# emiliofidalgo/liodom

Hardware: AMD Instinct MI355X
Metric: scans/sec (64×1800 cloud, prev_frames=20) at 1 GPU; pose RMSE vs CPU ref (higher is better)
Workload: dtype f64

## Files before the change

liodom_amd/csrc/kernels_knn.h:

```cpp
constexpr float kCellInv = 1.0f;
constexpr double kCellSize = 1.0;

struct Top5 {
  unsigned long long k0, k1, k2, k3, k4;
  int p0, p1, p2, p3, p4;
};
constexpr unsigned long long kTop5Empty = (0x7f800000ull << 32) | 0x7fffffffull;
__device__ __forceinline__ float top5_dist(unsigned long long k) { return __int_as_float((int)(k >> 32)); }
__device__ __forceinline__ int top5_index(unsigned long long k) { return (int)(unsigned int)(k & 0xFFFFFFFFull); }
#define TOP5_STAGE(K, P)                                          \
  {                                                               \
    const bool lt = ck < (K);                                     \
    const unsigned long long nk = lt ? ck : (K);                  \
    const int np = lt ? cp : (P);                                 \
    ck = lt ? (K) : ck;                                           \
    cp = lt ? (P) : cp;                                           \
    (K) = nk; (P) = np;                                           \
  }
__device__ __forceinline__ void top5_insert(Top5& t, float d, int wi, int pos) {
  unsigned long long ck = ((unsigned long long)(unsigned int)__float_as_int(d) << 32) | (unsigned int)wi;
  int cp = pos;
  if (ck < t.k4) {
    TOP5_STAGE(t.k0, t.p0)
    TOP5_STAGE(t.k1, t.p1)
    TOP5_STAGE(t.k2, t.p2)
    TOP5_STAGE(t.k3, t.p3)
    TOP5_STAGE(t.k4, t.p4)
  }
}
#undef TOP5_STAGE
__device__ __forceinline__ void top5_clear(Top5& t) {
  t.k0 = t.k1 = t.k2 = t.k3 = t.k4 = kTop5Empty;
  t.p0 = t.p1 = t.p2 = t.p3 = t.p4 = -1;
}
struct Top5Acc {
  Top5 t;
  __device__ __forceinline__ void consider(bool ok, float d, int wi, int pos) { if (ok && d <= top5_dist(t.k4)) top5_insert(t, d, wi, pos); }
};

struct Best2Acc {
  float m1, m2, m3;
  int p1, p2;
  __device__ __forceinline__ void clear() { m1 = m2 = m3 = __int_as_float(0x7f800000); p1 = p2 = -1; }
  __device__ __forceinline__ void consider(bool ok, float d0, int , int pos) {
    const float d = ok ? d0 : __int_as_float(0x7f800000);
    const bool lt1 = d < m1, lt2 = d < m2;
    m3 = __builtin_amdgcn_fmed3f(m2, m3, d);
    const int q2 = lt2 ? pos : p2;
    p2 = lt1 ? p1 : q2;
    m2 = __builtin_amdgcn_fmed3f(m1, m2, d);
    p1 = lt1 ? pos : p1;
    m1 = lt1 ? d : m1;
  }
};

#ifndef LIODOM_TUNE_B_BIG
#define LIODOM_TUNE_B_BIG 64
#define LIODOM_TUNE_B_LOADS_BIG 2
#define LIODOM_TUNE_B_LOADS_FLAT 2
#define LIODOM_TUNE_B_CURSOR false
#define LIODOM_TUNE_B_NEAR 0.0036f
#endif
#ifndef LIODOM_TUNE_B_WAVES
#define LIODOM_TUNE_B_WAVES 7
#endif
#ifndef LIODOM_TUNE_D_BIG
#define LIODOM_TUNE_D_BIG 128
#define LIODOM_TUNE_D_LOADS 4
#define LIODOM_TUNE_D_NEAR 0.04f
#endif
template <bool kDeep> struct KnnTune {
  static constexpr int kBigCell = kDeep ? LIODOM_TUNE_D_BIG : LIODOM_TUNE_B_BIG;
  static constexpr int kLoadsBig = kDeep ? LIODOM_TUNE_D_LOADS : LIODOM_TUNE_B_LOADS_BIG;
  static constexpr int kLoadsFlat = kDeep ? LIODOM_TUNE_D_LOADS : LIODOM_TUNE_B_LOADS_FLAT;
  static constexpr float kNearSq = kDeep ? LIODOM_TUNE_D_NEAR : LIODOM_TUNE_B_NEAR;
  static constexpr bool kProbeBoth = kDeep;
  static constexpr bool kHoistLoads = kDeep;
  static constexpr bool kCursor = kDeep ? false : LIODOM_TUNE_B_CURSOR;
};
constexpr int kKnnGridDiv = 2;
typedef float f32x2_t __attribute__((ext_vector_type(2)));
__device__ __forceinline__ float sqdist_cand(float qx, float qy, float qz, const float4& m) {
#if defined(LIODOM_KNN_PK)
  const f32x2_t q = {qx, qy};
  const f32x2_t mm = {m.x, m.y};
  const f32x2_t d = q - mm;
  const f32x2_t sq = d * d;
  float r = sq.x;
  r = r + sq.y;
  const float dz = qz - m.z;
  r = r + dz * dz;
  return r;
#else
  return sqdist_f(qx, qy, qz, m.x, m.y, m.z);
#endif
}
template <class Acc, int UB, int U, int kBigCell, bool kCursor = false>
__device__ __forceinline__ void knn_stream_cells(Acc& t, const float4* sp, int* s_incl, int* s_adj,
                                                 unsigned int start, unsigned int cnt, int hl,
                                                 float qx, float qy, float qz, unsigned int* dbg = nullptr) {
  const unsigned long long dbg_t0 = dbg ? wall_clock64() : 0ull;
  {
    const int half_base = (threadIdx.x & 32);
    unsigned int big = (unsigned int)((__ballot(cnt >= (unsigned int)kBigCell) >> half_base) & 0xFFFFFFFFull);
    while (big) {
      const int l = __ffs(big) - 1;
      big &= big - 1u;
      const int cs = __shfl((int)start, l, kKnnGroup), cc = __shfl((int)cnt, l, kKnnGroup);
      const float4* cp = sp + cs;
      for (int i = hl; i < cc; i += UB * kKnnGroup) {
        float4 m[UB];
#pragma unroll
        for (int u = 0; u < UB; u++) { const int iu = i + u * kKnnGroup; m[u] = cp[iu < cc ? iu : cc - 1]; }
#pragma unroll
        for (int u = 0; u < UB; u++) {
          const int iu = i + u * kKnnGroup;
          t.consider(iu < cc, sqdist_cand(qx, qy, qz, m[u]), __float_as_int(m[u].w), cs + iu);
        }
      }
    }
    if (cnt >= (unsigned int)kBigCell) cnt = 0;
  }
  const unsigned int dbg_nseg = dbg ? (unsigned int)__popc((unsigned int)(__ballot(cnt > 0) >> (threadIdx.x & 32))) : 0u;
  const int incl = half_incl_scan_i32((int)cnt);
  s_incl[hl] = incl;
  s_adj[hl] = (int)start - (incl - (int)cnt);
  __builtin_amdgcn_wave_barrier();
  const int T = s_incl[kKnnGroup - 1];
  const unsigned long long dbg_t1 = dbg ? wall_clock64() : 0ull;
  int cur = 0;
  for (int i = hl; i < T; i += U * kKnnGroup) {
    int a[U];
    int c[U];
#pragma unroll
    for (int u = 0; u < U; u++) { const int iu = i + u * kKnnGroup; a[u] = iu < T ? iu : T - 1; c[u] = 0; }
    if (kCursor) {
#pragma unroll
      for (int u = 0; u < U; u++) {
        while (s_incl[cur] <= a[u]) cur++;
        c[u] = cur;
      }
    } else {
#pragma unroll
      for (int step = kKnnGroup / 2; step >= 1; step >>= 1) {
        int pv[U];
#pragma unroll
        for (int u = 0; u < U; u++) pv[u] = s_incl[c[u] + step - 1];
#pragma unroll
        for (int u = 0; u < U; u++) c[u] += pv[u] <= a[u] ? step : 0;
      }
    }
    int adj[U];
#pragma unroll
    for (int u = 0; u < U; u++) adj[u] = s_adj[c[u]];
#pragma unroll
    for (int u = 0; u < U; u++) a[u] += adj[u];
    float4 m[U];
#pragma unroll
    for (int u = 0; u < U; u++) m[u] = sp[a[u]];
#pragma unroll
    for (int u = 0; u < U; u++)
      t.consider(i + u * kKnnGroup < T, sqdist_cand(qx, qy, qz, m[u]), __float_as_int(m[u].w), a[u]);
  }
  __builtin_amdgcn_wave_barrier();
  if (dbg && hl == 0) {
    dbg[0] = (unsigned int)(dbg_t1 - dbg_t0);
    dbg[1] = (unsigned int)(wall_clock64() - dbg_t1);
    dbg[2] = ((unsigned int)((T + U * kKnnGroup - 1) / (U * kKnnGroup)) << 16) | ((unsigned int)T << 20);
    dbg[3] = dbg_nseg;
  }
}

__device__ __forceinline__ bool best2_select(const Best2Acc& t, int hl, int half_shift, float& d5, int (&pos)[5]) {
  unsigned int v = (unsigned int)__float_as_int(t.m1), w = (unsigned int)__float_as_int(t.m2);
  int ph = t.p1, pn = t.p2;
  unsigned int g[6];
#pragma unroll
  for (int r = 0; r < 5; r++) {
    g[r] = half_min_u32(v);
    const unsigned int win = (unsigned int)((__ballot(v == g[r]) >> half_shift) & 0xFFFFFFFFull);
    const int l = __ffs(win) - 1;
    pos[r] = __shfl(ph, l, kKnnGroup);
    const bool mine = hl == l;
    v = mine ? w : v;
    w = mine ? 0x7f800000u : w;
    ph = mine ? pn : ph;
  }
  g[5] = half_min_u32(v);
  const unsigned int s3 = half_min_u32((unsigned int)__float_as_int(t.m3));
  const unsigned int one = 0x3f800000u;
  d5 = __int_as_float((int)g[4]);
  if (g[4] < one) return g[0] < g[1] && g[1] < g[2] && g[2] < g[3] && g[3] < g[4] && g[4] < g[5] && g[4] < s3;
  return s3 >= one;
}


__device__ __forceinline__ void knn_merge(Top5& t, Top5& g, int hl, int half_shift) {
  unsigned long long gk[5]; int gp[5];
#pragma unroll
  for (int r = 0; r < 5; r++) {
    const unsigned long long key = t.k0;
    const unsigned int dmin = half_min_u32((unsigned int)(key >> 32));
    unsigned int win = (unsigned int)((__ballot((unsigned int)(key >> 32) == dmin) >> half_shift) & 0xFFFFFFFFull);
    unsigned long long mk;
    if (__popc(win) == 1) {
      mk = ((unsigned long long)dmin << 32) | (unsigned int)__shfl((int)(unsigned int)(key & 0xFFFFFFFFull), __ffs(win) - 1, kKnnGroup);
    } else {
      mk = half_min_u64(key);
      win = (unsigned int)((__ballot(key == mk) >> half_shift) & 0xFFFFFFFFull);
    }
    const int wl = __ffs(win) - 1;
    gp[r] = __shfl(t.p0, wl, kKnnGroup);
    gk[r] = mk;
    if (hl == wl) {
      t.k0 = t.k1; t.k1 = t.k2; t.k2 = t.k3; t.k3 = t.k4; t.k4 = kTop5Empty;
      t.p0 = t.p1; t.p1 = t.p2; t.p2 = t.p3; t.p3 = t.p4; t.p4 = -1;
    }
  }
  g.k0 = gk[0]; g.k1 = gk[1]; g.k2 = gk[2]; g.k3 = gk[3]; g.k4 = gk[4];
  g.p0 = gp[0]; g.p1 = gp[1]; g.p2 = gp[2]; g.p3 = gp[3]; g.p4 = gp[4];
}

__device__ void rebuild_alloc(const DevView& v, int s, StreamState& st, int block, int nblocks);
__device__ void rebuild_count_and_pad(const DevView& v, int s, StreamState& st, int eb, int block, int* sbase, int* sslot, bool keep);

template <int kQ>
struct KnnShared {
  int incl[kQ][kKnnGroup];
  int adj[kQ][kKnnGroup];
  float nn[kQ][16];
  int res[kQ][4];
  double part[kQ][32];
  double blk[kQ][24];
};

__device__ __forceinline__ float best2_bound(const Best2Acc& t, int half_shift) {
  float B = 1.0f;
  const float thr[4] = {0.36f, 0.09f, 0.0225f, 0.0036f};
#pragma unroll
  for (int k = 0; k < 4; k++) {
    const int c = __popc((unsigned int)(__ballot(t.m1 <= thr[k]) >> half_shift)) + __popc((unsigned int)(__ballot(t.m2 <= thr[k]) >> half_shift));
    B = c >= 5 ? thr[k] : B;
  }
  return B;
}

template <class Tune>
__device__ __forceinline__ void knn_probe_cells(const DevView& v, const StreamState& st, int fc, int hl, int cx, int cy, int cz, float qx, float qy, float qz,
                                                const CellSlot* cells, const unsigned int* bits, unsigned int tmask,
                                                unsigned int& start, unsigned int& cnt, float& lb) {
  if (hl < 27) {
    const int dx = hl % 3 - 1, dy = (hl / 3) % 3 - 1, dz = hl / 9 - 1;
    const unsigned long long key = pack_cell(cx + dx, cy + dy, cz + dz);
    unsigned int h = hash_cell(key, tmask);
    if (Tune::kProbeBoth) {
      const unsigned int word = bits[h >> 5];
      const uint4 raw = *reinterpret_cast<const uint4*>(cells + h);
      const unsigned long long k = ((unsigned long long)raw.y << 32) | raw.x;
      bool more = ((word >> (h & 31)) & 1u) != 0u;
      if (more && k == key) { start = raw.z; cnt = raw.w; more = false; }
      for (int pr = 1; more && pr < v.table_size; pr++) {
        h = (h + 1) & tmask;
        if (!((bits[h >> 5] >> (h & 31)) & 1u)) break;
        const uint4 r2 = *reinterpret_cast<const uint4*>(cells + h);
        if ((((unsigned long long)r2.y << 32) | r2.x) == key) { start = r2.z; cnt = r2.w; break; }
      }
    } else {
      for (int pr = 0; pr < v.table_size; pr++) {
        if (!((bits[h >> 5] >> (h & 31)) & 1u)) break;
        const uint4 raw = *reinterpret_cast<const uint4*>(cells + h);
        const unsigned long long k = ((unsigned long long)raw.y << 32) | raw.x;
        if (k == key) { start = raw.z; cnt = raw.w; break; }
        h = (h + 1) & tmask;
      }
    }
    const float cs = (float)kCellSize;
    const float lx = (float)(cx + dx) * cs, ly = (float)(cy + dy) * cs, lz = (float)(cz + dz) * cs;
    const float ex = qx < lx ? lx - qx : (qx > lx + cs ? qx - (lx + cs) : 0.0f);
    const float ey = qy < ly ? ly - qy : (qy > ly + cs ? qy - (ly + cs) : 0.0f);
    const float ez = qz < lz ? lz - qz : (qz > lz + cs ? qz - (lz + cs) : 0.0f);
    lb = (ex * ex + ey * ey + ez * ez) * (1.0f - 1e-5f);
  } else if (hl == 27 && v.early_rebuild) {
    start = (unsigned int)v.ovf_base;
    cnt = (unsigned int)st.n_ovf[LD_TAB_PARITY(v, fc)];
  }
}

struct KnnPre {
  float gsq;
  float4 sq;
  int p[5];
  float4 c[5];
};
constexpr float kOvMargin = 0.03f;
#ifndef LIODOM_OV_MARGIN_PER_M
#define LIODOM_OV_MARGIN_PER_M 0.004f
#endif
constexpr float kOvMarginPerMetre = LIODOM_OV_MARGIN_PER_M;
constexpr float kOvMarginMax = 0.30f;
template <int kKnnThreads>
__device__ __forceinline__ void knn_presearch(const DevView& v, int s, const StreamState& st, int fc, int e, int E,
                                              KnnShared<kKnnThreads / kKnnGroup>& sh, KnnPre& pre, float range) {
  typedef KnnTune<(kKnnThreads >= 256)> Tune;
  const int grp = threadIdx.x / kKnnGroup, hl = threadIdx.x & (kKnnGroup - 1);
  const int ec = e < v.edge_cap ? e : v.edge_cap - 1;
  pre.gsq = 0.f;
  pre.sq = make_float4(0.f, 0.f, 0.f, __int_as_float(0x7f800000));
#pragma unroll
  for (int k = 0; k < 5; k++) { pre.p[k] = -1; pre.c[k] = make_float4(0.f, 0.f, 0.f, 0.f); }
  if (!v.knn_save_q) return;
  pre.sq = v.knn_save_q[(size_t)s * v.edge_cap + ec];
  const float qx = pre.sq.x, qy = pre.sq.y, qz = pre.sq.z;
  const bool act = e < E && !v.knn_exact_only && ld_isfinite((double)qx) && ld_isfinite((double)qy) && ld_isfinite((double)qz) &&
                   fabsf(qx) < 1.0e9f && fabsf(qy) < 1.0e9f && fabsf(qz) < 1.0e9f;
  if (!act) return;
  const int cx = (int)floorf(qx * kCellInv), cy = (int)floorf(qy * kCellInv), cz = (int)floorf(qz * kCellInv);
  const unsigned int tmask = st.table_mask;
  const int stab = s + LD_TAB_PARITY(v, fc) * v.n_streams;
  const CellSlot* cells = v.cells + (size_t)stab * v.table_size;
  const unsigned int* bits = v.cell_bits + (size_t)stab * (v.table_size >> 5);
  const float4* sp = v.sorted_pts + (size_t)stab * v.sorted_cap;
  unsigned int start = 0, cnt = 0;
  float lb = 0.0f;
  knn_probe_cells<Tune>(v, st, fc, hl, cx, cy, cz, qx, qy, qz, cells, bits, tmask, start, cnt, lb);
  const float margin = fminf(kOvMargin + kOvMarginPerMetre * range, kOvMarginMax);
  const float r = fminf(sqrtf(pre.sq.w), 1.0f) + margin;
  const float B = r * r * (1.0f + 1e-5f);
  Top5Acc ta;
  {
    const unsigned long long sentinel = ((unsigned long long)(unsigned int)__float_as_int(B) << 32) | 0x7fffffffull;
    ta.t.k0 = ta.t.k1 = ta.t.k2 = ta.t.k3 = ta.t.k4 = sentinel;
    ta.t.p0 = ta.t.p1 = ta.t.p2 = ta.t.p3 = ta.t.p4 = -1;
  }
  const bool all = cnt > 0 && !(lb > B);
  knn_stream_cells<Top5Acc, 2, 2, 64>(ta, sp, sh.incl[grp], sh.adj[grp], start, all ? cnt : 0u, hl, qx, qy, qz);
  float gl = B;
  if (ta.t.p4 >= 0) gl = fminf(gl, top5_dist(ta.t.k4));
  pre.gsq = __int_as_float((int)half_min_u32((unsigned int)__float_as_int(gl)));
  pre.p[0] = ta.t.p0; pre.p[1] = ta.t.p1; pre.p[2] = ta.t.p2; pre.p[3] = ta.t.p3; pre.p[4] = ta.t.p4;
#pragma unroll
  for (int k = 0; k < 5; k++) pre.c[k] = sp[pre.p[k] >= 0 ? pre.p[k] : 0];
}

template <int kKnnThreads, bool kPre = false, bool kTail = true, bool kWt = kPre>
__device__ __forceinline__ void knn_block(const DevView& v, int s, StreamState& st, int fc, int outer_it, int eb, int bv, int E,
                                          KnnShared<kKnnThreads / kKnnGroup>& sh, const float4& p_in, const double (&T_in)[12],
                                          const KnnPre& pre, const double* qt) {
  constexpr int kKnnQueries = kKnnThreads / kKnnGroup;
  typedef KnnTune<(kKnnThreads >= 256)> Tune;
  const int grp = threadIdx.x / kKnnGroup;
  const int e = bv * kKnnQueries + grp;
  const int hl = threadIdx.x & (kKnnGroup - 1);
  const int half_shift = (threadIdx.x & 32);
  const bool dbgb = (bv == 5) && (s == 0) && (threadIdx.x == 0) && (outer_it == 0);
  const unsigned long long t_blk = (kInstrument && (v.debug & 32)) ? wall_clock64() : 0ull;
  DBG_STAMP(v, dbgb, 1, 0);
  bool active = e < E;
  float qx = 0.f, qy = 0.f, qz = 0.f;
  if (active) {
    float4 p = p_in;
    double T[12];
#pragma unroll
    for (int i = 0; i < 12; i++) T[i] = T_in[i];
    if (!Tune::kHoistLoads) {
      p = v.edges[((size_t)eb * v.n_streams + s) * v.edge_cap + e];
#pragma unroll
      for (int i = 0; i < 12; i++) T[i] = st.odom[i];
    }
    transform_point(T, p.x, p.y, p.z, &qx, &qy, &qz);
    if (v.knn_q && hl == 0) v.knn_q[((size_t)s * 2 + outer_it) * v.edge_cap + e] = make_float4(qx, qy, qz, 0.f);
    active = ld_isfinite((double)qx) && ld_isfinite((double)qy) && ld_isfinite((double)qz) &&
             fabsf(qx) < 1.0e9f && fabsf(qy) < 1.0e9f && fabsf(qz) < 1.0e9f;
  }
  DBG_STAMP(v, dbgb, 1, 1); DBG_QSTAMP(1);
  if (hl == 0) { sh.res[grp][0] = 0; sh.res[grp][1] = -1; sh.res[grp][2] = -1; }
  float d5 = __int_as_float(0x7f800000);
  if (active) {
    const int cx = (int)floorf(qx * kCellInv), cy = (int)floorf(qy * kCellInv), cz = (int)floorf(qz * kCellInv);
    const unsigned int tmask = st.table_mask;
    const int stab = s + LD_TAB_PARITY(v, fc) * v.n_streams;
    const CellSlot* cells = v.cells + (size_t)stab * v.table_size;
    const unsigned int* bits = v.cell_bits + (size_t)stab * (v.table_size >> 5);
    const float4* sp = v.sorted_pts + (size_t)stab * v.sorted_cap;
    float d5_r = __int_as_float(0x7f800000);
    int pos5[5] = {-1, -1, -1, -1, -1};
    bool reranked = false;
    if (kPre) {
      if ((kInstrument && (v.debug & 64)) && hl == 0 && !(pre.gsq > 0.f)) atomicAdd(&v.dbg_clk[262], 1ull);
      if (pre.gsq > 0.f) {
        Top5 t, g;
        top5_clear(t);
#pragma unroll
        for (int k = 0; k < 5; k++) {
          if (pre.p[k] >= 0) top5_insert(t, sqdist_f(qx, qy, qz, pre.c[k].x, pre.c[k].y, pre.c[k].z), __float_as_int(pre.c[k].w), pre.p[k]);
        }
        knn_merge(t, g, hl, half_shift);
        const float d5n = g.p4 >= 0 ? top5_dist(g.k4) : __int_as_float(0x7f800000);
        const double ddx = (double)qx - (double)pre.sq.x, ddy = (double)qy - (double)pre.sq.y, ddz = (double)qz - (double)pre.sq.z;
        const double delta = sqrt(ddx * ddx + ddy * ddy + ddz * ddz) * (1.0 + 1e-12);
        const double r = sqrt((double)pre.gsq) * (1.0 - 2e-7) - delta;
        double limit = r > 0.0 ? r * r * (1.0 - 1e-6) : 0.0;
        {
          const double cs = kCellSize;
          const double fx = (double)qx - (double)(int)floorf(pre.sq.x * kCellInv) * cs, fy = (double)qy - (double)(int)floorf(pre.sq.y * kCellInv) * cs,
                       fz = (double)qz - (double)(int)floorf(pre.sq.z * kCellInv) * cs;
          const double edge = fmin(fmin(fmin(fx, cs - fx), fmin(fy, cs - fy)), fmin(fz, cs - fz));
          const double ro = (cs + edge) * (1.0 - 2e-7);
          const double lo = ro > 0.0 ? ro * ro * (1.0 - 1e-6) : 0.0;
          limit = limit < lo ? limit : lo;
        }
        reranked = (double)d5n < limit || limit > 1.0;
        if ((kInstrument && (v.debug & 64)) && hl == 0) {
          atomicAdd(&v.dbg_clk[261], 1ull);
          if (!reranked) {
            const float rn = fminf(sqrtf(pre.sq.w), 1.0f) + kOvMargin;
            atomicAdd(&v.dbg_clk[g.p4 < 0 ? 264 : 265], 1ull);
            if (delta > 0.01) atomicAdd(&v.dbg_clk[266], 1ull);
            if (pre.gsq < rn * rn) atomicAdd(&v.dbg_clk[267], 1ull);
            if (!(pre.sq.w < 1.0f)) atomicAdd(&v.dbg_clk[268], 1ull);
            if (delta > 0.03) atomicAdd(&v.dbg_clk[269], 1ull);
          }
        }
        if (reranked) {
          d5_r = d5n;
          pos5[0] = g.p0; pos5[1] = g.p1; pos5[2] = g.p2; pos5[3] = g.p3; pos5[4] = g.p4;
          if (d5n < 1.0f) {
#pragma unroll
            for (int k = 0; k < 5; k++) {
              if (pre.p[k] >= 0) {
                const int r = pre.p[k] == g.p0 ? 0 : pre.p[k] == g.p1 ? 1 : pre.p[k] == g.p2 ? 2 : pre.p[k] == g.p3 ? 3 : pre.p[k] == g.p4 ? 4 : -1;
                if (r >= 0) {
                  sh.nn[grp][r * 3 + 0] = pre.c[k].x; sh.nn[grp][r * 3 + 1] = pre.c[k].y; sh.nn[grp][r * 3 + 2] = pre.c[k].z;
                  if (r < 2) sh.res[grp][1 + r] = __float_as_int(pre.c[k].w);
                }
              }
            }
            if (hl == 0) sh.res[grp][0] = 1;
          }
        }
      }
    } else
    if (outer_it == 1 && v.knn_save_pos && !v.knn_exact_only) {
      const float gsq = v.knn_save_g[(size_t)s * v.edge_cap + e];
      if (gsq > 0.f) {
        const float4 sq = v.knn_save_q[(size_t)s * v.edge_cap + e];
        const int2 sv = v.knn_save_pos[((size_t)s * v.edge_cap + e) * kKnnGroup + hl];
        const float4 m0 = sp[sv.x >= 0 ? sv.x : 0], m1 = sp[sv.y >= 0 ? sv.y : 0];
        Best2Acc br;
        br.clear();
        br.consider(sv.x >= 0, sqdist_f(qx, qy, qz, m0.x, m0.y, m0.z), 0, sv.x);
        br.consider(sv.y >= 0, sqdist_f(qx, qy, qz, m1.x, m1.y, m1.z), 0, sv.y);
        float d5n;
        int p5[5];
        const bool sel_ok = best2_select(br, hl, half_shift, d5n, p5);
        const double ddx = (double)qx - (double)sq.x, ddy = (double)qy - (double)sq.y, ddz = (double)qz - (double)sq.z;
        const double delta = sqrt(ddx * ddx + ddy * ddy + ddz * ddz) * (1.0 + 1e-12);
        const double r = sqrt((double)gsq) * (1.0 - 2e-7) - delta;
        const double limit = r > 0.0 ? r * r * (1.0 - 1e-6) : 0.0;
        reranked = sel_ok && ((double)d5n < limit || limit > 1.0);
        if (reranked) {
          d5_r = d5n;
#pragma unroll
          for (int k = 0; k < 5; k++) pos5[k] = p5[k];
        }
      }
    }
    if ((kInstrument && (v.debug & 64)) && hl == 0 && outer_it == 1) atomicAdd(&v.dbg_clk[259 + (reranked ? 0 : 1)], 1ull);
    if (!reranked) {
    unsigned int start = 0, cnt = 0;
    float lb = 0.0f;
    knn_probe_cells<Tune>(v, st, fc, hl, cx, cy, cz, qx, qy, qz, cells, bits, tmask, start, cnt, lb);
    DBG_STAMP(v, dbgb, 1, 2); DBG_QSTAMP(2);
    float B = 1.0f;
    bool have_b = false;
    if (outer_it == 1 && v.knn_save_q) {
      const float4 sq = kPre ? pre.sq : v.knn_save_q[(size_t)s * v.edge_cap + e];
      if (sq.w < 1.0f) {
        const float ddx = qx - sq.x, ddy = qy - sq.y, ddz = qz - sq.z;
        const float delta = sqrtf(ddx * ddx + ddy * ddy + ddz * ddz);
        const float r = sqrtf(sq.w) * (1.0f + 1e-6f) + delta * (1.0f + 1e-6f) + 1e-7f;
        B = fminf(1.0f, r * r * (1.0f + 1e-5f));
        have_b = true;
      }
    }
    bool pend = cnt > 0;
    Best2Acc b2;
    b2.clear();
    int dbg_n = 0;
    bool dbg_two_phase = false;
    {
      const bool now = pend && (have_b ? !(lb > B) : (hl == 13 || hl == 27 || lb <= Tune::kNearSq));
      if (kInstrument && (v.debug & 32)) dbg_n = __shfl(half_incl_scan_i32(now ? (int)cnt : 0), kKnnGroup - 1, kKnnGroup);
      knn_stream_cells<Best2Acc, Tune::kLoadsBig, Tune::kLoadsFlat, Tune::kBigCell, Tune::kCursor>(b2, sp, sh.incl[grp], sh.adj[grp], start, now ? cnt : 0u, hl, qx, qy, qz,
                                                                                     ((kInstrument && (v.debug & 32)) && s == 0 && e < E) ? v.dbg_q + ((size_t)outer_it * v.edge_cap + e) * 12 + 8 : nullptr);
      pend = pend && !now;
    }
    DBG_STAMP(v, dbgb, 1, 3); DBG_QSTAMP(3);
    if (!have_b && ((__ballot(pend) >> half_shift) & 0xFFFFFFFFull)) {
      B = best2_bound(b2, half_shift);
      pend = pend && !(lb > B);
      if ((__ballot(pend) >> half_shift) & 0xFFFFFFFFull) {
        if (kInstrument && (v.debug & 32)) { dbg_n += __shfl(half_incl_scan_i32(pend ? (int)cnt : 0), kKnnGroup - 1, kKnnGroup); dbg_two_phase = true; }
        knn_stream_cells<Best2Acc, Tune::kLoadsBig, Tune::kLoadsFlat, Tune::kBigCell, Tune::kCursor>(b2, sp, sh.incl[grp], sh.adj[grp], start, pend ? cnt : 0u, hl, qx, qy, qz);
      }
    } else {
      pend = false;
    }
    DBG_STAMP(v, dbgb, 1, 4); DBG_QSTAMP(4);
    const bool certain = best2_select(b2, hl, half_shift, d5, pos5) && !v.knn_exact_only;
    if ((kInstrument && (v.debug & 32)) && s == 0 && e < E && hl == 0) v.dbg_q[((size_t)outer_it * v.edge_cap + e) * 12] = (unsigned int)dbg_n | (dbg_two_phase ? 0x40000000u : 0u) | (certain ? 0u : 0x80000000u);
    if ((kInstrument && (v.debug & 64)) && hl == 0) {
      atomicAdd(&v.dbg_clk[256 + (certain ? 0 : 1)], 1ull);
      if (dbg_two_phase) atomicAdd(&v.dbg_clk[258], 1ull);
      atomicAdd(&v.dbg_clk[384 + (dbg_n / 64 < 63 ? dbg_n / 64 : 63)], 1ull);
    }
    if (!certain) {
      const bool all = cnt > 0 && (!(lb > B) || (!have_b && (hl == 13 || hl == 27 || lb <= Tune::kNearSq)));
      Top5Acc ta;
      Top5 g;
      {
        const float bnd = d5 < 1.0f ? d5 : 1.0f;
        const unsigned long long sentinel = ((unsigned long long)(unsigned int)__float_as_int(bnd) << 32) | 0x7fffffffull;
        ta.t.k0 = ta.t.k1 = ta.t.k2 = ta.t.k3 = ta.t.k4 = sentinel;
        ta.t.p0 = ta.t.p1 = ta.t.p2 = ta.t.p3 = ta.t.p4 = -1;
      }
      knn_stream_cells<Top5Acc, 2, 2, 64>(ta, sp, sh.incl[grp], sh.adj[grp], start, all ? cnt : 0u, hl, qx, qy, qz);
      knn_merge(ta.t, g, hl, half_shift);
      d5 = g.p4 >= 0 ? top5_dist(g.k4) : __int_as_float(0x7f800000);
      pos5[0] = g.p0; pos5[1] = g.p1; pos5[2] = g.p2; pos5[3] = g.p3; pos5[4] = g.p4;
    }
    if (outer_it == 0 && v.knn_save_pos && !(kWt && !kPre)) {
      const float sk = (cnt > 0 && !(!(lb > B) || (!have_b && (hl == 13 || hl == 27 || lb <= Tune::kNearSq)))) ? lb : __int_as_float(0x7f800000);
      unsigned int gd = half_min_u32((unsigned int)__float_as_int(sk));
      const unsigned int m3m = half_min_u32((unsigned int)__float_as_int(b2.m3));
      gd = m3m < gd ? m3m : gd;
      float guard = __int_as_float((int)gd);
      {
        const float cs = (float)kCellSize;
        const float fx = qx - (float)cx * cs, fy = qy - (float)cy * cs, fz = qz - (float)cz * cs;
        float edge = fminf(fminf(fminf(fx, cs - fx), fminf(fy, cs - fy)), fminf(fz, cs - fz));
        edge = edge > 0.f ? edge : 0.f;
        const float outer = (cs + edge) * (cs + edge) * (1.0f - 1e-6f);
        guard = guard < outer ? guard : outer;
      }
      v.knn_save_pos[((size_t)s * v.edge_cap + e) * kKnnGroup + hl] = make_int2(b2.p1, b2.p2);
      if (hl == 0) v.knn_save_g[(size_t)s * v.edge_cap + e] = guard < 3.0e38f ? guard : 3.0e38f;
    }
    if ((kInstrument && (v.debug & 64)) && s == 0 && hl == 0) {
      const int bin = (int)((wall_clock64() - t_blk) / 100ull);
      atomicAdd(&v.dbg_clk[320 + (bin < 63 ? bin : 63)], 1ull);
      const int nb = dbg_n < 64 ? 0 : dbg_n < 128 ? 1 : dbg_n < 256 ? 2 : dbg_n < 512 ? 3 : dbg_n < 1024 ? 4 : 5;
      atomicAdd(&v.dbg_clk[448 + (bin / 4 < 7 ? bin / 4 : 7) * 8 + nb + (dbg_two_phase ? 0 : 0)], 1ull);
      if (!certain) atomicAdd(&v.dbg_clk[448 + (bin / 4 < 7 ? bin / 4 : 7) * 8 + 7], 1ull);
      if (dbg_two_phase) atomicAdd(&v.dbg_clk[448 + (bin / 4 < 7 ? bin / 4 : 7) * 8 + 6], 1ull);
    }
    }
    else d5 = d5_r;
    DBG_STAMP(v, dbgb, 1, 5); DBG_QSTAMP(5);
    if (d5 < 1.0f && !(kPre && reranked)) {
      const int mypos = hl == 0 ? pos5[0] : hl == 1 ? pos5[1] : hl == 2 ? pos5[2] : hl == 3 ? pos5[3] : pos5[4];
      if (hl < 5) {
        const float4 m = sp[mypos];
        sh.nn[grp][hl * 3 + 0] = m.x; sh.nn[grp][hl * 3 + 1] = m.y; sh.nn[grp][hl * 3 + 2] = m.z;
        if (hl < 2) sh.res[grp][1 + hl] = __float_as_int(m.w);
      }
      if (hl == 0) sh.res[grp][0] = 1;
    }
  }
  if (outer_it == 0 && v.knn_save_q && e < E && hl == 0) {
    v.knn_save_q[(size_t)s * v.edge_cap + e] = make_float4(qx, qy, qz, d5);
    if (!active && v.knn_save_g) v.knn_save_g[(size_t)s * v.edge_cap + e] = 0.f;
  }
  if (!kTail) return;
  __syncthreads();
  DBG_STAMP(v, dbgb, 1, 6); DBG_QSTAMP(6);
  if (kKnnThreads < 256 && v.knn_nn) {
    if (threadIdx.x < kKnnQueries * 5) {
      const int q = threadIdx.x / 5, j = threadIdx.x % 5;
      const int eq = bv * kKnnQueries + q;
      if (eq < v.edge_cap) {
        const int w = j == 0 ? sh.res[q][0] : (j == 1 ? sh.res[q][1] : (j == 2 ? sh.res[q][2] : 0));
        v.knn_nn[((size_t)s * v.edge_cap + eq) * 5 + j] = make_float4(sh.nn[q][j * 3], sh.nn[q][j * 3 + 1], sh.nn[q][j * 3 + 2], __int_as_float(w));
      }
    }
    return;
  }
  if (threadIdx.x < kKnnQueries) {
    const int q = threadIdx.x;
    const int eq = bv * kKnnQueries + q;
    bool valid = (eq < E) && (sh.res[q][0] != 0);
    float nx[5], ny[5], nz[5];
#pragma unroll
    for (int j = 0; j < 5; j++) { nx[j] = sh.nn[q][j * 3]; ny[j] = sh.nn[q][j * 3 + 1]; nz[j] = sh.nn[q][j * 3 + 2]; }
    if (valid) valid = line_gate(nx, ny, nz);
    if (eq < E) {
      float4* ca = v.corr_a + ((size_t)s * 2 + outer_it) * v.edge_cap + eq;
      float4* cb = v.corr_b + ((size_t)s * 2 + outer_it) * v.edge_cap + eq;
      int2* cidx = v.corr_idx + ((size_t)s * 2 + outer_it) * v.edge_cap + eq;
      const float4 oa = valid ? make_float4(nx[0], ny[0], nz[0], 1.0f) : make_float4(0, 0, 0, 0);
      const float4 ob = valid ? make_float4(nx[1], ny[1], nz[1], 0.0f) : make_float4(0, 0, 0, 0);
      const int2 oi = valid ? make_int2(sh.res[q][1], sh.res[q][2]) : make_int2(-1, -1);
      if (kWt) {
        wt_store_f4(ca, oa); wt_store_f4(cb, ob);
        wt_store_u64(cidx, ((unsigned long long)(unsigned int)oi.y << 32) | (unsigned int)oi.x);
      } else {
        *ca = oa; *cb = ob; *cidx = oi;
      }
    }
    const unsigned long long vb = __ballot(valid);
    const int nvalid = __popcll(vb);
    if (q == 0) {
      if (nvalid && !v.knn_partials) atomicAdd(&st.info.matches[outer_it], nvalid);
      unsigned char* cm = &v.corr_mask[((size_t)s * 2 + outer_it) * v.mask_stride + bv];
      if (kWt) wt_store_u8(cm, (unsigned char)vb); else *cm = (unsigned char)vb;
    }
    sh.res[q][3] = valid ? 1 : 0;
  } else if (kKnnThreads > 64 && v.knn_partials && threadIdx.x >= 64 && threadIdx.x < 64 + kKnnQueries) {
    const int q = threadIdx.x - 64;
    const int eq = bv * kKnnQueries + q;
    double flag = 0.0;
    if (eq < E && sh.res[q][0] != 0) {
      double Rm[12], pq[4], pt[3];
#pragma unroll
      for (int i = 0; i < 4; i++) pq[i] = kWt ? qt[i] : st.param_q[i];
#pragma unroll
      for (int i = 0; i < 3; i++) pt[i] = kWt ? qt[4 + i] : st.param_t[i];
      iso_from_qt(pq, pt, Rm);
      const float4 pe = v.edges[((size_t)eb * v.n_streams + s) * v.edge_cap + eq];
      const double p[3] = {(double)pe.x, (double)pe.y, (double)pe.z};
      const double a[3] = {(double)sh.nn[q][0], (double)sh.nn[q][1], (double)sh.nn[q][2]};
      const double b[3] = {(double)sh.nn[q][3], (double)sh.nn[q][4], (double)sh.nn[q][5]};
      double J[18], rs[3], rho0, rho1;
      const bool ok = residual_block(Rm, p, a, b, v.min_range, v.max_range, J, rs, &rho0, &rho1);
#pragma unroll
      for (int i = 0; i < 18; i++) sh.blk[q][i] = J[i];
      sh.blk[q][18] = rs[0]; sh.blk[q][19] = rs[1]; sh.blk[q][20] = rs[2]; sh.blk[q][21] = rho0; sh.blk[q][22] = rho1;
      flag = ok ? 1.0 : 2.0;
    }
    sh.blk[q][23] = flag;
  }
  if (!v.knn_partials) return;
  __syncthreads();
  if (hl < kAccN) {
    const double flag = sh.res[grp][3] ? sh.blk[grp][23] : 0.0;
    double x = 0.0;
    if (flag == 1.0) x = residual_entry(sh.blk[grp], sh.blk[grp] + 18, sh.blk[grp][21], sh.blk[grp][22], hl);
    else if (flag == 2.0 && hl == 28) x = 1.0;
    sh.part[grp][hl] = x;
  } else if (hl == kAccN) {
    sh.part[grp][hl] = sh.res[grp][3] ? 1.0 : 0.0;
  }
  __syncthreads();
  if (threadIdx.x <= kAccN) {
    double x = 0.0;
#pragma unroll
    for (int q = 0; q < kKnnQueries; q++) x += sh.part[q][threadIdx.x];
    double* dst = &v.knn_part[(((size_t)s * 2 + outer_it) * v.knn_blocks + bv) * 32 + threadIdx.x];
    if (kWt) wt_store_u64(dst, (unsigned long long)__double_as_longlong(x)); else *dst = x;
  }
  DBG_STAMP(v, dbgb, 1, 7); DBG_QSTAMP(7);
  if ((kInstrument && (v.debug & 64)) && s == 0 && threadIdx.x == 0) {
    const unsigned long long d = wall_clock64() - t_blk;
    const int bin = (int)(d / 100ull);
    atomicAdd(&v.dbg_clk[192 + (bin < 63 ? bin : 63)], 1ull);
  }
}

template <int kKnnThreads>
__device__ __forceinline__ void knn_tail_dual(const DevView& v, int s, int outer_it, int eb, int bvA, int bvB, bool haveB, int E,
                                              KnnShared<kKnnThreads / kKnnGroup>& shA, KnnShared<kKnnThreads / kKnnGroup>& shB, const double* qt) {
  constexpr int kKnnQueries = kKnnThreads / kKnnGroup;
  static_assert(kKnnThreads == 256, "two blocks of 8 queries on four waves");
  const int grp = threadIdx.x / kKnnGroup, hl = threadIdx.x & (kKnnGroup - 1);
  const int half = (int)threadIdx.x >> 7, t = (int)threadIdx.x & 127;
  KnnShared<kKnnQueries>& sh = half ? shB : shA;
  const int bv = half ? bvB : bvA;
  const bool live = half ? haveB : true;
  if (t < kKnnQueries && live) {
    const int q = t;
    const int eq = bv * kKnnQueries + q;
    bool valid = (eq < E) && (sh.res[q][0] != 0);
    float nx[5], ny[5], nz[5];
#pragma unroll
    for (int j = 0; j < 5; j++) { nx[j] = sh.nn[q][j * 3]; ny[j] = sh.nn[q][j * 3 + 1]; nz[j] = sh.nn[q][j * 3 + 2]; }
    if (valid) valid = line_gate(nx, ny, nz);
    if (eq < E) {
      const float4 oa = valid ? make_float4(nx[0], ny[0], nz[0], 1.0f) : make_float4(0, 0, 0, 0);
      const float4 ob = valid ? make_float4(nx[1], ny[1], nz[1], 0.0f) : make_float4(0, 0, 0, 0);
      const int2 oi = valid ? make_int2(sh.res[q][1], sh.res[q][2]) : make_int2(-1, -1);
      wt_store_f4(v.corr_a + ((size_t)s * 2 + outer_it) * v.edge_cap + eq, oa);
      wt_store_f4(v.corr_b + ((size_t)s * 2 + outer_it) * v.edge_cap + eq, ob);
      wt_store_u64(v.corr_idx + ((size_t)s * 2 + outer_it) * v.edge_cap + eq, ((unsigned long long)(unsigned int)oi.y << 32) | (unsigned int)oi.x);
    }
    const unsigned long long vb = __ballot(valid);
    if (q == 0) wt_store_u8(&v.corr_mask[((size_t)s * 2 + outer_it) * v.mask_stride + bv], (unsigned char)vb);
    sh.res[q][3] = valid ? 1 : 0;
  } else if (t >= 64 && t < 64 + kKnnQueries && live) {
    const int q = t - 64;
    const int eq = bv * kKnnQueries + q;
    double flag = 0.0;
    if (eq < E && sh.res[q][0] != 0) {
      double Rm[12], pq[4], pt[3];
#pragma unroll
      for (int i = 0; i < 4; i++) pq[i] = qt[i];
#pragma unroll
      for (int i = 0; i < 3; i++) pt[i] = qt[4 + i];
      iso_from_qt(pq, pt, Rm);
      const float4 pe = v.edges[((size_t)eb * v.n_streams + s) * v.edge_cap + eq];
      const double p[3] = {(double)pe.x, (double)pe.y, (double)pe.z};
      const double a[3] = {(double)sh.nn[q][0], (double)sh.nn[q][1], (double)sh.nn[q][2]};
      const double b[3] = {(double)sh.nn[q][3], (double)sh.nn[q][4], (double)sh.nn[q][5]};
      double J[18], rs[3], rho0, rho1;
      const bool ok = residual_block(Rm, p, a, b, v.min_range, v.max_range, J, rs, &rho0, &rho1);
#pragma unroll
      for (int i = 0; i < 18; i++) sh.blk[q][i] = J[i];
      sh.blk[q][18] = rs[0]; sh.blk[q][19] = rs[1]; sh.blk[q][20] = rs[2]; sh.blk[q][21] = rho0; sh.blk[q][22] = rho1;
      flag = ok ? 1.0 : 2.0;
    }
    sh.blk[q][23] = flag;
  }
  __syncthreads();
#pragma unroll
  for (int b = 0; b < 2; b++) {
    if (b == 1 && !haveB) break;
    KnnShared<kKnnQueries>& shb = b ? shB : shA;
    if (hl < kAccN) {
      const double flag = shb.res[grp][3] ? shb.blk[grp][23] : 0.0;
      double x = 0.0;
      if (flag == 1.0) x = residual_entry(shb.blk[grp], shb.blk[grp] + 18, shb.blk[grp][21], shb.blk[grp][22], hl);
      else if (flag == 2.0 && hl == 28) x = 1.0;
      shb.part[grp][hl] = x;
    } else if (hl == kAccN) {
      shb.part[grp][hl] = shb.res[grp][3] ? 1.0 : 0.0;
    }
  }
  __syncthreads();
  if (t <= kAccN && live) {
    double x = 0.0;
#pragma unroll
    for (int q = 0; q < kKnnQueries; q++) x += sh.part[q][t];
    wt_store_u64(&v.knn_part[(((size_t)s * 2 + outer_it) * v.knn_blocks + bv) * 32 + t], (unsigned long long)__double_as_longlong(x));
  }
}

__device__ __forceinline__ void chain_release_edges(const DevView& v, unsigned int signal_odo) {
  typedef __attribute__((address_space(1))) unsigned int gu32;
  if (signal_odo && threadIdx.x == 0) INJECT_DELAY(14);
  if (signal_odo && threadIdx.x == 0) __hip_atomic_store((gu32*)(v.pipe_flags + kEdgePipeBufs), signal_odo, __ATOMIC_RELAXED, __HIP_MEMORY_SCOPE_AGENT);
}

template <int kKnnThreads, bool kOv, bool kChain>
__device__ __forceinline__ bool knn_pass(const DevView& v, int s, int bxi, int byi, int outer_it, int eb, unsigned int wait_edges,
                                         unsigned int signal_odo, unsigned int seq, int scan_no, KnnShared<kKnnThreads / kKnnGroup>& sh, KnnShared<kKnnThreads / kKnnGroup>& sh2, double* sh_ov, int pred_copy = 0) {
  constexpr int kKnnQueries = kKnnThreads / kKnnGroup;
  static_assert(!(kOv && kChain), "the overlapped pass is the second pass, the chain-mode instance the first");
  StreamState& st = v.state[s];
  if (kOv) {
    if (!pipe_wait(v.ov_flags + s, seq, &st.status)) return false;
    OV_STAMP(v, threadIdx.x == 0 && bxi == 0, 9); OV_STAMP(v, threadIdx.x == 0 && bxi == v.knn_grid - 1, 13);
  } else if (kChain) {
    const bool pred_ok = pred_wait(v, s, bxi % kOvReplicas, (unsigned int)scan_no, sh_ov, &st.status, v.pipe_flags + eb, wait_edges, pred_copy);
    OV_STAMP(v, threadIdx.x == 0 && bxi == 0, 27);
    if (bxi == 0 && threadIdx.x == 0) { st.reb_frame_count = scan_no; st.n_used_tab[(scan_no + 1) & 1] = 0; st.reb_initialized = 1; st.cursor = 0; }
    if (pred_ok && bxi == 0 && threadIdx.x >= 64 && threadIdx.x < 76) st.pred_odom[scan_no & 1][threadIdx.x - 64] = sh_ov[threadIdx.x - 64];
    if (!pred_ok) return false;
  } else if (v.early_rebuild) {
    if (bxi >= v.knn_grid) { if (outer_it == 1) rebuild_alloc(v, s, st, bxi - v.knn_grid, (int)gridDim.x - v.knn_grid); return true; }
    if (outer_it == 0 && bxi == 0 && threadIdx.x == 0) {
      st.reb_frame_count = st.frame_count; st.n_used_tab[(st.frame_count + 1) & 1] = 0; st.reb_initialized = st.initialized;
      st.cursor = 0;
    }
    if (outer_it == 0 && bxi == 0 && threadIdx.x >= 64 && threadIdx.x < 76) st.pred_odom[st.frame_count & 1][threadIdx.x - 64] = st.odom[threadIdx.x - 64];
  }
  if (!kOv && outer_it == 0) {
    if (!kChain && signal_odo && bxi == 0 && byi == 0 && threadIdx.x == 0) {
      typedef __attribute__((address_space(1))) unsigned int gu32;
      __hip_atomic_store((gu32*)(v.pipe_flags + kEdgePipeBufs), signal_odo, __ATOMIC_RELAXED, __HIP_MEMORY_SCOPE_AGENT);
    }
    if (!kChain && wait_edges && !pipe_wait(v.pipe_flags + eb, wait_edges, &st.status)) return false;
  }
  typedef KnnTune<(kKnnThreads >= 256)> Tune;
  const int e_first = bxi * kKnnQueries + (int)(threadIdx.x / kKnnGroup);
  float4 p_first = make_float4(0.f, 0.f, 0.f, 0.f);
  double T[12] = {0, 0, 0, 0, 0, 0, 0, 0, 0, 0, 0, 0};
  if (Tune::kHoistLoads) {
    p_first = v.edges[((size_t)eb * v.n_streams + s) * v.edge_cap + (e_first < v.edge_cap ? e_first : v.edge_cap - 1)];
    if (!kOv && !kChain) {
#pragma unroll
      for (int i = 0; i < 12; i++) T[i] = st.odom[i];
    }
  }
  if (kChain) {
#pragma unroll
    for (int i = 0; i < 12; i++) T[i] = sh_ov[i];
  }
  const unsigned int st_status = st.status;
  const int st_init = kChain ? 1 : st.initialized;
  const int fc = kChain ? scan_no : st.frame_count;
  int E;
  if (kChain) {
    typedef __attribute__((address_space(1))) unsigned int gu32;
    E = (int)__hip_atomic_load((gu32*)(v.edge_cnt + eb * 32 + s), __ATOMIC_RELAXED, __HIP_MEMORY_SCOPE_AGENT);
  } else {
    E = st.n_edges_buf[eb];
  }
  if (st_status & LIODOM_STATUS_PIPE_TIMEOUT) return false;
  if (!st_init) return true;
  static_assert(kKnnGridDiv == 2, "k_knn handles exactly two query blocks per workgroup");
  constexpr bool kWt = kOv || kChain;
  if (bxi * kKnnQueries >= E) {
    if (threadIdx.x == 0) {
      unsigned char* cm = &v.corr_mask[((size_t)s * 2 + outer_it) * v.mask_stride + bxi];
      if (kWt) wt_store_u8(cm, 0); else *cm = 0;
      if (bxi + v.knn_grid < v.knn_blocks) { if (kWt) wt_store_u8(cm + v.knn_grid, 0); else cm[v.knn_grid] = 0; }
    }
    return true;
  }
  const int bv2 = bxi + v.knn_grid;
  const int e_second = bv2 * kKnnQueries + (int)(threadIdx.x / kKnnGroup);
  const bool second = bv2 < v.knn_blocks && bv2 * kKnnQueries < E;
  KnnPre pre1, pre2;
  float4 p_second = make_float4(0.f, 0.f, 0.f, 0.f);
  if (kOv) {
    if (second) p_second = v.edges[((size_t)eb * v.n_streams + s) * v.edge_cap + (e_second < v.edge_cap ? e_second : v.edge_cap - 1)];
    knn_presearch<kKnnThreads>(v, s, st, fc, e_first, E, sh, pre1, sqrtf(p_first.x * p_first.x + p_first.y * p_first.y + p_first.z * p_first.z));
    if (second) knn_presearch<kKnnThreads>(v, s, st, fc, e_second, E, sh2, pre2, sqrtf(p_second.x * p_second.x + p_second.y * p_second.y + p_second.z * p_second.z));
    else pre2.gsq = 0.f;
    if (!ov_wait_pose(v, s, bxi % kOvReplicas, seq, sh_ov, &st.status)) return false;
    OV_STAMP(v, threadIdx.x == 0 && bxi == 0, 10); OV_STAMP(v, threadIdx.x == 0 && bxi == v.knn_grid - 1, 14);
    if (kInstrument && (v.debug & 128) && threadIdx.x == 0) {
      sh_ov[19] = __longlong_as_double((long long)wall_clock64());
      const unsigned long long pub = *(volatile unsigned long long*)&v.dbg_clk[448 + 1];
      const long long d = (long long)wall_clock64() - (long long)pub;
      if (pub && d >= 0) atomicAdd(&v.dbg_clk[320 + (d / 25 < 63 ? d / 25 : 63)], 1ull);
    }
#pragma unroll
    for (int i = 0; i < 12; i++) T[i] = sh_ov[i];
  }
  if constexpr (kOv) {
    knn_block<kKnnThreads, true, false>(v, s, st, fc, outer_it, eb, bxi, E, sh, p_first, T, pre1, sh_ov + 12);
    if (second) knn_block<kKnnThreads, true, false>(v, s, st, fc, outer_it, eb, bv2, E, sh2, p_second, T, pre2, sh_ov + 12);
    else if (bv2 < v.knn_blocks && threadIdx.x == 0) wt_store_u8(&v.corr_mask[((size_t)s * 2 + outer_it) * v.mask_stride + bv2], 0);
    __syncthreads();
    knn_tail_dual<kKnnThreads>(v, s, outer_it, eb, bxi, bv2, second, E, sh, sh2, sh_ov + 12);
    if (!v.speculate) return true;
    const int cf = ov_confirm_pose(v, s, bxi % kOvReplicas, seq, sh_ov, &st.status);
    if ((kInstrument && (v.debug & 64)) && threadIdx.x == 0) atomicAdd(&v.dbg_clk[271 + (cf == 1 ? 0 : 1)], 1ull);
    return cf == 1;
  }
  knn_block<kKnnThreads, false, true, kWt>(v, s, st, fc, outer_it, eb, bxi, E, sh, p_first, T, pre1, kChain ? sh_ov + 12 : nullptr);
  if (bv2 >= v.knn_blocks) return true;
  if (!second) {
    if (threadIdx.x == 0) { unsigned char* cm = &v.corr_mask[((size_t)s * 2 + outer_it) * v.mask_stride + bv2]; if (kWt) wt_store_u8(cm, 0); else *cm = 0; }
    return true;
  }
  __syncthreads();
  double T2[12] = {0, 0, 0, 0, 0, 0, 0, 0, 0, 0, 0, 0};
  if (Tune::kHoistLoads) {
    p_second = v.edges[((size_t)eb * v.n_streams + s) * v.edge_cap + (e_second < v.edge_cap ? e_second : v.edge_cap - 1)];
    asm volatile("" ::: "memory");
    if (kChain) {
#pragma unroll
      for (int i = 0; i < 12; i++) T2[i] = sh_ov[i];
    } else {
#pragma unroll
      for (int i = 0; i < 12; i++) T2[i] = st.odom[i];
    }
  }
  knn_block<kKnnThreads, false, true, kWt>(v, s, st, fc, outer_it, eb, bv2, E, sh, p_second, T2, pre2, kChain ? sh_ov + 12 : nullptr);
  return true;
}

template <int kKnnThreads, bool kOv = false, bool kChain = false>
__global__ __launch_bounds__(kKnnThreads, (kKnnThreads >= 256 ? 1 : LIODOM_TUNE_B_WAVES)) void k_knn(DevView v, int s0, int outer_it, int eb, unsigned int wait_edges, unsigned int signal_odo, unsigned int seq, int scan_no) {
  constexpr int kKnnQueries = kKnnThreads / kKnnGroup;
#if defined(LIODOM_CHAIN_PRIO)
  if (kKnnThreads >= 256) __builtin_amdgcn_s_setprio(LIODOM_CHAIN_PRIO);
#endif
  __shared__ KnnShared<kKnnQueries> shs[kOv ? 2 : 1];
  KnnShared<kKnnQueries>& sh = shs[0];
  __shared__ double sh_ov[(kOv || kChain) ? 20 : 1];
  int bxi = (int)blockIdx.x, byi = (int)blockIdx.y;
  xcd_remap(bxi, byi);
  const int s = s0 + byi;
  if constexpr (kOv) {
    if (bxi >= v.knn_grid) {
      __shared__ int sh_rb_cnt[kMaxFrames + 1];
      __shared__ int sh_rb_slot[kMaxFrames];
      rebuild_count_and_pad(v, s, v.state[s], eb, bxi - v.knn_grid, sh_rb_cnt, sh_rb_slot, true);
      return;
    }
  }
  if (kInstrument && kOv && threadIdx.x == 0) sh_ov[19] = 0.0;
  if (kOv) { OV_STAMP(v, threadIdx.x == 0 && bxi == 0, 8); OV_STAMP(v, threadIdx.x == 0 && bxi == v.knn_grid - 1, 12); }
  else if (outer_it == 0) {
    if (kInstrument && (v.debug & 128) && threadIdx.x == 0 && bxi == 0) {
      volatile unsigned long long* c = v.dbg_clk + 448;
      const unsigned long long t16 = c[16], now = wall_clock64();
      if (t16 && c[18] > t16 && c[1] > c[18] && c[4] > c[1] && c[28] > c[4] && c[26] > c[28]) {
        unsigned long long* a = v.dbg_clk + 480;
        a[0] += c[18] - t16; a[1] += c[1] - c[18]; a[2] += c[4] - c[1]; a[3] += c[28] - c[4]; a[4] += now - t16; a[5] += 1ull;
        a[6] += c[19] > t16 ? 1ull : 0ull; a[7] += c[26] - c[28];
        if (c[20] > c[1]) { a[8] += c[20] - c[1]; a[9] += c[4] - c[20]; }
        if (c[19] > t16 && c[21] < t16) { a[10] += c[1] - c[19]; a[11] += c[20] - c[19]; a[12] += 1ull; a[13] += c[4] - c[1]; }
        if (c[19] > t16 && c[21] > t16) { a[14] += 1ull; a[15] += c[4] - c[1]; }
      }
    }
    OV_STAMP(v, threadIdx.x == 0 && bxi == 0, 16);
  }
  const bool pass_ok = knn_pass<kKnnThreads, kOv, kChain>(v, s, bxi, byi, outer_it, eb, wait_edges, signal_odo, seq, scan_no, sh, shs[kOv ? 1 : 0], sh_ov);
  if (kOv) { if (scan_no >= 0) { if (pass_ok) chain_count_done(v.knn_done0 + 32 + s); } else if (pass_ok || !v.speculate) ov_signal_knn_done(v, s, bxi, seq); }
  if (kChain) {
    int vd = 1;
    if (v.speculate) vd = pred_verdict_wait(v, s, bxi % kOvReplicas, (unsigned int)scan_no, &v.state[s].status);
    if (vd != 2 && bxi == 0) chain_release_edges(v, signal_odo);
    if (pass_ok && vd == 1) chain_count_done(v.knn_done0 + s);
  }
  if (kInstrument && (v.debug & 128) && threadIdx.x == 0) {
    if (kOv) {
      const long long t_seen = __double_as_longlong(sh_ov[19]);
      if (bxi * kKnnQueries < v.state[s].n_edges_buf[eb] && t_seen) { const long long d = (long long)wall_clock64() - t_seen; atomicAdd(&v.dbg_clk[256 + (d / 50 < 63 ? d / 50 : 63)], 1ull); }
    } else if (outer_it == 0) {
      const unsigned long long t0 = *(volatile unsigned long long*)&v.dbg_clk[448 + 16];
      const long long d = (long long)wall_clock64() - (long long)t0;
      if (t0 && d >= 0 && bxi * kKnnQueries < v.state[s].n_edges_buf[eb]) atomicAdd(&v.dbg_clk[384 + (d / 50 < 63 ? d / 50 : 63)], 1ull);
    }
  }
  if (kOv) {
    OV_STAMP(v, threadIdx.x == 0 && bxi == 0, 11); OV_STAMP(v, threadIdx.x == 0 && bxi == v.knn_grid - 1, 15);
    if (kInstrument && (v.debug & 128) && threadIdx.x == 0 && bxi * kKnnQueries < v.state[s].n_edges_buf[eb]) atomicMax(&v.dbg_clk[448 + 20], wall_clock64());
  }
  else if (outer_it == 0) OV_STAMP(v, threadIdx.x == 0 && bxi == v.knn_grid - 1, 17);
}

template <int kKnnThreads>
__global__ __launch_bounds__(kKnnThreads, 1) void k_knn_redo(DevView v, int s0, int eb, unsigned int seq, int scan_no, int alloc_blocks) {
  constexpr int kKnnQueries = kKnnThreads / kKnnGroup;
  __shared__ KnnShared<kKnnQueries> shs[2];
  __shared__ double sh_ov[20];
  __shared__ double sh_first[20];
  if ((int)blockIdx.x < alloc_blocks) { rebuild_alloc(v, s0 + (int)blockIdx.y, v.state[s0 + (int)blockIdx.y], (int)blockIdx.x, alloc_blocks); return; }
  int bxi = (int)blockIdx.x - alloc_blocks, byi = (int)blockIdx.y;
  const int s = s0 + byi;
  StreamState& st = v.state[s];
  const int rep = bxi % kOvReplicas;
  if (!granules_wait<LIODOM_POLL_POSE>(v.pose_xch0 + ((size_t)s * kOvReplicas + rep) * 512, kOvGranules, seq, sh_first, &st.status)) return;
  if (!granules_wait<LIODOM_POLL_POSE>(v.pose_xch0 + ((size_t)s * kOvReplicas + rep) * 512 + kOvFinalOffset, kOvGranules, seq, sh_ov, &st.status)) return;
  bool same = true;
  for (int i = 0; i < 19; i++) same = same && __double_as_longlong(sh_first[i]) == __double_as_longlong(sh_ov[i]);
  if (same) return;
  if (st.status & (LIODOM_STATUS_PIPE_TIMEOUT | LIODOM_STATUS_LM_SYNC_TIMEOUT)) return;
  if ((kInstrument && (v.debug & 64)) && threadIdx.x == 0) atomicAdd(&v.dbg_clk[273], 1ull);
  OV_STAMP(v, threadIdx.x == 0, 21);
  DevView vr = v;
  vr.knn_save_pos = nullptr;
  const int fc = st.frame_count;
  const int E = st.n_edges_buf[eb];
  const int outer_it = 1;
  if (!st.initialized || (st.status & LIODOM_STATUS_PIPE_TIMEOUT)) return;
  const int bv2 = bxi + v.knn_grid;
  if (bxi * kKnnQueries < E) {
    const bool second = bv2 < v.knn_blocks && bv2 * kKnnQueries < E;
    const float4* ed = v.edges + ((size_t)eb * v.n_streams + s) * v.edge_cap;
    const int e_first = bxi * kKnnQueries + (int)(threadIdx.x / kKnnGroup), e_second = bv2 * kKnnQueries + (int)(threadIdx.x / kKnnGroup);
    const float4 p_first = ed[e_first < v.edge_cap ? e_first : v.edge_cap - 1];
    const float4 p_second = ed[e_second < v.edge_cap ? e_second : v.edge_cap - 1];
    double T[12];
#pragma unroll
    for (int i = 0; i < 12; i++) T[i] = sh_ov[i];
    KnnPre none;
    none.gsq = 0.f;
    knn_block<kKnnThreads, false, false, true>(vr, s, st, fc, outer_it, eb, bxi, E, shs[0], p_first, T, none, sh_ov + 12);
    if (second) knn_block<kKnnThreads, false, false, true>(vr, s, st, fc, outer_it, eb, bv2, E, shs[1], p_second, T, none, sh_ov + 12);
    else if (bv2 < v.knn_blocks && threadIdx.x == 0) wt_store_u8(&v.corr_mask[((size_t)s * 2 + outer_it) * v.mask_stride + bv2], 0);
    __syncthreads();
    knn_tail_dual<kKnnThreads>(v, s, outer_it, eb, bxi, bv2, second, E, shs[0], shs[1], sh_ov + 12);
  }
  else return;
  if (scan_no >= 0) chain_count_done(v.knn_done0 + 32 + s); else ov_signal_knn_done(v, s, bxi, seq);
}

__global__ void k_ov_gate(DevView v, int s, unsigned int seq) {
  OV_STAMP(v, threadIdx.x == 0, 6);
  (void)pipe_wait(v.ov_flags + s, seq, &v.state[s].status);
  OV_STAMP(v, threadIdx.x == 0, 7);
}

__global__ __launch_bounds__(256) void k_line_gate(DevView v, int s0, int outer_it, int eb) {
  const int s = s0 + blockIdx.y;
  StreamState& st = v.state[s];
  if (v.knn8_cnt && blockIdx.x == 0 && threadIdx.x == 0) v.knn8_cnt[s] = 0;
  if (!st.initialized) return;
  const int E = st.n_edges_buf[eb];
  const int eq = blockIdx.x * 256 + threadIdx.x;
  const int Q = v.knn_queries;
  if (eq >= v.knn_blocks * Q) return;
  float nx[5], ny[5], nz[5];
  int found = 0, i0 = -1, i1 = -1;
  if (eq < E) {
    const float4* k = v.knn_nn + ((size_t)s * v.edge_cap + eq) * 5;
#pragma unroll
    for (int j = 0; j < 5; j++) {
      const float4 m = k[j];
      nx[j] = m.x; ny[j] = m.y; nz[j] = m.z;
      if (j == 0) found = __float_as_int(m.w);
      if (j == 1) i0 = __float_as_int(m.w);
      if (j == 2) i1 = __float_as_int(m.w);
    }
  } else {
#pragma unroll
    for (int j = 0; j < 5; j++) { nx[j] = 0.f; ny[j] = 0.f; nz[j] = 0.f; }
  }
  bool valid = (eq < E) && (found != 0);
  if (valid) valid = line_gate(nx, ny, nz);
  if (eq < E) {
    float4* ca = v.corr_a + ((size_t)s * 2 + outer_it) * v.edge_cap + eq;
    float4* cb = v.corr_b + ((size_t)s * 2 + outer_it) * v.edge_cap + eq;
    int2* cidx = v.corr_idx + ((size_t)s * 2 + outer_it) * v.edge_cap + eq;
    if (valid) {
      *ca = make_float4(nx[0], ny[0], nz[0], 1.0f);
      *cb = make_float4(nx[1], ny[1], nz[1], 0.0f);
      *cidx = make_int2(i0, i1);
    } else {
      *ca = make_float4(0, 0, 0, 0); *cb = make_float4(0, 0, 0, 0); *cidx = make_int2(-1, -1);
    }
  }
  const unsigned long long vb = __ballot(valid);
  const int lane = threadIdx.x & 63;
  if (lane == 0) { const int nvalid = __popcll(vb); if (nvalid) atomicAdd(&st.info.matches[outer_it], nvalid); }
  if ((lane % Q) == 0) v.corr_mask[((size_t)s * 2 + outer_it) * v.mask_stride + eq / Q] = (unsigned char)((vb >> lane) & ((1ull << Q) - 1ull));
}
```

liodom_amd/csrc/liodom_hip.hip:

```cpp
#include <hip/hip_runtime.h>

#include <algorithm>
#include <cmath>
#include <cstdint>
#include <cstdio>
#include <cstdlib>
#include <cstring>
#include <limits>
#include <atomic>
#include <chrono>
#include <mutex>
#include <string>
#include <vector>

#include "liodom_kernels.h"

using namespace liodom_dev;

namespace {

thread_local std::string g_last_error;

#define HIP_TRY(expr)                                                                         \
  do {                                                                                        \
    hipError_t _e = (expr);                                                                   \
    if (_e != hipSuccess) {                                                                   \
      char _buf[512];                                                                         \
      snprintf(_buf, sizeof(_buf), "%s failed: %s (%s:%d)", #expr, hipGetErrorString(_e),    \
               __FILE__, __LINE__);                                                           \
      g_last_error = _buf;                                                                    \
      return LIODOM_ERR_HIP;                                                                  \
    }                                                                                         \
  } while (0)

enum KernelId {
  KID_CLASSIFY = 0, KID_RING_EXTRACT, KID_COMPACT, KID_KNN, KID_LM, KID_HASH_CLEAR,
  KID_WINDOW_INSERT, KID_HASH_ALLOC, KID_HASH_SCATTER, KID_RING_SCATTER, KID_HASH_BUILD, KID_OTHER
};
const char* kKernelNames[LIODOM_NUM_KERNELS] = {
    "k_classify", "k_ring_extract", "k_compact_edges", "k_knn", "k_lm_solve",
    "k_hash_clear", "k_window_insert", "k_hash_alloc", "k_hash_scatter", "k_ring_scatter", "k_hash_build", "other"};

struct EventPair { hipEvent_t a, b; int kid; };

}

#include "liodom_map_host.h"

std::atomic<int> g_live_handles{0};

struct liodom_handle {
  liodom_handle() {
    for (int b = 0; b < kEdgePipeBufs; b++) { ev_free_valid[b] = false; eb_reader[b] = 0u; tk_seq[b] = 0u; }
  }
  liodom_params_t params;
  liodom_config_t config;
  DevView v{};
  DevView* d_view = nullptr;
  std::mutex mx_x, mx_o;
  hipStream_t stream = nullptr;
  hipStream_t stream_k = nullptr;
  bool counted_live = false;
  bool ov_ok = false;
  unsigned int ov_seq = 0;
  hipEvent_t ev_ov = nullptr;
  bool stream_c_shared = false;
  bool ov_suppress = false;
  bool ov_prev = false;
  double replay_enq_ns = 0.0, replay_wait_ns = 0.0;
  long long replay_timed = 0;
  bool chain_ok = false;
  bool chain_prev = false;
  unsigned int chain_count = 0;
  int verdict_scan = -1;
  bool verdict_confirmed = false;
  bool chain_fix_pending = false;
  bool chain_used = false;
  hipEvent_t ev_ch = nullptr;
  int ov_warm = 0;
  hipStream_t stream_x = nullptr;
  hipStream_t stream_c = nullptr;
  hipEvent_t ev_up[3] = {nullptr, nullptr, nullptr};
  hipEvent_t ev_xdone[3] = {nullptr, nullptr, nullptr};
  bool ev_xdone_valid[3] = {false, false, false};
  hipEvent_t ev_edges[kEdgePipeBufs] = {nullptr, nullptr, nullptr};
  hipEvent_t ev_free[kEdgePipeBufs] = {nullptr, nullptr, nullptr};
  std::atomic<bool> ev_free_valid[kEdgePipeBufs];
  int parity = 0;
  unsigned int ext_seq = 0, odo_seq = 0;
  unsigned int eb_seq[kEdgePipeBufs] = {0, 0, 0};
  std::atomic<unsigned int> eb_reader[kEdgePipeBufs];
  std::atomic<unsigned int> tk_seq[kEdgePipeBufs];
  int x_next = 0;
  int odo_fifo[2] = {0, 0}, odo_pending = 0;
  float4* host_edges = nullptr;
  int4* host_edges_meta = nullptr;
  unsigned int* host_edges_hdr = nullptr;
  float4* pin_ring = nullptr;
  std::vector<double> replay_stamps;
  hipEvent_t ev_pin[kEdgePipeBufs] = {nullptr, nullptr, nullptr};
  bool ev_pin_valid[kEdgePipeBufs] = {false, false, false};
  int pin_next = 0;
  bool safe_mode = false;
  bool ring_split_lb = false;
  unsigned int lb_tag = 0;
  bool ring_split = true;
  int ring_split_max_wgs = 0;
  bool streams_concurrent = true;
  std::atomic<bool> pipe_active{false};
  std::atomic<bool> replay_live{false};
  std::atomic<bool> fallback_pending{false};
  int pf_slot = -1;
  int last_eb = 0;
  hipEvent_t pose_event = nullptr;
  int S = 1, H = 0, P = 0;
  bool lockstep = false;
  size_t ring_lds_bytes = 0;
  float4* stage_in = nullptr;
  float4* resident = nullptr;
  int n_slots = 0;
  HostOut* host_out = nullptr;
  std::vector<int> scans_enqueued;
  std::vector<void*> allocs;
  std::atomic<bool> profiling{false};
  std::vector<liodom_map*> mappers;
  std::vector<int> mapper_cells_xy, mapper_cells_z;
  int hb_since = -1;
  int knn8_grid = 1;
  bool knn8 = false;
  bool lds_hash_build = false;
  bool use_flags = false;
  bool flag_gate = false;
  std::vector<EventPair> ev_pool;
  size_t ev_used = 0;
  double k_ms[LIODOM_NUM_KERNELS] = {0};
  long long k_count[LIODOM_NUM_KERNELS] = {0};
};

namespace {

template <typename T>
int dev_alloc(liodom_handle* h, T** p, size_t count, int memset_value = 0) {
  void* raw = nullptr;
  const size_t bytes = std::max<size_t>(count, 1) * sizeof(T);
  HIP_TRY(hipMalloc(&raw, bytes));
  h->allocs.push_back(raw);
  HIP_TRY(hipMemsetAsync(raw, memset_value, bytes, h->stream));
  *p = static_cast<T*>(raw);
  return LIODOM_OK;
}

void chain_flush(liodom_handle* h) {
  if (!h->chain_fix_pending) return;
  h->chain_fix_pending = false;
  if (h->verdict_scan == h->scans_enqueued[0] && h->verdict_confirmed) return;
  const int nA = (h->v.edge_cap + 255) / 256;
  hipLaunchKernelGGL(k_chain_redo0<256>, dim3(nA, 1), dim3(256), 0, h->stream_k, h->v, 0, 0, 0u, 0u, 0u, h->scans_enqueued[0], nA, 0, 1);
}
hipError_t sync_odometry(liodom_handle* h) {
  chain_flush(h);
  hipError_t e = hipStreamSynchronize(h->stream);
  if (e == hipSuccess && h->chain_used && h->stream_k) e = hipStreamSynchronize(h->stream_k);
  return e;
}

int drain_events(liodom_handle* h) {
  if (h->ev_used == 0) return LIODOM_OK;
  HIP_TRY(hipStreamSynchronize(h->stream));
  if (h->stream_x) HIP_TRY(hipStreamSynchronize(h->stream_x));
  for (size_t i = 0; i < h->ev_used; i++) {
    float ms = 0.f;
    HIP_TRY(hipEventElapsedTime(&ms, h->ev_pool[i].a, h->ev_pool[i].b));
    h->k_ms[h->ev_pool[i].kid] += ms;
    h->k_count[h->ev_pool[i].kid] += 1;
  }
  h->ev_used = 0;
  return LIODOM_OK;
}

struct ProfScope {
  liodom_handle* h;
  EventPair* ep = nullptr;
  hipStream_t st;
  ProfScope(liodom_handle* hh, int kid, hipStream_t stream = nullptr) : h(hh), st(stream ? stream : hh->stream) {
    if (!h->profiling) return;
    if (h->ev_used == h->ev_pool.size()) {
      if (h->ev_pool.size() < 4096) {
        EventPair e; e.kid = kid;
        if (hipEventCreate(&e.a) != hipSuccess || hipEventCreate(&e.b) != hipSuccess) return;
        h->ev_pool.push_back(e);
      } else {
        drain_events(h);
      }
    }
    ep = &h->ev_pool[h->ev_used++];
    ep->kid = kid;
    hipEventRecord(ep->a, st);
  }
  ~ProfScope() { if (ep) hipEventRecord(ep->b, st); }
};

inline int cdiv(long long a, long long b) { return (int)((a + b - 1) / b); }

int launch_extract(liodom_handle* h, hipStream_t q, int eb, int s0, int count, const float4* in, size_t in_stride,
                   int n, int height, int width, unsigned int wait_odo = 0, int mirror = 0, unsigned int* pub_flag = nullptr, unsigned int* pub_host = nullptr, unsigned int pub_value = 0u) {
  const DevView& v = h->v;
  const int tiles = std::max(1, cdiv(n, kTilePts));
  if (v.lidar_type == 1 && width > 0 && (long long)h->H * width <= (long long)v.max_points) {
    ProfScope ps(h, KID_RING_SCATTER, q);
    hipLaunchKernelGGL(k_row_compact, dim3(h->H, count), dim3(kRowThreads), 0, q, v, s0, in, in_stride, n, height, width);
  } else {
    if (h->ring_split_lb && !((long long)tiles * count <= h->ring_split_max_wgs && h->ring_split)) {
      ProfScope ps(h, KID_RING_SCATTER, q);
      if (++h->lb_tag == 0u) h->lb_tag = 1u;
      hipLaunchKernelGGL(k_ring_split_lb, dim3(tiles * count), dim3(kTileThreads), ring_split_lb_lds_bytes(h->H), q, v, s0, in, in_stride, n, height, width, tiles, h->lb_tag);
      hipLaunchKernelGGL(k_ring_split_fix, dim3(1, count), dim3(kTileThreads), ring_split_lb_lds_bytes(h->H), q, v, s0, in, in_stride, n, height, width, tiles);
    } else if (h->ring_split && (long long)tiles * count <= h->ring_split_max_wgs) {
      ProfScope ps(h, KID_RING_SCATTER, q);
      hipLaunchKernelGGL(k_ring_split, dim3(tiles, count), dim3(kTileThreads), ring_scatter_lds_bytes(h->H), q, v, s0, in, in_stride, n, height, width);
    } else {
    {
      ProfScope ps(h, KID_CLASSIFY, q);
      hipLaunchKernelGGL(k_classify, dim3(tiles, count), dim3(kTileThreads), 0, q, v, s0, in, in_stride, n, height, width);
    }
    {
      ProfScope ps(h, KID_RING_SCATTER, q);
      hipLaunchKernelGGL(k_ring_scatter, dim3(tiles, count), dim3(kTileThreads), ring_scatter_lds_bytes(h->H), q, v, s0, in, in_stride, n);
    }
    }
  }
  {
    ProfScope ps(h, KID_RING_EXTRACT, q);
    const int ext = ring_extract_threads(v.scan_regions);
    const int w = h->config.max_width > 0 ? h->config.max_width : std::max(1, h->config.max_points / std::max(1, h->H));
    const int total = std::max(0, w - 10), sector = total / std::max(1, v.scan_regions);
    const bool big = total - sector * (v.scan_regions - 1) > kExLPR * kExIPL;
    const dim3 grid(h->H, count), block(ext);
    if (ext <= 256) {
      if (big) hipLaunchKernelGGL((k_ring_extract<256, kExIPLBig>), grid, block, h->ring_lds_bytes, q, v, s0);
      else hipLaunchKernelGGL((k_ring_extract<256, kExIPL>), grid, block, h->ring_lds_bytes, q, v, s0);
    } else {
      if (big) hipLaunchKernelGGL((k_ring_extract<1024, kExIPLBig>), grid, block, h->ring_lds_bytes, q, v, s0);
      else hipLaunchKernelGGL((k_ring_extract<1024, kExIPL>), grid, block, h->ring_lds_bytes, q, v, s0);
    }
  }
  {
    ProfScope ps(h, KID_COMPACT, q);
    hipLaunchKernelGGL(k_compact_edges, dim3(kCompactBlocks, count), dim3(256), 0, q, v, s0, eb, wait_odo, mirror, pub_flag, pub_host, pub_value);
  }
  HIP_TRY(hipGetLastError());
  return LIODOM_OK;
}

int enqueue_odometry(liodom_handle* h, int eb, int s0, int count, unsigned int wait_edges, unsigned int signal_odo);

int launch_odometry(liodom_handle* h, int eb, int s0, int count, unsigned int wait_edges = 0, unsigned int signal_odo = 0) {
  const int rc = enqueue_odometry(h, eb, s0, count, wait_edges, signal_odo);
  if (rc) return rc;
  h->last_eb = eb;
  for (int i = 0; i < count; i++) h->scans_enqueued[s0 + i]++;
  return LIODOM_OK;
}

struct OverlapModes { bool ov, chain; };
OverlapModes overlap_modes(const liodom_handle* h) {
  const bool base = h->v.early_rebuild && h->use_flags && g_live_handles.load() <= 1;
  return {base && h->ov_ok, base && h->chain_ok && !h->flag_gate};
}

int enqueue_odometry(liodom_handle* h, int eb, int s0, int count, unsigned int wait_edges, unsigned int signal_odo) {
  const DevView& v = h->v;
  const bool knn_small = h->lockstep;
  if (v.use_imu) {
    ProfScope ps(h, KID_OTHER);
    hipLaunchKernelGGL(k_imu_override, dim3(cdiv(count, 64)), dim3(64), 0, h->stream, v, s0, count);
  }
  const int map_blocks = cdiv(h->v.map_cap, 256);
  const bool early = v.early_rebuild != 0;
  const int nC = cdiv(h->v.edge_cap * std::max(1, h->P - 1), kLmThreads), nP = cdiv(h->v.edge_cap, kLmThreads);
  const OverlapModes om = overlap_modes(h);
  const bool chain_cand = om.chain && wait_edges != 0u;
  const bool overlap_ok = (om.ov || chain_cand) && !h->profiling && !h->ov_suppress && count == 1;
  constexpr int kOvWarmScans = 2;
  const bool overlap = overlap_ok && h->ov_warm >= kOvWarmScans;
  if (h->ov_warm < kOvWarmScans) h->ov_warm++;
  unsigned int seq_k = 0u;
  if (overlap) {
    if (++h->ov_seq == 0u) h->ov_seq = 1u;
    seq_k = h->ov_seq;
    if (!h->ov_prev) {
      HIP_TRY(hipEventRecord(h->ev_ov, h->stream));
      HIP_TRY(hipStreamWaitEvent(h->stream_k, h->ev_ov, 0));
    }
  }
  const bool chain = overlap && chain_cand;
  if (chain != h->chain_prev) {
    if (chain) {
      if (h->ov_prev) { HIP_TRY(hipEventRecord(h->ev_ov, h->stream)); HIP_TRY(hipStreamWaitEvent(h->stream_k, h->ev_ov, 0)); }
    } else {
      chain_flush(h);
      HIP_TRY(hipEventRecord(h->ev_ch, h->stream_k));
      HIP_TRY(hipStreamWaitEvent(h->stream, h->ev_ch, 0));
    }
  }
  h->chain_prev = chain;
  h->ov_prev = overlap;
  if (chain) {
    h->chain_used = true;
    const int scan_no = h->scans_enqueued[s0];
    h->chain_count += (unsigned int)v.knn_grid;
    const unsigned int done_target = h->chain_count;
    const int gx = (h->v.lm_groups - 1) * 8 + 1;
    const size_t lds = lm_lds_bytes(h->v.edge_cap);
    const int nCP = cdiv(h->v.edge_cap * std::max(1, h->P - 1), 256) + cdiv(h->v.edge_cap, 256);
    hipLaunchKernelGGL((k_knn<256, false, true>), dim3(v.knn_grid, 1), dim3(256), 0, h->stream_k, v, s0, 0, eb, wait_edges, signal_odo, seq_k, scan_no);
    if (v.speculate) {
      const int nA = cdiv(h->v.edge_cap, 256);
      hipLaunchKernelGGL(k_chain_redo0<256>, dim3(nA + v.knn_grid + 1, 1), dim3(256), 0, h->stream_k, v, s0, eb, wait_edges, signal_odo, seq_k, scan_no, nA, 1, h->chain_fix_pending ? 1 : 0);
    }
    h->chain_fix_pending = v.speculate != 0;
    hipLaunchKernelGGL((k_lm_solve<0, true>), dim3(gx, 1), dim3(kLmThreads), lds, h->stream, v, s0, eb, seq_k, done_target);
    if (!v.speculate) hipLaunchKernelGGL(k_ov_gate, dim3(1), dim3(64), 0, h->stream_k, v, s0, seq_k);
    hipLaunchKernelGGL((k_knn<256, true>), dim3(v.knn_grid + nCP, 1), dim3(256), 0, h->stream_k, v, s0, 1, eb, 0u, 0u, seq_k, scan_no);
    if (v.speculate) hipLaunchKernelGGL(k_knn_redo<256>, dim3(kRebuildAllocBlocks + v.knn_grid, 1), dim3(256), 0, h->stream_k, v, s0, eb, seq_k, scan_no, kRebuildAllocBlocks);
    hipLaunchKernelGGL((k_lm_solve<1, true>), dim3(gx, 1), dim3(kLmThreads), lds, h->stream, v, s0, eb, seq_k, done_target);
    if (!v.speculate) hipLaunchKernelGGL(k_rebuild_alloc, dim3(kRebuildAllocBlocks, 1), dim3(256), 0, h->stream_k, v, s0);
    const int nCf = cdiv(h->v.edge_cap * std::max(1, h->P - 1), kRebFinThreads), nPf = cdiv(h->v.edge_cap, kRebFinThreads);
    hipLaunchKernelGGL(k_rebuild_fin, dim3(nPf + kRebuildAuxBlocks + nCf, 1), dim3(kRebFinThreads), 0, h->stream_k, v, s0, eb);
    HIP_TRY(hipGetLastError());
    return LIODOM_OK;
  }
  for (int it = 0; it < 2; it++) {
    {
      ProfScope ps(h, KID_KNN);
      const int kx = v.knn_grid + ((early && it == 1 && !seq_k) ? kRebuildAuxBlocks : 0);
      if (knn_small && h->knn8) {
        const dim3 g8(h->knn8_grid, count);
        if (it == 0) hipLaunchKernelGGL(k_knn8<0>, g8, dim3(kKnn8Threads), 0, h->stream, v, s0, eb);
        else hipLaunchKernelGGL(k_knn8<1>, g8, dim3(kKnn8Threads), 0, h->stream, v, s0, eb);
        hipLaunchKernelGGL(k_knn8_exact, dim3(kKnn8ExactBlocks, count), dim3(kKnn8Threads), 0, h->stream, v, s0, it, eb);
        hipLaunchKernelGGL(k_line_gate, dim3(cdiv(h->v.knn_blocks * h->v.knn_queries, 256), count), dim3(256), 0, h->stream, v, s0, it, eb);
      } else if (knn_small) {
        hipLaunchKernelGGL(k_knn<128>, dim3(kx, count), dim3(128), 0, h->stream, v, s0, it, eb, wait_edges, signal_odo, 0u, 0);
        hipLaunchKernelGGL(k_line_gate, dim3(cdiv(h->v.knn_blocks * h->v.knn_queries, 256), count), dim3(256), 0, h->stream, v, s0, it, eb);
      } else if (it == 1 && seq_k) {
        hipLaunchKernelGGL(k_ov_gate, dim3(1), dim3(64), 0, h->stream_k, v, s0, seq_k);
        hipLaunchKernelGGL((k_knn<256, true>), dim3(kx, count), dim3(256), 0, h->stream_k, v, s0, it, eb, 0u, 0u, seq_k, -1);
        if (v.speculate) hipLaunchKernelGGL(k_knn_redo<256>, dim3(v.knn_grid, count), dim3(256), 0, h->stream_k, v, s0, eb, seq_k, -1, 0);
        hipLaunchKernelGGL(k_rebuild_alloc, dim3(kRebuildAllocBlocks, count), dim3(256), 0, h->stream, v, s0);
      } else {
        hipLaunchKernelGGL(k_knn<256>, dim3(kx, count), dim3(256), 0, h->stream, v, s0, it, eb, wait_edges, signal_odo, 0u, 0);
      }
    }
    {
      ProfScope ps(h, KID_LM);
      const int extra = !early ? 0 : (it == 0 ? nC + nP : nP + kRebuildAuxBlocks + nC);
      const int gx = std::max(h->v.lm_groups + extra, (h->v.lm_groups - 1) * 8 + 1);
      if (it == 0) hipLaunchKernelGGL((k_lm_solve<0, false>), dim3(gx, count), dim3(kLmThreads), lm_lds_bytes(h->v.edge_cap), h->stream, v, s0, eb, seq_k, 0u);
      else hipLaunchKernelGGL((k_lm_solve<1, false>), dim3(gx, count), dim3(kLmThreads), lm_lds_bytes(h->v.edge_cap), h->stream, v, s0, eb, seq_k, 0u);
    }
  }
  if (v.mapping) {
    for (int s = s0; s < s0 + count; s++) {
      liodom_map* mp = h->mappers[s];
      if (!mp) continue;
      ProfScope ps(h, KID_OTHER);
      StreamState* st = v.state + s;
      int rc = map_enqueue_update(mp, v.edges + ((size_t)eb * v.n_streams + s) * v.edge_cap, &st->n_edges_buf[eb], st->final_odom, h->stream);
      if (rc) return rc;
      rc = map_enqueue_local(mp, st->final_odom, h->mapper_cells_xy[s], h->mapper_cells_z[s], v.recv_pts + (size_t)s * v.recv_cap,
                             v.recv_cap, &st->n_recv, h->stream, 1);
      if (rc) return rc;
    }
  }
  if (early) {
  } else if (h->lds_hash_build) {
    ProfScope ps(h, KID_HASH_BUILD);
    const bool rebuild = !v.hash_incr || h->hb_since < 0 || h->hb_since >= kHbPeriod - 1;
    h->hb_since = rebuild ? 0 : h->hb_since + 1;
    if (!rebuild) hipLaunchKernelGGL(k_hash_append, dim3(count), dim3(kBuildThreads), 0, h->stream, v, s0, eb);
    else hipLaunchKernelGGL(k_hash_build, dim3(count), dim3(kBuildThreads), hash_build_lds_bytes(), h->stream, v, s0, eb);
  } else {
    {
      ProfScope ps(h, KID_WINDOW_INSERT);
      hipLaunchKernelGGL(k_window_insert, dim3(map_blocks, count), dim3(256), 0, h->stream, v, s0, eb);
    }
    {
      ProfScope ps(h, KID_HASH_ALLOC);
      hipLaunchKernelGGL(k_hash_alloc, dim3(map_blocks, count), dim3(256), 0, h->stream, v, s0);
    }
    {
      ProfScope ps(h, KID_HASH_SCATTER);
      hipLaunchKernelGGL(k_hash_scatter, dim3(map_blocks, count), dim3(256), 0, h->stream, v, s0);
    }
  }
  if (v.filter_local_map) {
    {
      ProfScope ps(h, KID_OTHER);
      hipLaunchKernelGGL(k_voxel_bbox, dim3(count), dim3(1024), 0, h->stream, v, s0);
      hipLaunchKernelGGL(k_voxel_insert, dim3(map_blocks, count), dim3(256), 0, h->stream, v, s0);
      hipLaunchKernelGGL(k_voxel_alloc, dim3(map_blocks, count), dim3(256), 0, h->stream, v, s0);
      hipLaunchKernelGGL(k_voxel_scatter, dim3(map_blocks, count), dim3(256), 0, h->stream, v, s0);
      hipLaunchKernelGGL(k_voxel_centroid, dim3(cdiv(h->v.map_cap, 8), count), dim3(256), 0, h->stream, v, s0);
      hipLaunchKernelGGL(k_filt_insert, dim3(map_blocks, count), dim3(256), 0, h->stream, v, s0);
    }
    {
      ProfScope ps(h, KID_HASH_ALLOC);
      hipLaunchKernelGGL(k_filt_alloc, dim3(map_blocks, count), dim3(256), 0, h->stream, v, s0);
    }
    {
      ProfScope ps(h, KID_HASH_SCATTER);
      hipLaunchKernelGGL(k_filt_scatter, dim3(map_blocks, count), dim3(256), 0, h->stream, v, s0);
    }
  }
  HIP_TRY(hipGetLastError());
  return LIODOM_OK;
}

int enter(liodom_handle* h) {
  if (!h) return LIODOM_ERR_INVALID_ARG;
  HIP_TRY(hipSetDevice(h->config.device));
  return LIODOM_OK;
}
int check_stream(liodom_handle* h, int stream) {
  int rc = enter(h);
  if (rc) return rc;
  if (stream < 0 || stream >= h->S) { g_last_error = "stream index out of range"; return LIODOM_ERR_INVALID_ARG; }
  return LIODOM_OK;
}
int check_usable(liodom_handle* h) {
  if (h->fallback_pending.load()) {
    g_last_error = "the handle had a LIODOM_STATUS_PIPE_TIMEOUT: call liodom_reset() before processing further scans";
    return LIODOM_ERR_HIP;
  }
  return LIODOM_OK;
}
struct SideLocks {
  std::unique_lock<std::mutex> lo, lx;
  SideLocks(liodom_handle* h, bool odo, bool ext) {
    if (odo || h->profiling) lo = std::unique_lock<std::mutex>(h->mx_o);
    if (ext || h->profiling) lx = std::unique_lock<std::mutex>(h->mx_x);
    if (h->profiling && !(lo.owns_lock() && lx.owns_lock())) {
      if (lx.owns_lock()) lx.unlock();
      if (!lo.owns_lock()) lo = std::unique_lock<std::mutex>(h->mx_o);
      lx = std::unique_lock<std::mutex>(h->mx_x);
    }
  }
};
hipStream_t extract_queue(liodom_handle* h) { return h->profiling ? h->stream : h->stream_x; }

int round_up(int x, int m) { return (x + m - 1) / m * m; }

int env_int(const char* name, int dflt) {
  const char* e = std::getenv(name);
  return e ? std::atoi(e) : dflt;
}

int tickets_idle(liodom_handle* h) {
  for (int b = 0; b < kEdgePipeBufs; b++) {
    if (h->tk_seq[b].load() != 0u) { g_last_error = "edge tickets of liodom_extract_edges_device are outstanding: consume them with liodom_odometry_step_device first"; return LIODOM_ERR_BUSY; }
  }
  return LIODOM_OK;
}
int drain_pipeline(liodom_handle* h) {
  const bool replayed = h->replay_live.exchange(false);
  if (h->pf_slot >= 0 || h->parity != 0 || h->pipe_active.exchange(false) || replayed) {
    HIP_TRY(hipStreamSynchronize(h->stream_x));
    HIP_TRY(sync_odometry(h));
    h->pf_slot = -1; h->parity = 0; h->ev_free_valid[0] = h->ev_free_valid[1] = h->ev_free_valid[2] = false;
    for (int b = 0; b < kEdgePipeBufs; b++) h->eb_reader[b] = 0;
  }
  return LIODOM_OK;
}

int enqueue_pipeline_odometry(liodom_handle* h, int eb, unsigned int wait_seq) {
  int rc;
  if (h->use_flags) {
    const unsigned int m = ++h->odo_seq == 0 ? ++h->odo_seq : h->odo_seq;
    if (h->flag_gate) {
      hipLaunchKernelGGL(k_pipe_gate, dim3(1), dim3(64), 0, h->stream, h->v, 0, eb, wait_seq, m - 1u);
      rc = launch_odometry(h, eb, 0, h->S);
    } else {
      rc = launch_odometry(h, eb, 0, h->S, wait_seq, m - 1u);
    }
    if (rc) return rc;
    h->eb_reader[eb] = m;
  } else {
    HIP_TRY(hipStreamWaitEvent(h->stream, h->ev_edges[eb], 0));
    rc = launch_odometry(h, eb, 0, h->S);
    if (rc) return rc;
    HIP_TRY(hipEventRecord(h->ev_free[eb], h->stream));
    h->ev_free_valid[eb] = true;
  }
  return LIODOM_OK;
}

int issue_extract(liodom_handle* h, int slot, int eb, int n, int height, int width) {
  hipStream_t q = extract_queue(h);
  const float4* in = h->resident + (size_t)slot * h->S * (size_t)h->v.max_points;
  if (h->use_flags) {
    h->eb_seq[eb] = ++h->ext_seq;
    if (h->ext_seq == 0) h->eb_seq[eb] = ++h->ext_seq;
    return launch_extract(h, q, eb, 0, h->S, in, (size_t)h->v.max_points, n, height, width, h->eb_reader[eb], 0,
                          h->v.pipe_flags + eb, nullptr, h->eb_seq[eb]);
  }
  if (h->ev_free_valid[eb]) HIP_TRY(hipStreamWaitEvent(q, h->ev_free[eb], 0));
  int rc = launch_extract(h, q, eb, 0, h->S, in, (size_t)h->v.max_points, n, height, width);
  if (rc) return rc;
  HIP_TRY(hipEventRecord(h->ev_edges[eb], q));
  return LIODOM_OK;
}

void enter_safe_mode(liodom_handle* h) {
  h->safe_mode = true;
  h->use_flags = false;
  h->chain_ok = false;
  h->v.lm_groups = 1;
  h->v.early_rebuild = 0;
  h->ring_split = false;
  h->ring_split_lb = false;
}

int reset_state(liodom_handle* h) {
  if (h->stream_x) HIP_TRY(hipStreamSynchronize(h->stream_x));
  HIP_TRY(hipStreamSynchronize(h->stream));
  if (h->stream_k) HIP_TRY(hipStreamSynchronize(h->stream_k));
  if (h->fallback_pending.exchange(false)) enter_safe_mode(h);
  std::vector<StreamState> init((size_t)h->S);
  for (auto& st : init) {
    std::memset(&st, 0, sizeof(st));
    iso_identity(st.odom); iso_identity(st.prev_odom); iso_identity(st.final_odom); iso_identity(st.pred_odom[0]); iso_identity(st.pred_odom[1]);
    st.param_q[3] = 1.0;
    st.table_mask = (uint32_t)h->v.table_size - 1u;
  }
  HIP_TRY(hipMemcpyAsync(h->v.state, init.data(), sizeof(StreamState) * init.size(), hipMemcpyHostToDevice, h->stream));
  HIP_TRY(hipMemsetAsync(h->v.pub_counter, 0, sizeof(unsigned int) * (size_t)kEdgeBufs, h->stream));
  if (h->v.lb_ticket) { HIP_TRY(hipMemsetAsync(h->v.lb_ticket, 0, sizeof(unsigned int), h->stream)); HIP_TRY(hipMemsetAsync(h->v.lb_ovf, 0, sizeof(unsigned int) * (size_t)h->S, h->stream)); }
  {
    std::vector<double> qid((size_t)h->S * 4, 0.0);
    for (int s = 0; s < h->S; s++) qid[(size_t)s * 4 + 3] = 1.0;
    HIP_TRY(hipMemcpy(h->v.imu_q, qid.data(), sizeof(double) * qid.size(), hipMemcpyHostToDevice));
  }
  {
    const size_t total = (size_t)h->S * h->v.table_size * (h->v.early_rebuild ? 2 : 1);
    hipLaunchKernelGGL(k_init_cells, dim3((unsigned)((total + 255) / 256)), dim3(256), 0, h->stream, h->v);
    HIP_TRY(hipGetLastError());
  }
  h->pf_slot = -1; h->parity = 0; h->last_eb = 0; h->ev_free_valid[0] = h->ev_free_valid[1] = h->ev_free_valid[2] = false;
  h->replay_live.store(false);
  h->hb_since = -1;
  h->ext_seq = h->odo_seq = 0;
  h->ov_warm = 0; h->ov_prev = false;
  for (int b = 0; b < kEdgePipeBufs; b++) { h->tk_seq[b] = 0u; h->ev_pin_valid[b] = false; }
  if (h->stream_c && !h->stream_c_shared) HIP_TRY(hipStreamSynchronize(h->stream_c));
  h->x_next = 0; h->odo_pending = 0;
  if (h->host_edges_hdr) std::memset(h->host_edges_hdr, 0, sizeof(unsigned int) * 2 * kEdgePipeBufs);
  for (int b = 0; b < kEdgePipeBufs; b++) { h->eb_seq[b] = 0; h->eb_reader[b] = 0; }
  HIP_TRY(hipMemsetAsync(h->v.pipe_flags, 0, sizeof(unsigned int) * (kEdgePipeBufs + 1), h->stream));
  HIP_TRY(hipMemsetAsync(h->v.lm_xch, 0, sizeof(unsigned long long) * (size_t)h->S * 2 * kLmGroupsMax * 64, h->stream));
  HIP_TRY(hipMemsetAsync(h->v.pose_xch, 0, sizeof(unsigned long long) * (size_t)h->S * 64, h->stream));
  HIP_TRY(hipMemsetAsync(h->v.redo_sync, 0, sizeof(unsigned int) * 64, h->stream));
  if (h->v.pred_xch) HIP_TRY(hipMemsetAsync(h->v.pred_xch, 0, sizeof(unsigned long long) * (size_t)h->S * kOvReplicas * 512, h->stream));
  HIP_TRY(hipMemsetAsync(h->v.knn_done0, 0, sizeof(unsigned int) * ((size_t)h->S + 64), h->stream));
  h->chain_prev = false; h->chain_count = 0; h->chain_fix_pending = false; h->verdict_scan = -1; h->replay_enq_ns = 0.0; h->replay_wait_ns = 0.0; h->replay_timed = 0;
  std::memset(h->host_out, 0, sizeof(HostOut) * 2 * (size_t)h->S);
  std::fill(h->scans_enqueued.begin(), h->scans_enqueued.end(), 0);
  HIP_TRY(hipMemsetAsync(h->v.win_n, 0, sizeof(int) * (size_t)h->S * h->P, h->stream));
  HIP_TRY(hipStreamSynchronize(h->stream));
  return LIODOM_OK;
}

}

extern "C" {

const char* liodom_last_error(void) { return g_last_error.c_str(); }

void liodom_params_default(liodom_params_t* p) {
  if (!p) return;
  std::memset(p, 0, sizeof(*p));
  p->min_range = 3.0;
  p->max_range = 75.0;
  p->lidar_type = 0;
  p->scan_lines = 64;
  p->scan_regions = 8;
  p->edges_per_region = 10;
  p->min_points_per_scan = 8 * 10 + 10;
  p->local_map_size = 5;
  p->save_results = 0;
  std::strcpy(p->results_dir, "~/");
  std::strcpy(p->fixed_frame, "odom");
  std::strcpy(p->base_frame, "base_link");
  p->laser_frame[0] = 0;
  p->use_imu = 0; p->filter_local_map = 0; p->mapping = 0;
  p->publish_tf = 1;
}

void liodom_config_default(liodom_config_t* c) {
  if (!c) return;
  std::memset(c, 0, sizeof(*c));
  c->device = 0; c->n_streams = 1; c->max_points = 64 * 1800; c->max_width = 1800;
  c->reserved1 = 0; c->lm_apply_step_on_ftol = 0; c->pose_log_capacity = 1024; c->debug_buffers = 0;
  c->lm_workgroups = 0;
  c->pose_rotation_mode = 1;
}

int liodom_create(const liodom_params_t* params, const liodom_config_t* config, liodom_handle_t** out) {
  if (!params || !config || !out) return LIODOM_ERR_INVALID_ARG;
  *out = nullptr;
  if (params->scan_lines < 1 || params->scan_lines > 254 || params->scan_regions < 1 ||
      params->edges_per_region < 0 || params->local_map_size < 1 || params->local_map_size > (uint64_t)kMaxFrames ||
      config->n_streams < 1 || config->max_points < 1 || !(params->max_range > params->min_range)) {
    g_last_error = "liodom_create: parameter out of range";
    return LIODOM_ERR_INVALID_ARG;
  }
  int ndev = 0;
  if (hipGetDeviceCount(&ndev) != hipSuccess || ndev <= 0) {
    g_last_error = "no HIP device available (libliodom_hip has no CPU fallback)";
    return LIODOM_ERR_NO_DEVICE;
  }
  if (config->device < 0 || config->device >= ndev) { g_last_error = "bad device ordinal"; return LIODOM_ERR_INVALID_ARG; }
  HIP_TRY(hipSetDevice(config->device));
  liodom_handle* h = new liodom_handle();
  h->params = *params;
  h->config = *config;
  h->S = config->n_streams; h->H = params->scan_lines; h->P = (int)params->local_map_size;
  h->lockstep = config->n_streams >= 16;
  int rc = LIODOM_OK;
  auto fail = [&](int code) { liodom_destroy(h); return code; };
  int prio_least = 0, prio_greatest = 0;
  (void)hipDeviceGetStreamPriorityRange(&prio_least, &prio_greatest);
  const bool use_prio = prio_least != prio_greatest;
  auto make_stream = [&](hipStream_t* st, int prio) {
    return use_prio ? hipStreamCreateWithPriority(st, hipStreamNonBlocking, prio) : hipStreamCreateWithFlags(st, hipStreamNonBlocking);
  };
  if (make_stream(&h->stream, prio_greatest) != hipSuccess) { g_last_error = "hipStreamCreate failed"; return fail(LIODOM_ERR_HIP); }
  if (hipEventCreateWithFlags(&h->ev_ov, hipEventDisableTiming) != hipSuccess) { g_last_error = "hipEventCreate failed"; return fail(LIODOM_ERR_HIP); }
  if (hipEventCreateWithFlags(&h->pose_event, hipEventDisableTiming) != hipSuccess) { g_last_error = "hipEventCreate failed"; return fail(LIODOM_ERR_HIP); }
  const int prio_x = (prio_least - prio_greatest >= 2) ? prio_greatest + 1 : prio_least;
  if (make_stream(&h->stream_x, prio_x) != hipSuccess) { g_last_error = "hipStreamCreate failed"; return fail(LIODOM_ERR_HIP); }
  for (int b = 0; b < kEdgePipeBufs; b++) {
    if (hipEventCreateWithFlags(&h->ev_edges[b], hipEventDisableTiming) != hipSuccess ||
        hipEventCreateWithFlags(&h->ev_free[b], hipEventDisableTiming) != hipSuccess) { g_last_error = "hipEventCreate failed"; return fail(LIODOM_ERR_HIP); }
  }

  DevView& v = h->v;
  v.min_range = params->min_range; v.max_range = params->max_range;
  v.lidar_type = params->lidar_type; v.scan_lines = params->scan_lines;
  v.scan_regions = params->scan_regions; v.edges_per_region = params->edges_per_region;
  v.min_points_per_scan = (long long)params->min_points_per_scan;
  v.prev_frames = h->P;
  v.apply_on_ftol = config->lm_apply_step_on_ftol;
  v.rotation_mode = config->pose_rotation_mode != 0 ? 1 : 0;
  v.filter_local_map = (params->filter_local_map && !params->mapping) ? 1 : 0;
  h->lds_hash_build = h->lockstep;
  {
    int cus = 0;
    (void)hipDeviceGetAttribute(&cus, hipDeviceAttributeMultiprocessorCount, config->device);
    const int ecap = round_up(std::max(1, params->scan_lines * params->scan_regions * (params->edges_per_region + 1)), 64);
    h->use_flags = !h->lockstep;
    h->flag_gate = !(config->n_streams == 1 && cdiv(cdiv(ecap, 8), 2) * 4 <= cus * 12);
    for (const char* name : {"AMD_SERIALIZE_KERNEL", "HIP_LAUNCH_BLOCKING", "ROCPROFILER_PMC", "ROCPROF_COUNTERS"}) {
      const char* e = std::getenv(name);
      if (e && e[0] && std::strcmp(e, "0") != 0) h->use_flags = false;
    }
    if (env_int("LIODOM_PIPE_FLAGS", 1) == 0) h->use_flags = false;
  }
  if (const char* e = std::getenv("LIODOM_HASH_BUILD")) h->lds_hash_build = std::strcmp(e, "global") != 0;
  v.lds_cells_max = std::max(1, std::min(kLdsCellsMax, env_int("LIODOM_LDS_CELLS_MAX", kLdsCellsMax)));
  {
    const int ecap = params->scan_lines * params->scan_regions * (params->edges_per_region + 1);
    const int auto_g = config->n_streams > 4 ? 1 : (ecap >= 2048 ? kLmGroupsMax : (ecap >= 512 ? 4 : 1));
    v.lm_groups = config->lm_workgroups == 0 ? auto_g
                                             : (config->lm_workgroups >= kLmGroupsMax ? kLmGroupsMax : (config->lm_workgroups < 1 ? 1 : config->lm_workgroups));
  }
  v.vox_inv = 1.0f / 0.4f;
  v.n_streams = h->S;
  v.max_points = config->max_points;
  v.ring_cap = config->max_points;
  v.slots_per_ring = params->scan_regions * (params->edges_per_region + 1);
  h->ring_lds_bytes = ring_extract_lds_bytes(v.slots_per_ring, params->scan_regions);
  if (h->ring_lds_bytes > 160 * 1024) { g_last_error = "pick lists (scan_regions * (edges_per_region + 1)) exceed 160 KiB of LDS"; return fail(LIODOM_ERR_CAPACITY); }
  v.edge_cap = round_up(std::max(1, h->H * v.slots_per_ring), 64);
  v.use_imu = params->use_imu ? 1 : 0;
  iso_identity(v.laser_to_base);
  v.mapping = params->mapping ? 1 : 0;
  v.early_rebuild = (!h->lds_hash_build && !v.filter_local_map && !params->mapping && config->n_streams <= 4) ? 1 : 0;
  if (env_int("LIODOM_EARLY_REBUILD", 1) == 0) v.early_rebuild = 0;
  if (env_int("LIODOM_SAFE_MODE", 0) != 0) enter_safe_mode(h);
  v.recv_cap = v.mapping ? (config->recv_capacity > 0 ? config->recv_capacity : 262144) : 0;
  v.map_cap = v.edge_cap * h->P + v.recv_cap;
  int ts = 1024;
  while (ts < 2 * (v.map_cap + (v.early_rebuild ? 8 * v.edge_cap : 0))) ts <<= 1;
  v.table_size = ts;
  v.pose_log_cap = std::max(1, config->pose_log_capacity);
  v.debug = config->debug_buffers & 1;
  if (kInstrument) { const int dc = env_int("LIODOM_DEBUG_CLOCKS", 0); if (dc != 0) v.debug |= ((dc & (128 | 256)) ? (dc & 32) : 32) | (dc & (64 | 128)) | ((dc >> 8) << 8); }
  v.ring_id_stride = (size_t)round_up(config->max_points + 512, 256);

  const size_t S = (size_t)h->S;
#define ALLOC(ptr, count, fill) do { rc = dev_alloc(h, &(ptr), (count), (fill)); if (rc != LIODOM_OK) return fail(rc); } while (0)
  ALLOC(v.state, S, 0);
  ALLOC(v.ring_id, S * v.ring_id_stride, 0xFF);
  v.tile_cap = std::max(1, cdiv(config->max_points, kTilePts));
  ALLOC(v.tile_hist, S * (size_t)v.tile_cap * h->H, 0);
  h->ring_split_lb = h->lockstep && params->lidar_type == 0 && !h->safe_mode && env_int("LIODOM_RING_SPLIT_LB", 1) != 0;
  v.ring_pitch = round_up(cdiv((long long)config->max_points * 9, (long long)std::max(1, h->H) * 8), 8);
  if (const char* e = std::getenv("LIODOM_RING_PITCH")) v.ring_pitch = std::max(8, std::atoi(e));
  v.ring_stride = h->ring_split_lb ? std::max((size_t)config->max_points, (size_t)h->H * (size_t)v.ring_pitch) : (size_t)config->max_points;
  v.lb_hpad = round_up(h->H, 64);
  if (h->ring_split_lb) {
    ALLOC(v.lb_desc, S * (size_t)v.tile_cap * v.lb_hpad, 0); ALLOC(v.lb_ticket, 1, 0); ALLOC(v.lb_ovf, S, 0);
    const size_t lds = ring_split_lb_lds_bytes(h->H);
    if (lds > 48 * 1024 && (hipFuncSetAttribute(reinterpret_cast<const void*>(&k_ring_split_lb), hipFuncAttributeMaxDynamicSharedMemorySize, (int)lds) != hipSuccess ||
                            hipFuncSetAttribute(reinterpret_cast<const void*>(&k_ring_split_fix), hipFuncAttributeMaxDynamicSharedMemorySize, (int)lds) != hipSuccess)) {
      (void)hipGetLastError(); h->ring_split_lb = false;
    }
  } else { v.lb_desc = nullptr; v.lb_ticket = nullptr; v.lb_ovf = nullptr; }
  ALLOC(v.ring_pts, S * v.ring_stride + kExLPR * kExIPLBig + 64, 0);
  ALLOC(v.ring_src, S * v.ring_stride, 0);
  ALLOC(v.ring_start, S * (size_t)(h->H + 1), 0);
  ALLOC(v.ring_len, S * (size_t)h->H, 0);
  ALLOC(v.edges_pad, S * h->H * v.slots_per_ring, 0);
  ALLOC(v.edges_pad_meta, S * h->H * v.slots_per_ring, 0);
  ALLOC(v.ring_nedges, S * h->H, 0);
  {
    h->ring_split = env_int("LIODOM_RING_SPLIT", 1) != 0 && !h->safe_mode;
    if (h->ring_split) {
      int cus = 0, per_cu = 0;
      (void)hipDeviceGetAttribute(&cus, hipDeviceAttributeMultiprocessorCount, config->device);
      const size_t lds = ring_scatter_lds_bytes(h->H);
      if (lds > 48 * 1024 &&
          hipFuncSetAttribute(reinterpret_cast<const void*>(&k_ring_split), hipFuncAttributeMaxDynamicSharedMemorySize, (int)lds) != hipSuccess) {
        (void)hipGetLastError(); per_cu = 0;
      } else if (hipOccupancyMaxActiveBlocksPerMultiprocessor(&per_cu, reinterpret_cast<const void*>(&k_ring_split), kTileThreads, lds) != hipSuccess) {
        (void)hipGetLastError(); per_cu = 0;
      }
      long long budget = (long long)std::max(0, per_cu) * std::max(0, cus) / 2;
      if (budget > 256) budget = 256;
      h->ring_split_max_wgs = (int)budget;
      const int tiles_one = std::max(1, cdiv(config->max_points, kTilePts));
      if (tiles_one > h->ring_split_max_wgs) h->ring_split = false;
    }
    v.split_ctr = nullptr;
    v.split_hist = nullptr; v.split_pad = round_up(v.tile_cap, 8);
    if (h->ring_split) { ALLOC(v.split_ctr, 2 * S, 0); ALLOC(v.split_hist, S * (size_t)h->H * v.split_pad + 64, 0); }
  }
  ALLOC(v.ring_npoints, S * h->H, 0);
  ALLOC(v.ring_c, S * v.ring_stride, 0);
  ALLOC(v.ring_picked, S * v.ring_stride, 0);
  ALLOC(v.edges, kEdgeBufs * S * v.edge_cap, 0);
  ALLOC(v.edges_meta, kEdgeBufs * S * v.edge_cap, 0);
  ALLOC(v.corr_a, S * 2 * v.edge_cap, 0);
  ALLOC(v.corr_b, S * 2 * v.edge_cap, 0);
  ALLOC(v.corr_idx, S * 2 * v.edge_cap, 0xFF);
  if (v.debug & 1) ALLOC(v.knn_q, S * 2 * v.edge_cap, 0); else v.knn_q = nullptr;
  ALLOC(v.win_pts, S * h->P * v.edge_cap, 0);
  ALLOC(v.win_n, S * h->P, 0);
  ALLOC(v.win_base, S * (h->P + 1), 0);
  ALLOC(v.win_slot, S * h->P, 0);
  const size_t ntab = v.early_rebuild ? 2 : 1;
  ALLOC(v.cells, ntab * S * v.table_size, 0);
  ALLOC(v.pt_rank, S * v.map_cap, 0);
  ALLOC(v.cell_bits, ntab * S * (size_t)(v.table_size / 32), 0);
  v.used_cap = v.early_rebuild ? v.map_cap + 8 * v.edge_cap : v.map_cap;
  ALLOC(v.used_cells, ntab * S * (size_t)v.used_cap, 0);
  ALLOC(v.pt_cell, S * v.map_cap, 0xFF);
  if (v.recv_cap) ALLOC(v.recv_pts, S * v.recv_cap, 0);
  ALLOC(v.imu_q, S * 4, 0);
  v.ovf_base = v.early_rebuild ? v.map_cap + 8 * v.edge_cap : v.map_cap;
  v.sorted_cap = v.early_rebuild ? v.ovf_base + v.edge_cap : v.map_cap;
  const bool hash_incr_on = env_int("LIODOM_HASH_INCR", 1) != 0;
  if (hash_incr_on && h->lockstep && h->lds_hash_build && !params->mapping && !params->filter_local_map && !v.early_rebuild)
    v.sorted_cap = 2 * v.map_cap + 65536 + (kHbPeriod - 1) * v.edge_cap;
  ALLOC(v.sorted_pts, (v.early_rebuild ? 2 : 1) * S * (size_t)v.sorted_cap, 0);
  if (v.early_rebuild) ALLOC(v.cell_pad, 2 * S * (size_t)v.table_size, 0); else v.cell_pad = nullptr;
  v.rebuild_delta = 0.25f;
  if (const char* e = std::getenv("LIODOM_REBUILD_DELTA")) { const float d = (float)std::atof(e); if (d > 0.0f && d <= 0.45f) v.rebuild_delta = d; }
  if (v.filter_local_map) {
    ALLOC(v.vox_cells, S * v.table_size, 0);
    ALLOC(v.vox_fill, S * v.table_size, 0);
    ALLOC(v.vox_used_list, S * v.map_cap, 0);
    ALLOC(v.pt_vox, S * v.map_cap, 0xFF);
    ALLOC(v.vox_pts, S * v.map_cap, 0);
    ALLOC(v.filt_pts, S * v.map_cap, 0);
    ALLOC(v.filt_int, S * v.map_cap, 0);
  }
  ALLOC(v.pose_log, S * v.pose_log_cap * 7, 0);
  ALLOC(v.info_log, S * v.pose_log_cap, 0);
  ALLOC(h->stage_in, S * (size_t)config->max_points, 0);
  ALLOC(v.dbg_clk, 16 * 32, 0);
  if (v.debug & 32) ALLOC(v.dbg_q, 2 * (size_t)v.edge_cap * 12, 0); else v.dbg_q = nullptr;
  ALLOC(v.lm_xch, S * 2 * kLmGroupsMax * 64, 0);
  ALLOC(v.pose_xch, S * 64, 0);
  ALLOC(v.redo_sync, 64, 0);
  ALLOC(v.pipe_flags, kEdgePipeBufs + 1, 0);
  v.host_edges = nullptr; v.host_edges_meta = nullptr; v.host_edges_hdr = nullptr;
  if (S == 1) {
    const size_t ne = (size_t)kEdgePipeBufs * v.edge_cap;
    void *he = nullptr, *hm = nullptr, *hh = nullptr;
    if (hipHostMalloc(&he, sizeof(float4) * ne, hipHostMallocMapped | hipHostMallocCoherent) != hipSuccess ||
        hipHostMalloc(&hm, sizeof(int4) * ne, hipHostMallocMapped | hipHostMallocCoherent) != hipSuccess ||
        hipHostMalloc(&hh, sizeof(unsigned int) * 2 * kEdgePipeBufs, hipHostMallocMapped | hipHostMallocCoherent) != hipSuccess) {
      if (he) hipHostFree(he);
      if (hm) hipHostFree(hm);
      g_last_error = "hipHostMalloc (edge mirror) failed"; return fail(LIODOM_ERR_HIP);
    }
    h->host_edges = static_cast<float4*>(he); h->host_edges_meta = static_cast<int4*>(hm); h->host_edges_hdr = static_cast<unsigned int*>(hh);
    std::memset(hh, 0, sizeof(unsigned int) * 2 * kEdgePipeBufs);
    void *de = nullptr, *dm = nullptr, *dh = nullptr;
    if (hipHostGetDevicePointer(&de, he, 0) != hipSuccess || hipHostGetDevicePointer(&dm, hm, 0) != hipSuccess ||
        hipHostGetDevicePointer(&dh, hh, 0) != hipSuccess) { g_last_error = "hipHostGetDevicePointer failed"; return fail(LIODOM_ERR_HIP); }
    v.host_edges = static_cast<float4*>(de); v.host_edges_meta = static_cast<int4*>(dm); v.host_edges_hdr = static_cast<unsigned int*>(dh);
  }
  if (h->use_flags) {
    unsigned int* probe = nullptr;
    ALLOC(probe, 4, 0);
    hipLaunchKernelGGL(k_set_flag, dim3(1), dim3(1), 0, h->stream, probe + 2, 1u);
    hipLaunchKernelGGL(k_set_flag, dim3(1), dim3(1), 0, h->stream_x, probe + 3, 1u);
    if (hipStreamSynchronize(h->stream) != hipSuccess || hipStreamSynchronize(h->stream_x) != hipSuccess) { g_last_error = "stream probe failed"; return fail(LIODOM_ERR_HIP); }
    hipLaunchKernelGGL(k_probe_wait, dim3(1), dim3(64), 0, h->stream, probe, probe + 1);
    hipLaunchKernelGGL(k_set_flag, dim3(1), dim3(1), 0, h->stream_x, probe, 1u);
    unsigned int res = 0;
    if (hipStreamSynchronize(h->stream) != hipSuccess || hipStreamSynchronize(h->stream_x) != hipSuccess ||
        hipMemcpy(&res, probe + 1, sizeof(res), hipMemcpyDeviceToHost) != hipSuccess) { g_last_error = "stream probe failed"; return fail(LIODOM_ERR_HIP); }
    h->streams_concurrent = res == 1u;
    if (!h->streams_concurrent) h->use_flags = false;
  }
  if (h->lockstep) ALLOC(v.knn_nn, S * (size_t)v.edge_cap * 5, 0); else v.knn_nn = nullptr;
  h->knn8 = h->lockstep && env_int("LIODOM_KNN8", 1) != 0;
  h->knn8_grid = std::max(1, cdiv(cdiv(v.edge_cap, kKnn8Queries), kKnnGridDiv));
  v.hash_incr = (hash_incr_on && h->knn8 && h->lds_hash_build && !params->mapping && !params->filter_local_map && h->P > kHbPeriod &&
                 v.sorted_cap >= 2 * v.map_cap + (kHbPeriod - 1) * v.edge_cap) ? 1 : 0;
  v.hb_spill_base = v.sorted_cap - (kHbPeriod - 1) * v.edge_cap;
  if (v.hash_incr) ALLOC(v.cell_cap, S * (size_t)v.table_size, 0); else v.cell_cap = nullptr;
  v.hb_slack_min = kHbSlackMin; v.hb_new_room = kHbNewRoom;
  if (const char* e = std::getenv("LIODOM_HB_SLACK")) v.hb_slack_min = std::max(0, std::atoi(e));
  if (const char* e = std::getenv("LIODOM_HB_NEW_ROOM")) v.hb_new_room = std::max(1, std::atoi(e));
  if (h->knn8) { ALLOC(v.knn8_cnt, S, 0); ALLOC(v.knn8_list, S * (size_t)v.edge_cap, 0); } else { v.knn8_cnt = nullptr; v.knn8_list = nullptr; }
  v.knn_queries = h->lockstep ? 4 : 8;
  v.knn_partials = h->lockstep ? 0 : 1;
  v.knn_blocks = round_up(cdiv(v.edge_cap, v.knn_queries), 4);
  v.knn_grid = std::max(1, cdiv(v.knn_blocks, kKnnGridDiv));
  {
    const int save = env_int("LIODOM_KNN_SAVE", 2);
    if (save >= 1) ALLOC(v.knn_save_q, S * (size_t)v.edge_cap, 0); else v.knn_save_q = nullptr;
    if (save >= 2) { ALLOC(v.knn_save_pos, S * (size_t)v.edge_cap * kKnnGroup, 0xFF); ALLOC(v.knn_save_g, S * (size_t)v.edge_cap, 0); }
    else { v.knn_save_pos = nullptr; v.knn_save_g = nullptr; }
  }
  v.knn_exact_only = env_int("LIODOM_KNN_EXACT_ONLY", 0) != 0 ? 1 : 0;
  ALLOC(v.knn_part, S * 2 * (size_t)v.knn_blocks * 32, 0);
  ALLOC(v.ov_flags, S, 0);
  ALLOC(v.pose_xch0, S * (size_t)kOvReplicas * 512, 0);
  ALLOC(v.knn_done, S * (size_t)v.knn_grid, 0);
  ALLOC(v.knn_done0, S + 64, 0);
  if (v.early_rebuild) ALLOC(v.pred_xch, S * (size_t)kOvReplicas * 512, 0); else v.pred_xch = nullptr;
  ALLOC(v.edge_cnt, (size_t)kEdgeBufs * 32, 0);
  ALLOC(v.pub_counter, (size_t)kEdgeBufs, 0);
  if (v.early_rebuild) ALLOC(v.edges_keep, S * (size_t)v.edge_cap, 0); else v.edges_keep = nullptr;
  v.mask_stride = round_up(v.knn_blocks, 128);
  ALLOC(v.corr_mask, S * 2 * (size_t)v.mask_stride, 0);
  {
    void* hp = nullptr;
    if (hipHostMalloc(&hp, sizeof(HostOut) * 2 * S, hipHostMallocMapped | hipHostMallocCoherent) != hipSuccess) { g_last_error = "hipHostMalloc failed"; return fail(LIODOM_ERR_HIP); }
    h->host_out = static_cast<HostOut*>(hp);
    std::memset(hp, 0, sizeof(HostOut) * 2 * S);
    void* dp = nullptr;
    if (hipHostGetDevicePointer(&dp, hp, 0) != hipSuccess) { g_last_error = "hipHostGetDevicePointer failed"; return fail(LIODOM_ERR_HIP); }
    v.host_out = static_cast<HostOut*>(dp);
    h->scans_enqueued.assign(S, 0);
    h->mappers.assign(S, nullptr); h->mapper_cells_xy.assign(S, 2); h->mapper_cells_z.assign(S, 1);
  }
  if (ring_scatter_lds_bytes(h->H) > 48 * 1024) {
    if (hipFuncSetAttribute(reinterpret_cast<const void*>(&k_ring_scatter), hipFuncAttributeMaxDynamicSharedMemorySize,
                            (int)ring_scatter_lds_bytes(h->H)) != hipSuccess) {
      g_last_error = "hipFuncSetAttribute(max dynamic LDS) failed"; return fail(LIODOM_ERR_HIP);
    }
  }
  if (hipFuncSetAttribute(reinterpret_cast<const void*>(&k_hash_build), hipFuncAttributeMaxDynamicSharedMemorySize,
                          (int)hash_build_lds_bytes()) != hipSuccess) {
    g_last_error = "hipFuncSetAttribute(max dynamic LDS) failed"; return fail(LIODOM_ERR_HIP);
  }
  v.lm_lds_reduce = lm_lds_reduce_fits(v.edge_cap) ? 1 : 0;
  if (lm_lds_bytes(v.edge_cap) + 8192 > 160 * 1024) { g_last_error = "liodom_create: edge capacity too large for the solve's LDS tile"; return fail(LIODOM_ERR_INVALID_ARG); }
  if (hipFuncSetAttribute(reinterpret_cast<const void*>(&k_lm_solve<0, false>), hipFuncAttributeMaxDynamicSharedMemorySize, (int)lm_lds_bytes(h->v.edge_cap)) != hipSuccess ||
      hipFuncSetAttribute(reinterpret_cast<const void*>(&k_lm_solve<1, false>), hipFuncAttributeMaxDynamicSharedMemorySize, (int)lm_lds_bytes(h->v.edge_cap)) != hipSuccess ||
      hipFuncSetAttribute(reinterpret_cast<const void*>(&k_lm_solve<0, true>), hipFuncAttributeMaxDynamicSharedMemorySize, (int)lm_lds_bytes(h->v.edge_cap)) != hipSuccess ||
      hipFuncSetAttribute(reinterpret_cast<const void*>(&k_lm_solve<1, true>), hipFuncAttributeMaxDynamicSharedMemorySize, (int)lm_lds_bytes(h->v.edge_cap)) != hipSuccess) {
    g_last_error = "hipFuncSetAttribute(max dynamic LDS) failed"; return fail(LIODOM_ERR_HIP);
  }
  if (h->ring_lds_bytes > 48 * 1024) {
    if (hipFuncSetAttribute(reinterpret_cast<const void*>(&k_ring_extract<256, kExIPL>), hipFuncAttributeMaxDynamicSharedMemorySize, (int)h->ring_lds_bytes) != hipSuccess ||
        hipFuncSetAttribute(reinterpret_cast<const void*>(&k_ring_extract<256, kExIPLBig>), hipFuncAttributeMaxDynamicSharedMemorySize, (int)h->ring_lds_bytes) != hipSuccess ||
        hipFuncSetAttribute(reinterpret_cast<const void*>(&k_ring_extract<1024, kExIPL>), hipFuncAttributeMaxDynamicSharedMemorySize, (int)h->ring_lds_bytes) != hipSuccess ||
        hipFuncSetAttribute(reinterpret_cast<const void*>(&k_ring_extract<1024, kExIPLBig>), hipFuncAttributeMaxDynamicSharedMemorySize, (int)h->ring_lds_bytes) != hipSuccess) {
      g_last_error = "hipFuncSetAttribute(max dynamic LDS) failed"; return fail(LIODOM_ERR_HIP);
    }
  }
  {
    int cus = 0;
    (void)hipDeviceGetAttribute(&cus, hipDeviceAttributeMultiprocessorCount, config->device);
    const int knn_overlap = env_int("LIODOM_KNN_OVERLAP", 1);
    h->ov_ok = knn_overlap != 0 && v.early_rebuild && S == 1 && v.knn_partials && (knn_overlap == 2 || (long long)v.knn_grid * 4 * 3 <= (long long)cus * 24);
    h->chain_ok = v.early_rebuild && S == 1 && v.knn_partials && !v.use_imu && (long long)v.knn_grid * 4 * 2 <= (long long)cus * 24;
    if (knn_overlap == 0 || env_int("LIODOM_CHAIN", 1) == 0) h->chain_ok = false;
    v.speculate = (h->ov_ok || h->chain_ok) ? 1 : 0;
    if (v.speculate) v.speculate = std::max(0, std::min(7, env_int("LIODOM_SPECULATE", 1)));
    v.spec_backoff = 16;
    v.spec_theta = 0.8;
    if (const char* e = std::getenv("LIODOM_SPEC_THETA")) v.spec_theta = std::atof(e);
    if ((h->ov_ok || h->chain_ok) && make_stream(&h->stream_k, prio_greatest) != hipSuccess) { g_last_error = "hipStreamCreate failed"; return fail(LIODOM_ERR_HIP); }
    if (h->chain_ok && hipEventCreateWithFlags(&h->ev_ch, hipEventDisableTiming) != hipSuccess) { g_last_error = "hipEventCreate failed"; return fail(LIODOM_ERR_HIP); }
  }
  {
    double ms = 50.0;
    if (const char* e = std::getenv("LIODOM_WAIT_MS")) { const double x = std::atof(e); if (x >= 1.0 && x <= 10000.0) ms = x; }
    const unsigned long long ticks = (unsigned long long)(ms * 1.0e5);
    if (hipMemcpyToSymbol(HIP_SYMBOL(g_wait_ticks), &ticks, sizeof(ticks)) != hipSuccess) { g_last_error = "hipMemcpyToSymbol(g_wait_ticks) failed"; return fail(LIODOM_ERR_HIP); }
  }
  ALLOC(h->d_view, 1, 0);
  if (hipMemcpy(h->d_view, &h->v, sizeof(DevView), hipMemcpyHostToDevice) != hipSuccess) { g_last_error = "DevView upload failed"; return fail(LIODOM_ERR_HIP); }
  rc = reset_state(h);
  if (rc != LIODOM_OK) return fail(rc);
  g_live_handles.fetch_add(1);
  h->counted_live = true;
  *out = h;
  return LIODOM_OK;
#undef ALLOC
}

void liodom_destroy(liodom_handle_t* h) {
  if (!h) return;
  if (h->counted_live) g_live_handles.fetch_sub(1);
  if (h->stream_x) hipStreamSynchronize(h->stream_x);
  if (h->stream) hipStreamSynchronize(h->stream);
  if (h->stream_k) { hipStreamSynchronize(h->stream_k); hipStreamDestroy(h->stream_k); }
  if (h->ev_ov) hipEventDestroy(h->ev_ov);
  if (h->ev_ch) hipEventDestroy(h->ev_ch);
  for (liodom_map* mp : h->mappers) {
    if (!mp) continue;
    mp->stream = nullptr; mp->own_stream = false;
    if (hipStreamCreateWithFlags(&mp->stream, hipStreamNonBlocking) == hipSuccess) mp->own_stream = true;
  }
  for (void* p : h->allocs) hipFree(p);
  if (h->resident) hipFree(h->resident);
  if (h->host_out) hipHostFree(h->host_out);
  if (h->host_edges) hipHostFree(h->host_edges);
  if (h->host_edges_meta) hipHostFree(h->host_edges_meta);
  if (h->host_edges_hdr) hipHostFree(h->host_edges_hdr);
  if (h->pin_ring) hipHostFree(h->pin_ring);
  for (int b = 0; b < kEdgePipeBufs; b++) { if (h->ev_pin[b]) hipEventDestroy(h->ev_pin[b]); }
  for (auto& e : h->ev_pool) { hipEventDestroy(e.a); hipEventDestroy(e.b); }
  if (h->pose_event) hipEventDestroy(h->pose_event);
  for (int b = 0; b < kEdgePipeBufs; b++) { if (h->ev_edges[b]) hipEventDestroy(h->ev_edges[b]); if (h->ev_free[b]) hipEventDestroy(h->ev_free[b]); }
  if (h->stream_c && !h->stream_c_shared) { hipStreamSynchronize(h->stream_c); hipStreamDestroy(h->stream_c); }
  for (int b = 0; b < 3; b++) { if (h->ev_up[b]) hipEventDestroy(h->ev_up[b]); if (h->ev_xdone[b]) hipEventDestroy(h->ev_xdone[b]); }
  if (h->stream_x) hipStreamDestroy(h->stream_x);
  if (h->stream) hipStreamDestroy(h->stream);
  delete h;
}

int liodom_reset(liodom_handle_t* h) {
  int rc = enter(h);
  if (rc) return rc;
  SideLocks lk(h, true, true);
  return reset_state(h);
}

static int copy_edges_out(liodom_handle_t* h, int stream, int eb, hipStream_t q, float* edges_xyzi, int32_t* edge_ring,
                          int32_t* edge_idx, int32_t* edge_src, int cap, int* n_edges) {
  int E = 0;
  HIP_TRY(hipMemcpyAsync(&E, &h->v.state[stream].n_edges_buf[eb], sizeof(int), hipMemcpyDeviceToHost, q));
  HIP_TRY(hipStreamSynchronize(q));
  if (n_edges) *n_edges = E;
  if (E > cap) { g_last_error = "edge buffer too small"; return LIODOM_ERR_CAPACITY; }
  if (E == 0) return LIODOM_OK;
  if (edges_xyzi)
    HIP_TRY(hipMemcpyAsync(edges_xyzi, h->v.edges + ((size_t)eb * h->S + stream) * h->v.edge_cap, sizeof(float4) * (size_t)E, hipMemcpyDeviceToHost, q));
  std::vector<int4> meta;
  if (edge_ring || edge_idx || edge_src) {
    meta.resize((size_t)E);
    HIP_TRY(hipMemcpyAsync(meta.data(), h->v.edges_meta + ((size_t)eb * h->S + stream) * h->v.edge_cap, sizeof(int4) * (size_t)E, hipMemcpyDeviceToHost, q));
  }
  HIP_TRY(hipStreamSynchronize(q));
  for (int i = 0; i < E && !meta.empty(); i++) {
    if (edge_ring) edge_ring[i] = meta[i].x;
    if (edge_idx) edge_idx[i] = meta[i].y;
    if (edge_src) edge_src[i] = meta[i].z;
  }
  return LIODOM_OK;
}

int liodom_extract_edges(liodom_handle_t* h, int stream, const float* xyzi, int64_t n, int height,
                         int width, float* edges_xyzi, int32_t* edge_ring, int32_t* edge_idx,
                         int32_t* edge_src, int cap, int* n_edges) {
  int rc = check_stream(h, stream);
  if (rc) return rc;
  if ((rc = check_usable(h))) return rc;
  if (n < 0 || n > h->v.max_points || (n > 0 && !xyzi)) { g_last_error = "bad point count"; return LIODOM_ERR_CAPACITY; }
  SideLocks lk(h, false, true);
  hipStream_t q = extract_queue(h);
  float4* in = h->stage_in + (size_t)stream * h->v.max_points;
  if (n) HIP_TRY(hipMemcpyAsync(in, xyzi, sizeof(float4) * (size_t)n, hipMemcpyHostToDevice, q));
  rc = launch_extract(h, q, kEdgeBufX, stream, 1, in, 0, (int)n, height, width);
  if (rc) return rc;
  return copy_edges_out(h, stream, kEdgeBufX, q, edges_xyzi, edge_ring, edge_idx, edge_src, cap, n_edges);
}

int liodom_get_edges(liodom_handle_t* h, int stream, float* edges_xyzi, int32_t* edge_ring,
                     int32_t* edge_idx, int32_t* edge_src, int cap, int* n_edges) {
  int rc = check_stream(h, stream);
  if (rc) return rc;
  SideLocks lk(h, true, false);
  return copy_edges_out(h, stream, h->last_eb, h->stream, edges_xyzi, edge_ring, edge_idx, edge_src, cap, n_edges);
}

static int wait_pose(liodom_handle_t* h, int s0, int count, double* pose_out, liodom_step_info_t* info, int lag = 0) {
  bool timed_out = false;
  for (int i = 0; i < count; i++) {
    const int expect = h->scans_enqueued[s0 + i] - lag;
    volatile HostOut* ho = h->host_out + (size_t)(s0 + i) * 2 + ((expect - 1) & 1);
    unsigned long long spins = 0;
    while (__atomic_load_n(&ho->seq, __ATOMIC_ACQUIRE) != expect) {
      if ((++spins & 0xFFFFull) == 0) {
        const hipError_t q = hipStreamQuery(h->stream);
        if (q != hipErrorNotReady && q != hipSuccess) { g_last_error = std::string("stream error while waiting: ") + hipGetErrorString(q); return LIODOM_ERR_HIP; }
        if (q == hipSuccess && __atomic_load_n(&ho->seq, __ATOMIC_ACQUIRE) != expect) { g_last_error = "stream drained without publishing the scan result"; return LIODOM_ERR_HIP; }
      }
    }
    const HostOut* r = h->host_out + (size_t)(s0 + i) * 2 + ((expect - 1) & 1);
    if (pose_out) std::memcpy(pose_out + 7 * i, r->pose, sizeof(double) * 7);
    if (info) info[i] = r->info;
    if (r->info.status & (LIODOM_STATUS_PIPE_TIMEOUT | LIODOM_STATUS_LM_SYNC_TIMEOUT)) timed_out = true;
    if (s0 + i == 0) { h->verdict_scan = expect; h->verdict_confirmed = r->pad == 1; }
  }
  if (timed_out) {
    h->fallback_pending.store(true);
    g_last_error = "a kernel timed out waiting for another kernel of the handle (LIODOM_STATUS_PIPE_TIMEOUT / LM_SYNC_TIMEOUT): kernels are "
                   "serialised across streams (profiler with --pmc, AMD_SERIALIZE_KERNEL, debugger) or the GPU is saturated by another "
                   "process; the scan's result is invalid; call liodom_reset(): the handle then continues in safe mode (no in-kernel waits)";
    return LIODOM_ERR_HIP;
  }
  return LIODOM_OK;
}

int liodom_odometry_step(liodom_handle_t* h, int stream, const float* edges_xyzi, int n_edges,
                         double stamp, double* pose_out, liodom_step_info_t* info) {
  (void)stamp;
  int rc = check_stream(h, stream);
  if (rc) return rc;
  if ((rc = check_usable(h))) return rc;
  if (n_edges < 0 || n_edges > h->v.edge_cap || (n_edges > 0 && !edges_xyzi)) { g_last_error = "edge count exceeds capacity"; return LIODOM_ERR_CAPACITY; }
  SideLocks lk(h, true, false);
  if ((rc = tickets_idle(h))) return rc;
  rc = drain_pipeline(h);
  if (rc) return rc;
  if (n_edges)
    HIP_TRY(hipMemcpyAsync(h->v.edges + (size_t)stream * h->v.edge_cap, edges_xyzi, sizeof(float4) * (size_t)n_edges, hipMemcpyHostToDevice, h->stream));
  {
    ProfScope ps(h, KID_OTHER);
    hipLaunchKernelGGL(k_set_edges, dim3(1), dim3(64), 0, h->stream, h->v, stream, n_edges, 0);
  }
  rc = launch_odometry(h, 0, stream, 1);
  if (rc) return rc;
  return wait_pose(h, stream, 1, pose_out, info);
}

static int ensure_pin_ring(liodom_handle* h) {
  if (h->pin_ring) return LIODOM_OK;
  void* p = nullptr;
  HIP_TRY(hipHostMalloc(&p, sizeof(float4) * (size_t)kEdgePipeBufs * (size_t)h->v.max_points, hipHostMallocDefault));
  h->pin_ring = static_cast<float4*>(p);
  for (int b = 0; b < kEdgePipeBufs; b++) HIP_TRY(hipEventCreateWithFlags(&h->ev_pin[b], hipEventDisableTiming));
  return LIODOM_OK;
}

int liodom_scan_buffer(liodom_handle_t* h, int stream, float** xyzi, int64_t* capacity_points) {
  int rc = check_stream(h, stream);
  if (rc) return rc;
  if (!xyzi) return LIODOM_ERR_INVALID_ARG;
  if (h->S != 1) { g_last_error = "liodom_scan_buffer: one-stream handles only"; return LIODOM_ERR_UNSUPPORTED; }
  SideLocks lk(h, false, true);
  if ((rc = ensure_pin_ring(h))) return rc;
  const int r = h->pin_next;
  if (h->ev_pin_valid[r]) { HIP_TRY(hipEventSynchronize(h->ev_pin[r])); h->ev_pin_valid[r] = false; }
  *xyzi = reinterpret_cast<float*>(h->pin_ring + (size_t)r * h->v.max_points);
  if (capacity_points) *capacity_points = h->v.max_points;
  return LIODOM_OK;
}

int liodom_extract_edges_device(liodom_handle_t* h, int stream, const float* xyzi, int64_t n, int height, int width,
                                liodom_edge_ticket_t* ticket) {
  int rc = check_stream(h, stream);
  if (rc) return rc;
  if ((rc = check_usable(h))) return rc;
  if (!ticket) return LIODOM_ERR_INVALID_ARG;
  if (h->S != 1) { g_last_error = "liodom_extract_edges_device: one-stream handles only (lock-step handles advance all streams together: liodom_process_resident)"; return LIODOM_ERR_UNSUPPORTED; }
  if (n < 0 || n > h->v.max_points || (n > 0 && !xyzi)) { g_last_error = "bad point count"; return LIODOM_ERR_CAPACITY; }
  SideLocks lk(h, false, true);
  if (h->pf_slot >= 0) { g_last_error = "liodom_extract_edges_device: a pipelined replay of this handle has an extraction issued ahead: call liodom_sync() first"; return LIODOM_ERR_NEEDS_SYNC; }
  if (h->replay_live.load()) { g_last_error = "liodom_extract_edges_device: scans of a pipelined replay (liodom_process_resident / liodom_replay_*) are still in the edge buffers: call liodom_sync() first"; return LIODOM_ERR_NEEDS_SYNC; }
  const int eb = h->x_next;
  if (h->tk_seq[eb].load() != 0u) {
    g_last_error = "liodom_extract_edges_device: all hand-off slots hold edge clouds no liodom_odometry_step_device has taken yet";
    return LIODOM_ERR_BUSY;
  }
  hipStream_t q = extract_queue(h);
  float4* in = h->stage_in + (size_t)stream * h->v.max_points;
  if (n) {
    if ((rc = ensure_pin_ring(h))) return rc;
    const char* lo = reinterpret_cast<const char*>(h->pin_ring);
    const char* hi = lo + sizeof(float4) * (size_t)kEdgePipeBufs * (size_t)h->v.max_points;
    const char* src = reinterpret_cast<const char*>(xyzi);
    bool own = src >= lo && src < hi, pinned = own;
    if (!own) {
      hipPointerAttribute_t attr;
      if (hipPointerGetAttributes(&attr, xyzi) == hipSuccess) pinned = attr.type == hipMemoryTypeHost;
      else (void)hipGetLastError();
    }
    const int r = own ? (int)((src - lo) / (sizeof(float4) * (size_t)h->v.max_points)) : h->pin_next;
    if (!pinned) {
      if (h->ev_pin_valid[r]) { HIP_TRY(hipEventSynchronize(h->ev_pin[r])); h->ev_pin_valid[r] = false; }
      std::memcpy(h->pin_ring + (size_t)r * h->v.max_points, xyzi, sizeof(float4) * (size_t)n);
      xyzi = reinterpret_cast<const float*>(h->pin_ring + (size_t)r * h->v.max_points);
    }
    HIP_TRY(hipMemcpyAsync(in, xyzi, sizeof(float4) * (size_t)n, hipMemcpyHostToDevice, q));
    if (own || !pinned) {
      HIP_TRY(hipEventRecord(h->ev_pin[r], q));
      h->ev_pin_valid[r] = true;
      h->pin_next = (r + 1) % kEdgePipeBufs;
    }
  }
  unsigned int seq = ++h->ext_seq;
  if (seq == 0u) seq = ++h->ext_seq;
  unsigned int* host_seq = h->v.host_edges_hdr ? h->v.host_edges_hdr + eb : nullptr;
  unsigned int* const dev_flag = h->use_flags ? h->v.pipe_flags + eb : (unsigned int*)nullptr;
  rc = launch_extract(h, q, eb, stream, 1, in, 0, (int)n, height, width, 0u, 1, dev_flag, host_seq, seq);
  if (rc) return rc;
  if (!h->use_flags) HIP_TRY(hipEventRecord(h->ev_edges[eb], q));
  h->eb_seq[eb] = seq;
  h->pipe_active.store(true);
  h->tk_seq[eb].store(seq);
  h->x_next = (eb + 1) % kEdgePipeBufs;
  ticket->seq = seq; ticket->slot = eb; ticket->stream = stream; ticket->reserved = 0;
  return LIODOM_OK;
}

int liodom_wait_edges(liodom_handle_t* h, const liodom_edge_ticket_t* ticket, float* edges_xyzi, int32_t* edge_ring,
                      int32_t* edge_idx, int32_t* edge_src, int cap, int* n_edges) {
  if (!h || !ticket) return LIODOM_ERR_INVALID_ARG;
  int rc = check_stream(h, ticket->stream);
  if (rc) return rc;
  const int eb = ticket->slot;
  if (eb < 0 || eb >= kEdgePipeBufs || !h->host_edges_hdr) { g_last_error = "liodom_wait_edges: bad ticket"; return LIODOM_ERR_INVALID_ARG; }
  volatile unsigned int* hs = h->host_edges_hdr + eb;
  unsigned long long spins = 0;
  while ((int)(__atomic_load_n(hs, __ATOMIC_ACQUIRE) - ticket->seq) < 0) {
    if ((++spins & 0xFFFFull) == 0) {
      const hipError_t q = hipStreamQuery(extract_queue(h));
      if (q != hipErrorNotReady && q != hipSuccess) { g_last_error = std::string("stream error while waiting for edges: ") + hipGetErrorString(q); return LIODOM_ERR_HIP; }
      if (q == hipSuccess && (int)(__atomic_load_n(hs, __ATOMIC_ACQUIRE) - ticket->seq) < 0) { g_last_error = "extraction stream drained without publishing the ticket's edges"; return LIODOM_ERR_HIP; }
    }
  }
  if (__atomic_load_n(hs, __ATOMIC_ACQUIRE) != ticket->seq) { g_last_error = "liodom_wait_edges: the ticket's slot has been reused (stale ticket)"; return LIODOM_ERR_INVALID_ARG; }
  const int E = (int)h->host_edges_hdr[kEdgePipeBufs + eb];
  if (n_edges) *n_edges = E;
  if (E > cap && (edges_xyzi || edge_ring || edge_idx || edge_src)) { g_last_error = "edge buffer too small"; return LIODOM_ERR_CAPACITY; }
  const float4* he = h->host_edges + (size_t)eb * h->v.edge_cap;
  const int4* hm = h->host_edges_meta + (size_t)eb * h->v.edge_cap;
  if (edges_xyzi && E) std::memcpy(edges_xyzi, he, sizeof(float4) * (size_t)E);
  if (edge_ring || edge_idx || edge_src) {
    for (int i = 0; i < E; i++) {
      if (edge_ring) edge_ring[i] = hm[i].x;
      if (edge_idx) edge_idx[i] = hm[i].y;
      if (edge_src) edge_src[i] = hm[i].z;
    }
  }
  return LIODOM_OK;
}

int liodom_odometry_submit_device(liodom_handle_t* h, const liodom_edge_ticket_t* ticket, double stamp) {
  (void)stamp;
  if (!h || !ticket) return LIODOM_ERR_INVALID_ARG;
  int rc = check_stream(h, ticket->stream);
  if (rc) return rc;
  if ((rc = check_usable(h))) return rc;
  const int eb = ticket->slot;
  if (h->S != 1 || eb < 0 || eb >= kEdgePipeBufs) { g_last_error = "liodom_odometry_submit_device: bad ticket"; return LIODOM_ERR_INVALID_ARG; }
  SideLocks lk(h, true, false);
  if (ticket->seq == 0u || h->tk_seq[eb].load() != ticket->seq) {
    g_last_error = "liodom_odometry_submit_device: stale or unknown ticket (already consumed, or voided by liodom_reset)";
    return LIODOM_ERR_INVALID_ARG;
  }
  for (int i = 0; i < h->odo_pending; i++) if (h->odo_fifo[i] == eb) { g_last_error = "liodom_odometry_submit_device: ticket already submitted"; return LIODOM_ERR_INVALID_ARG; }
  if (h->odo_pending >= 2) { g_last_error = "liodom_odometry_submit_device: two scans are in flight: collect a pose first (liodom_odometry_collect)"; return LIODOM_ERR_BUSY; }
  rc = enqueue_pipeline_odometry(h, eb, ticket->seq);
  if (rc) return rc;
  h->pipe_active.store(true);
  h->odo_fifo[h->odo_pending++] = eb;
  return LIODOM_OK;
}

int liodom_odometry_collect(liodom_handle_t* h, int stream, double* pose_out, liodom_step_info_t* info) {
  int rc = check_stream(h, stream);
  if (rc) return rc;
  SideLocks lk(h, true, false);
  if (h->odo_pending <= 0) { g_last_error = "liodom_odometry_collect: no scan has been submitted"; return LIODOM_ERR_INVALID_ARG; }
  rc = wait_pose(h, stream, 1, pose_out, info, h->odo_pending - 1);
  const int eb = h->odo_fifo[0];
  h->odo_fifo[0] = h->odo_fifo[1];
  h->odo_pending--;
  h->tk_seq[eb].store(0u);
  return rc;
}

int liodom_odometry_step_device(liodom_handle_t* h, const liodom_edge_ticket_t* ticket, double stamp, double* pose_out,
                                liodom_step_info_t* info) {
  if (!h || !ticket) return LIODOM_ERR_INVALID_ARG;
  if (h->odo_pending != 0) { g_last_error = "liodom_odometry_step_device: a submitted scan has not been collected (liodom_odometry_collect)"; return LIODOM_ERR_BUSY; }
  const int rc = liodom_odometry_submit_device(h, ticket, stamp);
  if (rc) return rc;
  return liodom_odometry_collect(h, ticket->stream, pose_out, info);
}

int liodom_process_scan(liodom_handle_t* h, int stream, const float* xyzi, int64_t n, int height,
                        int width, double stamp, double* pose_out, liodom_step_info_t* info) {
  (void)stamp;
  int rc = check_stream(h, stream);
  if (rc) return rc;
  if ((rc = check_usable(h))) return rc;
  if (n < 0 || n > h->v.max_points || (n > 0 && !xyzi)) { g_last_error = "bad point count"; return LIODOM_ERR_CAPACITY; }
  SideLocks lk(h, true, true);
  if ((rc = tickets_idle(h))) return rc;
  rc = drain_pipeline(h);
  if (rc) return rc;
  float4* in = h->stage_in + (size_t)stream * h->v.max_points;
  if (n) HIP_TRY(hipMemcpyAsync(in, xyzi, sizeof(float4) * (size_t)n, hipMemcpyHostToDevice, h->stream));
  rc = launch_extract(h, h->stream, 0, stream, 1, in, 0, (int)n, height, width);
  if (rc) return rc;
  rc = launch_odometry(h, 0, stream, 1);
  if (rc) return rc;
  return wait_pose(h, stream, 1, pose_out, info);
}

static int rebuild_search_structure(liodom_handle* h, int stream) {
  const DevView& v = h->v;
  const int map_blocks = cdiv(v.map_cap, 256);
  hipLaunchKernelGGL(k_hash_reset, dim3(64), dim3(256), 0, h->stream, v, stream);
  hipLaunchKernelGGL(k_hash_reset_done, dim3(1), dim3(1), 0, h->stream, v, stream);
  if (h->lds_hash_build) {
    hipLaunchKernelGGL(k_hash_build, dim3(1), dim3(kBuildThreads), hash_build_lds_bytes(), h->stream, v, stream, -1);
  } else {
    hipLaunchKernelGGL(k_window_insert, dim3(map_blocks, 1), dim3(256), 0, h->stream, v, stream, -1);
    hipLaunchKernelGGL(k_hash_alloc, dim3(map_blocks, 1), dim3(256), 0, h->stream, v, stream);
    hipLaunchKernelGGL(k_hash_scatter, dim3(map_blocks, 1), dim3(256), 0, h->stream, v, stream);
  }
  HIP_TRY(hipGetLastError());
  return LIODOM_OK;
}

int liodom_set_received_map(liodom_handle_t* h, int stream, const float* xyzi, int64_t n) {
  int rc = check_stream(h, stream);
  if (rc) return rc;
  if (!h->v.mapping) { g_last_error = "liodom_set_received_map: the handle was created with mapping = 0"; return LIODOM_ERR_UNSUPPORTED; }
  if (n < 0 || (n > 0 && !xyzi)) return LIODOM_ERR_INVALID_ARG;
  if (n > h->v.recv_cap) { g_last_error = "liodom_set_received_map: cloud larger than recv_capacity"; return LIODOM_ERR_CAPACITY; }
  SideLocks lk(h, true, false);
  const int ni = (int)n;
  if (n) HIP_TRY(hipMemcpyAsync(h->v.recv_pts + (size_t)stream * h->v.recv_cap, xyzi, sizeof(float4) * (size_t)n, hipMemcpyHostToDevice, h->stream));
  HIP_TRY(hipMemcpyAsync(&h->v.state[stream].n_recv, &ni, sizeof(int), hipMemcpyHostToDevice, h->stream));
  rc = rebuild_search_structure(h, stream);
  if (rc) return rc;
  HIP_TRY(sync_odometry(h));
  return LIODOM_OK;
}

int liodom_set_imu_orientation(liodom_handle_t* h, int stream, const double* q_xyzw) {
  int rc = check_stream(h, stream);
  if (rc) return rc;
  if (!q_xyzw) return LIODOM_ERR_INVALID_ARG;
  SideLocks lk(h, true, false);
  HIP_TRY(hipMemcpyAsync(h->v.imu_q + (size_t)stream * 4, q_xyzw, sizeof(double) * 4, hipMemcpyHostToDevice, h->stream));
  return LIODOM_OK;
}

int liodom_set_laser_to_base(liodom_handle_t* h, const double* T) {
  if (!h || !T) return LIODOM_ERR_INVALID_ARG;
  if (int rc = enter(h)) return rc;
  SideLocks lk(h, true, true);
  for (int k = 0; k < 12; k++) h->v.laser_to_base[k] = T[k];
  return LIODOM_OK;
}

int liodom_get_received_map(liodom_handle_t* h, int stream, float* xyzi, int64_t cap, int64_t* n_points) {
  int rc = check_stream(h, stream);
  if (rc) return rc;
  if (!h->v.mapping) { if (n_points) *n_points = 0; return LIODOM_OK; }
  SideLocks lk(h, true, false);
  HIP_TRY(sync_odometry(h));
  int n = 0;
  HIP_TRY(hipMemcpy(&n, &h->v.state[stream].n_recv, sizeof(int), hipMemcpyDeviceToHost));
  if (n_points) *n_points = n;
  if (n > cap) { g_last_error = "received-map buffer too small"; return LIODOM_ERR_CAPACITY; }
  if (n && xyzi) HIP_TRY(hipMemcpy(xyzi, h->v.recv_pts + (size_t)stream * h->v.recv_cap, sizeof(float4) * (size_t)n, hipMemcpyDeviceToHost));
  return LIODOM_OK;
}

int liodom_attach_mapper(liodom_handle_t* h, int stream, liodom_map_t* m, int cells_xy, int cells_z) {
  int rc = check_stream(h, stream);
  if (rc) return rc;
  if (!h->v.mapping) { g_last_error = "liodom_attach_mapper: the handle was created with mapping = 0"; return LIODOM_ERR_UNSUPPORTED; }
  SideLocks lk(h, true, false);
  HIP_TRY(sync_odometry(h));
  if (liodom_map* old = h->mappers[stream]) {
    h->mappers[stream] = nullptr;
    old->stream = nullptr; old->own_stream = false;
    HIP_TRY(hipStreamCreateWithFlags(&old->stream, hipStreamNonBlocking));
    old->own_stream = true;
  }
  if (!m) return LIODOM_OK;
  if (m->device != h->config.device) { g_last_error = "liodom_attach_mapper: map and handle live on different devices"; return LIODOM_ERR_INVALID_ARG; }
  if (cells_xy < 0 || cells_z < 0) return LIODOM_ERR_INVALID_ARG;
  HIP_TRY(hipStreamSynchronize(m->stream));
  if (m->own_stream) { (void)hipStreamDestroy(m->stream); m->own_stream = false; }
  m->stream = h->stream;
  h->mappers[stream] = m;
  h->mapper_cells_xy[stream] = cells_xy;
  h->mapper_cells_z[stream] = cells_z;
  return LIODOM_OK;
}

int liodom_alloc_resident(liodom_handle_t* h, int n_slots) {
  if (!h || n_slots < 1) return LIODOM_ERR_INVALID_ARG;
  int rc0 = enter(h);
  if (rc0) return rc0;
  SideLocks lk(h, true, true);
  HIP_TRY(hipStreamSynchronize(h->stream_x));
  HIP_TRY(sync_odometry(h));
  h->pf_slot = -1;
  if (h->resident) { hipFree(h->resident); h->resident = nullptr; h->n_slots = 0; }
  const size_t bytes = sizeof(float4) * (size_t)h->S * (size_t)n_slots * (size_t)h->v.max_points;
  void* raw = nullptr;
  HIP_TRY(hipMalloc(&raw, bytes));
  h->resident = static_cast<float4*>(raw);
  h->n_slots = n_slots;
  return LIODOM_OK;
}

int liodom_upload_scan(liodom_handle_t* h, int stream, int slot, const float* xyzi, int64_t n) {
  int rc = check_stream(h, stream);
  if (rc) return rc;
  if (!h->resident || slot < 0 || slot >= h->n_slots || n < 0 || n > h->v.max_points) { g_last_error = "bad resident slot"; return LIODOM_ERR_INVALID_ARG; }
  SideLocks lk(h, false, true);
  float4* dst = h->resident + ((size_t)slot * h->S + stream) * (size_t)h->v.max_points;
  if (n) HIP_TRY(hipMemcpy(dst, xyzi, sizeof(float4) * (size_t)n, hipMemcpyHostToDevice));
  return LIODOM_OK;
}

int liodom_process_resident(liodom_handle_t* h, int slot, int64_t n, int height, int width,
                            double* poses_out, liodom_step_info_t* infos_out) {
  return liodom_process_resident_pipelined(h, slot, -1, n, height, width, poses_out, infos_out);
}

static int replay_one(liodom_handle_t* h, int slot, int next_slot, int64_t n, int height, int width, bool wait,
                      double* poses_out, liodom_step_info_t* infos_out, const float* next_host = nullptr, int64_t host_stride = 0);

int liodom_process_resident_pipelined(liodom_handle_t* h, int slot, int next_slot, int64_t n, int height,
                                      int width, double* poses_out, liodom_step_info_t* infos_out) {
  int rc0 = enter(h);
  if (rc0) return rc0;
  if ((rc0 = check_usable(h))) return rc0;
  SideLocks lk(h, true, true);
  if ((rc0 = tickets_idle(h))) return rc0;
  return replay_one(h, slot, next_slot, n, height, width, poses_out != nullptr || infos_out != nullptr, poses_out, infos_out);
}

int liodom_replay_resident(liodom_handle_t* h, int first_slot, int count, int ahead, int depth, int64_t n, int height, int width,
                           double* poses_out, liodom_step_info_t* infos_out) {
  int rc0 = enter(h);
  if (rc0) return rc0;
  if ((rc0 = check_usable(h))) return rc0;
  if (count < 0 || first_slot < 0 || depth < 0 || depth > 1) { g_last_error = "bad resident range / depth"; return LIODOM_ERR_INVALID_ARG; }
  SideLocks lk(h, true, true);
  if ((rc0 = tickets_idle(h))) return rc0;
  auto out_p = [&](int i) { return poses_out ? poses_out + (size_t)i * h->S * 7 : nullptr; };
  auto out_i = [&](int i) { return infos_out ? infos_out + (size_t)i * h->S : nullptr; };
  const auto t_call = std::chrono::steady_clock::now();
  h->replay_stamps.clear();
  h->replay_stamps.reserve((size_t)count);
  auto stamp = [&]() { h->replay_stamps.push_back(std::chrono::duration<double, std::micro>(std::chrono::steady_clock::now() - t_call).count()); };
  for (int i = 0; i < count; i++) {
    const int slot = first_slot + i;
    const int next = (i + 1 < count || ahead) ? slot + 1 : -1;
    if (depth == 0) {
      const int rc = replay_one(h, slot, next, n, height, width, true, out_p(i), out_i(i));
      if (rc) return rc;
      continue;
    }
    const auto t_a = std::chrono::steady_clock::now();
    int rc = replay_one(h, slot, next, n, height, width, false, nullptr, nullptr);
    if (rc) return rc;
    const auto t_b = std::chrono::steady_clock::now();
    if (i > 0) { rc = wait_pose(h, 0, h->S, out_p(i - 1), out_i(i - 1), 1); if (rc) return rc; stamp(); }
    h->replay_enq_ns += std::chrono::duration<double, std::nano>(t_b - t_a).count();
    h->replay_wait_ns += std::chrono::duration<double, std::nano>(std::chrono::steady_clock::now() - t_b).count();
    h->replay_timed++;
  }
  if (depth == 1 && count > 0) { const int rc = wait_pose(h, 0, h->S, out_p(count - 1), out_i(count - 1), 0); if (rc) return rc; stamp(); }
  return LIODOM_OK;
}

static int upload_slot_async(liodom_handle_t* h, int slot, const float* host, int64_t stride, int64_t n) {
  const int r = slot % 3;
  if (!h->stream_c) {
    if (h->stream_k) { h->stream_c = h->stream_k; h->stream_c_shared = true; }
    else HIP_TRY(hipStreamCreateWithFlags(&h->stream_c, hipStreamNonBlocking));
  }
  if (!h->ev_up[0]) {
    for (int b = 0; b < 3; b++) {
      HIP_TRY(hipEventCreateWithFlags(&h->ev_up[b], hipEventDisableTiming));
      HIP_TRY(hipEventCreateWithFlags(&h->ev_xdone[b], hipEventDisableTiming));
    }
  }
  hipStream_t q = extract_queue(h);
  if (h->ev_xdone_valid[r]) HIP_TRY(hipStreamWaitEvent(h->stream_c, h->ev_xdone[r], 0));
  for (int s = 0; s < h->S && n > 0; s++) {
    float4* dst = h->resident + ((size_t)slot * h->S + s) * (size_t)h->v.max_points;
    HIP_TRY(hipMemcpyAsync(dst, host + (size_t)s * (size_t)stride, sizeof(float4) * (size_t)n, hipMemcpyHostToDevice, h->stream_c));
  }
  HIP_TRY(hipEventRecord(h->ev_up[r], h->stream_c));
  HIP_TRY(hipStreamWaitEvent(q, h->ev_up[r], 0));
  return LIODOM_OK;
}
static int upload_slot_consumed(liodom_handle_t* h, int slot) {
  const int r = slot % 3;
  HIP_TRY(hipEventRecord(h->ev_xdone[r], extract_queue(h)));
  h->ev_xdone_valid[r] = true;
  return LIODOM_OK;
}

static int replay_one(liodom_handle_t* h, int slot, int next_slot, int64_t n, int height, int width, bool wait,
                      double* poses_out, liodom_step_info_t* infos_out, const float* next_host, int64_t host_stride) {
  if (!h->resident || slot < 0 || slot >= h->n_slots || next_slot >= h->n_slots || n < 0 || n > h->v.max_points) {
    g_last_error = "bad resident slot"; return LIODOM_ERR_INVALID_ARG;
  }
  h->replay_live.store(true);
  const int eb = h->parity;
  int rc;
  if (h->pf_slot != slot) {
    rc = issue_extract(h, slot, eb, (int)n, height, width);
    if (rc) return rc;
  }
  h->pf_slot = -1;
  rc = enqueue_pipeline_odometry(h, eb, h->eb_seq[eb]);
  if (rc) return rc;
  h->parity = (eb + 1) % kEdgePipeBufs;
  if (next_slot >= 0) {
    if (next_host) { rc = upload_slot_async(h, next_slot, next_host, host_stride, n); if (rc) return rc; }
    rc = issue_extract(h, next_slot, h->parity, (int)n, height, width);
    if (rc) return rc;
    if (next_host) { rc = upload_slot_consumed(h, next_slot); if (rc) return rc; }
    h->pf_slot = next_slot;
  }
  if (wait) return wait_pose(h, 0, h->S, poses_out, infos_out);
  return LIODOM_OK;
}

int liodom_replay_host(liodom_handle_t* h, const float* xyzi_base, int64_t scan_stride_floats, int count, int depth,
                       int64_t n, int height, int width, double* poses_out, liodom_step_info_t* infos_out) {
  int rc0 = enter(h);
  if (rc0) return rc0;
  if ((rc0 = check_usable(h))) return rc0;
  if (count < 0 || depth < 0 || depth > 1 || n < 0 || n > h->v.max_points || (count > 0 && n > 0 && !xyzi_base) || scan_stride_floats < 4 * n) {
    g_last_error = "liodom_replay_host: bad arguments"; return LIODOM_ERR_INVALID_ARG;
  }
  constexpr int kRing = 3;
  if (h->n_slots < kRing) { const int rc = liodom_alloc_resident(h, kRing); if (rc) return rc; }
  SideLocks lk(h, true, true);
  int rc = tickets_idle(h);
  if (rc) return rc;
  rc = drain_pipeline(h);
  if (rc) return rc;
  struct Suppress { liodom_handle* h; ~Suppress() { h->ov_suppress = false; } } suppress{h};
  h->ov_suppress = true;
  auto out_p = [&](int i) { return poses_out ? poses_out + (size_t)i * h->S * 7 : nullptr; };
  auto out_i = [&](int i) { return infos_out ? infos_out + (size_t)i * h->S : nullptr; };
  auto src = [&](int i) { return xyzi_base + (size_t)i * (size_t)h->S * (size_t)scan_stride_floats; };
  for (int i = 0; i < count; i++) {
    const int slot = i % kRing, next = (i + 1 < count) ? (i + 1) % kRing : -1;
    if (i == 0) {
      rc = upload_slot_async(h, slot, src(0), scan_stride_floats, n);
      if (rc) return rc;
      rc = issue_extract(h, slot, h->parity, (int)n, height, width);
      if (rc) return rc;
      h->pf_slot = slot;
      rc = upload_slot_consumed(h, slot);
      if (rc) return rc;
    }
    const float* nh = next >= 0 ? src(i + 1) : nullptr;
    if (depth == 0) {
      rc = replay_one(h, slot, next, n, height, width, true, out_p(i), out_i(i), nh, scan_stride_floats);
      if (rc) return rc;
      continue;
    }
    rc = replay_one(h, slot, next, n, height, width, false, nullptr, nullptr, nh, scan_stride_floats);
    if (rc) return rc;
    if (i > 0) { rc = wait_pose(h, 0, h->S, out_p(i - 1), out_i(i - 1), 1); if (rc) return rc; }
  }
  if (depth == 1 && count > 0) { rc = wait_pose(h, 0, h->S, out_p(count - 1), out_i(count - 1), 0); if (rc) return rc; }
  if (h->stream_c) HIP_TRY(hipStreamSynchronize(h->stream_c));
  for (int b = 0; b < 3; b++) h->ev_xdone_valid[b] = false;
  return drain_pipeline(h);
}

int liodom_pin_host_buffer(void* p, int64_t bytes) {
  if (!p || bytes <= 0) return LIODOM_ERR_INVALID_ARG;
  HIP_TRY(hipHostRegister(p, (size_t)bytes, hipHostRegisterDefault));
  return LIODOM_OK;
}
int liodom_unpin_host_buffer(void* p) {
  if (!p) return LIODOM_ERR_INVALID_ARG;
  HIP_TRY(hipHostUnregister(p));
  return LIODOM_OK;
}

int liodom_sync(liodom_handle_t* h) {
  int rc0 = enter(h);
  if (rc0) return rc0;
  SideLocks lk(h, true, true);
  HIP_TRY(hipStreamSynchronize(h->stream_x));
  HIP_TRY(sync_odometry(h));
  if (h->stream_k) HIP_TRY(hipStreamSynchronize(h->stream_k));
  if (h->pf_slot < 0) return drain_pipeline(h);
  return LIODOM_OK;
}

int liodom_get_pose_log(liodom_handle_t* h, int stream, int first, int count, double* poses_out,
                        liodom_step_info_t* infos_out) {
  int rc = check_stream(h, stream);
  if (rc) return rc;
  if (first < 0 || count < 0 || first + count > h->v.pose_log_cap) { g_last_error = "pose log range"; return LIODOM_ERR_INVALID_ARG; }
  SideLocks lk(h, true, false);
  HIP_TRY(sync_odometry(h));
  if (poses_out && count)
    HIP_TRY(hipMemcpy(poses_out, h->v.pose_log + ((size_t)stream * h->v.pose_log_cap + first) * 7, sizeof(double) * 7 * (size_t)count, hipMemcpyDeviceToHost));
  if (infos_out && count)
    HIP_TRY(hipMemcpy(infos_out, h->v.info_log + (size_t)stream * h->v.pose_log_cap + first, sizeof(liodom_step_info_t) * (size_t)count, hipMemcpyDeviceToHost));
  return LIODOM_OK;
}

static int get_window_impl(liodom_handle_t* h, int stream, float* xyzi, int64_t cap, int64_t* n_points, int* n_frames) {
  HIP_TRY(sync_odometry(h));
  StreamState st;
  HIP_TRY(hipMemcpy(&st, h->v.state + stream, sizeof(st), hipMemcpyDeviceToHost));
  const int P = h->P;
  std::vector<int> base((size_t)P + 1), slot((size_t)P);
  HIP_TRY(hipMemcpy(base.data(), h->v.win_base + (size_t)stream * (P + 1), sizeof(int) * (P + 1), hipMemcpyDeviceToHost));
  HIP_TRY(hipMemcpy(slot.data(), h->v.win_slot + (size_t)stream * P, sizeof(int) * P, hipMemcpyDeviceToHost));
  if (n_points) *n_points = st.n_map;
  if (n_frames) *n_frames = st.n_frames;
  if (st.n_map > cap) { g_last_error = "window buffer too small"; return LIODOM_ERR_CAPACITY; }
  for (int j = 0; j < st.n_frames && xyzi; j++) {
    const int cnt = base[j + 1] - base[j];
    if (cnt > 0)
      HIP_TRY(hipMemcpy(xyzi + 4 * (size_t)base[j], h->v.win_pts + ((size_t)stream * P + slot[j]) * h->v.edge_cap,
                        sizeof(float4) * (size_t)cnt, hipMemcpyDeviceToHost));
  }
  return LIODOM_OK;
}

int liodom_get_window(liodom_handle_t* h, int stream, float* xyzi, int64_t cap, int64_t* n_points, int* n_frames) {
  int rc = check_stream(h, stream);
  if (rc) return rc;
  SideLocks lk(h, true, false);
  return get_window_impl(h, stream, xyzi, cap, n_points, n_frames);
}

int liodom_get_local_map(liodom_handle_t* h, int stream, float* xyzi, int64_t cap, int64_t* n_points, int* filtered) {
  int rc = check_stream(h, stream);
  if (rc) return rc;
  SideLocks lk(h, true, false);
  HIP_TRY(sync_odometry(h));
  StreamState st;
  HIP_TRY(hipMemcpy(&st, h->v.state + stream, sizeof(st), hipMemcpyDeviceToHost));
  if (filtered) *filtered = st.n_filt > 0 ? 1 : 0;
  if (st.n_filt == 0) {
    int nf = 0;
    int64_t nw = 0;
    rc = get_window_impl(h, stream, xyzi, cap, &nw, &nf);
    const int nr = h->v.mapping ? st.n_recv : 0;
    if (n_points) *n_points = nw + nr;
    if (rc) return rc;
    if (nw + nr > cap) { g_last_error = "local-map buffer too small"; return LIODOM_ERR_CAPACITY; }
    if (nr && xyzi) HIP_TRY(hipMemcpy(xyzi + 4 * (size_t)nw, h->v.recv_pts + (size_t)stream * h->v.recv_cap, sizeof(float4) * (size_t)nr, hipMemcpyDeviceToHost));
    return LIODOM_OK;
  }
  const int n = st.n_filt;
  if (n_points) *n_points = n;
  if (n > cap) { g_last_error = "local-map buffer too small"; return LIODOM_ERR_CAPACITY; }
  std::vector<float4> pts((size_t)n);
  std::vector<float> inten((size_t)n);
  HIP_TRY(hipMemcpy(pts.data(), h->v.filt_pts + (size_t)stream * h->v.map_cap, sizeof(float4) * (size_t)n, hipMemcpyDeviceToHost));
  HIP_TRY(hipMemcpy(inten.data(), h->v.filt_int + (size_t)stream * h->v.map_cap, sizeof(float) * (size_t)n, hipMemcpyDeviceToHost));
  std::vector<int> order((size_t)n);
  for (int i = 0; i < n; i++) order[i] = i;
  auto leaf = [&](int i) { unsigned int u; std::memcpy(&u, &pts[i].w, 4); return u; };
  std::sort(order.begin(), order.end(), [&](int a, int b) { return leaf(a) < leaf(b); });
  for (int i = 0; i < n && xyzi; i++) {
    const float4& p = pts[order[i]];
    xyzi[4 * i] = p.x; xyzi[4 * i + 1] = p.y; xyzi[4 * i + 2] = p.z; xyzi[4 * i + 3] = inten[order[i]];
  }
  return LIODOM_OK;
}

int liodom_get_correspondences(liodom_handle_t* h, int stream, int it, int32_t* valid, int32_t* idx_a,
                               int32_t* idx_b, int cap, int* n) {
  int rc = check_stream(h, stream);
  if (rc) return rc;
  if (it < 0 || it > 1) return LIODOM_ERR_INVALID_ARG;
  SideLocks lk(h, true, false);
  HIP_TRY(sync_odometry(h));
  StreamState st;
  HIP_TRY(hipMemcpy(&st, h->v.state + stream, sizeof(st), hipMemcpyDeviceToHost));
  const int E = st.n_edges_buf[h->last_eb];
  if (n) *n = E;
  if (E > cap) { g_last_error = "correspondence buffer too small"; return LIODOM_ERR_CAPACITY; }
  std::vector<int2> ci((size_t)std::max(E, 1));
  if (E) HIP_TRY(hipMemcpy(ci.data(), h->v.corr_idx + ((size_t)stream * 2 + it) * h->v.edge_cap, sizeof(int2) * (size_t)E, hipMemcpyDeviceToHost));
  for (int i = 0; i < E; i++) {
    if (valid) valid[i] = ci[i].x >= 0 ? 1 : 0;
    if (idx_a) idx_a[i] = ci[i].x;
    if (idx_b) idx_b[i] = ci[i].y;
  }
  return LIODOM_OK;
}

int liodom_get_knn_queries(liodom_handle_t* h, int stream, int it, float* xyz0, int cap, int* n) {
  int rc = check_stream(h, stream);
  if (rc) return rc;
  if (it < 0 || it > 1) return LIODOM_ERR_INVALID_ARG;
  if (!h->v.knn_q) { g_last_error = "create the handle with debug_buffers = 1"; return LIODOM_ERR_UNSUPPORTED; }
  SideLocks lk(h, true, false);
  HIP_TRY(sync_odometry(h));
  int E = 0;
  HIP_TRY(hipMemcpy(&E, &h->v.state[stream].n_edges_buf[h->last_eb], sizeof(int), hipMemcpyDeviceToHost));
  if (n) *n = E;
  if (E > cap) { g_last_error = "query buffer too small"; return LIODOM_ERR_CAPACITY; }
  if (E && xyz0) HIP_TRY(hipMemcpy(xyz0, h->v.knn_q + ((size_t)stream * 2 + it) * h->v.edge_cap, sizeof(float4) * (size_t)E, hipMemcpyDeviceToHost));
  return LIODOM_OK;
}

int liodom_get_curvature(liodom_handle_t* h, int stream, double* curv, int64_t cap, int32_t* ring_offsets) {
  int rc = check_stream(h, stream);
  if (rc) return rc;
  if (!(h->v.debug & 1)) { g_last_error = "create the handle with debug_buffers = 1"; return LIODOM_ERR_UNSUPPORTED; }
  SideLocks lk(h, true, true);
  HIP_TRY(hipStreamSynchronize(h->stream_x));
  HIP_TRY(sync_odometry(h));
  std::vector<int> rs((size_t)h->H + 1), rl((size_t)h->H);
  HIP_TRY(hipMemcpy(rs.data(), h->v.ring_start + (size_t)stream * (h->H + 1), sizeof(int) * (h->H + 1), hipMemcpyDeviceToHost));
  HIP_TRY(hipMemcpy(rl.data(), h->v.ring_len + (size_t)stream * h->H, sizeof(int) * h->H, hipMemcpyDeviceToHost));
  int64_t off = 0;
  for (int r = 0; r < h->H; r++) { if (ring_offsets) ring_offsets[r] = (int32_t)off; off += rl[r]; }
  if (ring_offsets) ring_offsets[h->H] = (int32_t)off;
  if (off > cap) { g_last_error = "curvature buffer too small"; return LIODOM_ERR_CAPACITY; }
  int64_t o = 0;
  for (int r = 0; r < h->H && curv; r++) {
    if (rl[r]) HIP_TRY(hipMemcpy(curv + o, h->v.ring_c + (size_t)stream * h->v.ring_stride + rs[r], sizeof(double) * (size_t)rl[r], hipMemcpyDeviceToHost));
    o += rl[r];
  }
  return LIODOM_OK;
}

int liodom_set_profiling(liodom_handle_t* h, int enable) {
  int rc = enter(h);
  if (rc) return rc;
  std::unique_lock<std::mutex> lo(h->mx_o), lx(h->mx_x);
  rc = drain_events(h);
  h->profiling = enable != 0;
  return rc;
}

int liodom_get_kernel_stats(liodom_handle_t* h, liodom_kernel_stat_t* stats) {
  if (!h || !stats) return LIODOM_ERR_INVALID_ARG;
  int rc = enter(h);
  if (rc) return rc;
  SideLocks lk(h, true, true);
  rc = drain_events(h);
  if (rc) return rc;
  for (int i = 0; i < LIODOM_NUM_KERNELS; i++) {
    std::memset(&stats[i], 0, sizeof(stats[i]));
    std::strncpy(stats[i].name, kKernelNames[i], sizeof(stats[i].name) - 1);
    stats[i].launches = h->k_count[i];
    stats[i].total_ms = h->k_ms[i];
  }
  return LIODOM_OK;
}

int liodom_reset_kernel_stats(liodom_handle_t* h) {
  int rc = enter(h);
  if (rc) return rc;
  SideLocks lk(h, true, true);
  rc = drain_events(h);
  for (int i = 0; i < LIODOM_NUM_KERNELS; i++) { h->k_ms[i] = 0; h->k_count[i] = 0; }
  return rc;
}

int liodom_debug_set_inject_seed(liodom_handle_t* h, unsigned int seed) {
#if defined(LIODOM_INJECT_DELAY)
  if (!h) return LIODOM_ERR_INVALID_ARG;
  if (int rc = enter(h)) return rc;
  SideLocks lk(h, true, true);
  HIP_TRY(hipStreamSynchronize(h->stream_x));
  HIP_TRY(sync_odometry(h));
  HIP_TRY(hipMemcpyToSymbol(HIP_SYMBOL(g_inject_seed), &seed, sizeof(seed)));
  return LIODOM_OK;
#else
  (void)h; (void)seed;
  g_last_error = "liodom_debug_set_inject_seed: the product library carries no delay injection; build a variant with -DLIODOM_INJECT_DELAY (tools/variant_build.sh)";
  return LIODOM_ERR_UNSUPPORTED;
#endif
}

int liodom_debug_replay_stamps(liodom_handle_t* h, double* out_us, int cap) {
  if (!h || !out_us || cap < 0) return LIODOM_ERR_INVALID_ARG;
  const int n = (int)std::min<size_t>(h->replay_stamps.size(), (size_t)cap);
  for (int i = 0; i < n; i++) out_us[i] = h->replay_stamps[(size_t)i];
  return n;
}
int liodom_debug_clocks(liodom_handle_t* h, unsigned long long* out512) {
  if (!h || !out512) return LIODOM_ERR_INVALID_ARG;
  if (!kInstrument) { g_last_error = "liodom_debug_clocks: the product library carries no instrumentation; build a variant with -DLIODOM_INSTRUMENT (tools/variant_build.sh)"; return LIODOM_ERR_UNSUPPORTED; }
  if (int rc = enter(h)) return rc;
  SideLocks lk(h, true, true);
  HIP_TRY(hipStreamSynchronize(h->stream_x));
  HIP_TRY(sync_odometry(h));
  HIP_TRY(hipMemcpy(out512, h->v.dbg_clk, sizeof(unsigned long long) * 512, hipMemcpyDeviceToHost));
  return LIODOM_OK;
}

int liodom_debug_knn_times(liodom_handle_t* h, unsigned int* out, int* cap) {
  if (!h || !cap) return LIODOM_ERR_INVALID_ARG;
  *cap = h->v.edge_cap;
  if (!out) return LIODOM_OK;
  if (!h->v.dbg_q) return LIODOM_ERR_UNSUPPORTED;
  if (int rc = enter(h)) return rc;
  SideLocks lk(h, true, true);
  HIP_TRY(hipStreamSynchronize(h->stream_x));
  HIP_TRY(sync_odometry(h));
  HIP_TRY(hipMemcpy(out, h->v.dbg_q, sizeof(unsigned int) * 2 * (size_t)h->v.edge_cap * 12, hipMemcpyDeviceToHost));
  return LIODOM_OK;
}

int liodom_get_modes(liodom_handle_t* h, char* buf, int cap) {
  if (!h || !buf || cap < 2) return LIODOM_ERR_INVALID_ARG;
  if (int rc = enter(h)) return rc;
  SideLocks lk(h, true, true);
  const DevView& v = h->v;
  const OverlapModes om = overlap_modes(h);
  int spec[4] = {0, 0, 0, 0}, hbs[4] = {0, 0, 0, 0};
  unsigned int done_cnt[64] = {0};
  if (v.knn_done0) (void)hipMemcpy(done_cnt, v.knn_done0, sizeof(done_cnt), hipMemcpyDeviceToHost);
  (void)hipMemcpy(spec, reinterpret_cast<const char*>(v.state) + offsetof(StreamState, spec_stats), sizeof(spec), hipMemcpyDeviceToHost);
  (void)hipMemcpy(hbs, reinterpret_cast<const char*>(v.state) + offsetof(StreamState, hb_stats), sizeof(hbs), hipMemcpyDeviceToHost);
  snprintf(buf, (size_t)cap,
           "n_streams=%d early_rebuild=%d hash_build=%s pipe_flags=%d flag_gate=%d lm_groups=%d knn_instance=%d knn_queries=%d "
           "knn_grid=%d/%d knn8=%d hash_incr=%d hash_rebuilds=%d hash_appends=%d hash_appends_spilled=%d hash_points_spilled=%d knn_partials=%d knn_saved_bound=%d knn_exact_only=%d line_gate_kernel=%d filter_local_map=%d mapping=%d "
           "rotation_mode=%d table_size=%d rebuild_delta=%.3f knn_overlap=%d streams_concurrent=%d safe_mode=%d ring_split=%d ring_split_max_wgs=%d ring_split_lb=%d chain=%d speculate=%d spec_early=%d/%d spec_unconfirmed=%d/%d chain_done=%u/%u/%u replay_enqueue_us=%.2f replay_wait_us=%.2f debug=%d",
           h->S, v.early_rebuild, v.early_rebuild ? "streamed" : (h->lds_hash_build ? "lds" : "global"), h->use_flags ? 1 : 0,
           (h->use_flags && h->flag_gate) ? 1 : 0, v.lm_groups, h->lockstep ? 128 : 256, v.knn_queries, v.knn_grid,
           v.knn_blocks, h->knn8 ? 1 : 0, v.hash_incr, hbs[0], hbs[1], hbs[2], hbs[3], v.knn_partials, v.knn_save_pos ? 2 : (v.knn_save_q ? 1 : 0), v.knn_exact_only, v.knn_nn ? 1 : 0, v.filter_local_map, v.mapping,
           v.rotation_mode, v.table_size, (double)v.rebuild_delta,
           (om.ov || om.chain) ? 1 : 0, h->streams_concurrent ? 1 : 0, h->safe_mode ? 1 : 0, h->ring_split ? 1 : 0, h->ring_split ? h->ring_split_max_wgs : 0, h->ring_split_lb ? 1 : 0,
           om.chain ? 1 : 0, v.speculate, spec[0], spec[2], spec[1], spec[3], h->chain_count, done_cnt[0], done_cnt[32],
           h->replay_timed ? h->replay_enq_ns / (1e3 * (double)h->replay_timed) : 0.0, h->replay_timed ? h->replay_wait_ns / (1e3 * (double)h->replay_timed) : 0.0, v.debug);
  return LIODOM_OK;
}

int liodom_device_count(int* count) {
  if (!count) return LIODOM_ERR_INVALID_ARG;
  int n = 0;
  if (hipGetDeviceCount(&n) != hipSuccess) n = 0;
  *count = n;
  return LIODOM_OK;
}

int liodom_device_pci_bus_id(int device, char* bus_id, int cap) {
  if (!bus_id || cap < 16) return LIODOM_ERR_INVALID_ARG;
  HIP_TRY(hipDeviceGetPCIBusId(bus_id, cap, device));
  return LIODOM_OK;
}

int liodom_device_info(liodom_handle_t* h, char* name, int name_cap, int* compute_units) {
  if (!h) return LIODOM_ERR_INVALID_ARG;
  hipDeviceProp_t prop;
  HIP_TRY(hipGetDeviceProperties(&prop, h->config.device));
  if (name && name_cap > 0) {
    const char* nm = prop.name[0] ? prop.name : prop.gcnArchName;
    std::strncpy(name, nm, (size_t)name_cap - 1); name[name_cap - 1] = 0;
  }
  if (compute_units) *compute_units = prop.multiProcessorCount;
  return LIODOM_OK;
}

}
```

liodom_amd/csrc/wave_ops.h:

```cpp
#pragma once
#include <hip/hip_runtime.h>

namespace liodom_dev {

constexpr int DPP_XOR1 = 0xB1;
constexpr int DPP_XOR2 = 0x4E;
constexpr int DPP_HALF_MIRROR = 0x141;
constexpr int DPP_MIRROR = 0x140;
constexpr int DPP_ROW_SHR1 = 0x111, DPP_ROW_SHR2 = 0x112, DPP_ROW_SHR4 = 0x114, DPP_ROW_SHR8 = 0x118;
constexpr int DPP_ROW_BCAST15 = 0x142, DPP_ROW_BCAST31 = 0x143;

template <int CTRL>
__device__ __forceinline__ int dpp_i32(int v) {
  return __builtin_amdgcn_update_dpp(0, v, CTRL, 0xF, 0xF, true);
}
template <int CTRL>
__device__ __forceinline__ unsigned long long dpp_u64(unsigned long long v) {
  const int lo = dpp_i32<CTRL>((int)(unsigned int)v);
  const int hi = dpp_i32<CTRL>((int)(unsigned int)(v >> 32));
  return ((unsigned long long)(unsigned int)hi << 32) | (unsigned int)lo;
}
template <int CTRL>
__device__ __forceinline__ double dpp_f64(double v) {
  return __longlong_as_double((long long)dpp_u64<CTRL>((unsigned long long)__double_as_longlong(v)));
}

__device__ __forceinline__ int xor16_i32(int v) {
  const auto r = __builtin_amdgcn_permlane16_swap((unsigned int)v, (unsigned int)v, false, false);
  const int a = (int)r[0], b = (int)r[1];
  return (a != v) ? a : b;
}
__device__ __forceinline__ int xor32_i32(int v) {
  const auto r = __builtin_amdgcn_permlane32_swap((unsigned int)v, (unsigned int)v, false, false);
  const int a = (int)r[0], b = (int)r[1];
  return (a != v) ? a : b;
}
__device__ __forceinline__ unsigned long long xor16_u64(unsigned long long v) {
  const unsigned int lo = (unsigned int)xor16_i32((int)(unsigned int)v);
  const unsigned int hi = (unsigned int)xor16_i32((int)(unsigned int)(v >> 32));
  return ((unsigned long long)hi << 32) | lo;
}
__device__ __forceinline__ unsigned long long xor32_u64(unsigned long long v) {
  const unsigned int lo = (unsigned int)xor32_i32((int)(unsigned int)v);
  const unsigned int hi = (unsigned int)xor32_i32((int)(unsigned int)(v >> 32));
  return ((unsigned long long)hi << 32) | lo;
}

__device__ __forceinline__ unsigned long long row_max_u64(unsigned long long v) {
  unsigned long long o;
  o = dpp_u64<DPP_XOR1>(v); v = o > v ? o : v;
  o = dpp_u64<DPP_XOR2>(v); v = o > v ? o : v;
  o = dpp_u64<DPP_HALF_MIRROR>(v); v = o > v ? o : v;
  o = dpp_u64<DPP_MIRROR>(v); v = o > v ? o : v;
  return v;
}
__device__ __forceinline__ unsigned long long wave_max_u64(unsigned long long v) {
  v = row_max_u64(v);
  unsigned long long o = xor16_u64(v); v = o > v ? o : v;
  o = xor32_u64(v); v = o > v ? o : v;
  return v;
}
__device__ __forceinline__ unsigned long long half_min_u64(unsigned long long v) {
  unsigned long long o;
  o = dpp_u64<DPP_XOR1>(v); v = o < v ? o : v;
  o = dpp_u64<DPP_XOR2>(v); v = o < v ? o : v;
  o = dpp_u64<DPP_HALF_MIRROR>(v); v = o < v ? o : v;
  o = dpp_u64<DPP_MIRROR>(v); v = o < v ? o : v;
  o = xor16_u64(v); v = o < v ? o : v;
  return v;
}
__device__ __forceinline__ unsigned int half_min_u32(unsigned int v) {
  unsigned int o;
  o = (unsigned int)dpp_i32<DPP_XOR1>((int)v); v = o < v ? o : v;
  o = (unsigned int)dpp_i32<DPP_XOR2>((int)v); v = o < v ? o : v;
  o = (unsigned int)dpp_i32<DPP_HALF_MIRROR>((int)v); v = o < v ? o : v;
  o = (unsigned int)dpp_i32<DPP_MIRROR>((int)v); v = o < v ? o : v;
  o = (unsigned int)xor16_i32((int)v); v = o < v ? o : v;
  return v;
}
__device__ __forceinline__ unsigned int wave_max_u32(unsigned int v) {
  unsigned int o;
  o = (unsigned int)dpp_i32<DPP_XOR1>((int)v); v = o > v ? o : v;
  o = (unsigned int)dpp_i32<DPP_XOR2>((int)v); v = o > v ? o : v;
  o = (unsigned int)dpp_i32<DPP_HALF_MIRROR>((int)v); v = o > v ? o : v;
  o = (unsigned int)dpp_i32<DPP_MIRROR>((int)v); v = o > v ? o : v;
  o = (unsigned int)xor16_i32((int)v); v = o > v ? o : v;
  o = (unsigned int)xor32_i32((int)v); v = o > v ? o : v;
  return v;
}
__device__ __forceinline__ int wave_min_i32(int v) {
  int o;
  o = dpp_i32<DPP_XOR1>(v); v = o < v ? o : v;
  o = dpp_i32<DPP_XOR2>(v); v = o < v ? o : v;
  o = dpp_i32<DPP_HALF_MIRROR>(v); v = o < v ? o : v;
  o = dpp_i32<DPP_MIRROR>(v); v = o < v ? o : v;
  o = xor16_i32(v); v = o < v ? o : v;
  o = xor32_i32(v); v = o < v ? o : v;
  return v;
}

__device__ __forceinline__ double row_sum_f64(double x) {
  x += dpp_f64<DPP_XOR1>(x);
  x += dpp_f64<DPP_XOR2>(x);
  x += dpp_f64<DPP_HALF_MIRROR>(x);
  x += dpp_f64<DPP_MIRROR>(x);
  return x;
}

__device__ __forceinline__ int wave_incl_scan_i32(int v) {
  v += __builtin_amdgcn_update_dpp(0, v, DPP_ROW_SHR1, 0xF, 0xF, true);
  v += __builtin_amdgcn_update_dpp(0, v, DPP_ROW_SHR2, 0xF, 0xF, true);
  v += __builtin_amdgcn_update_dpp(0, v, DPP_ROW_SHR4, 0xF, 0xF, true);
  v += __builtin_amdgcn_update_dpp(0, v, DPP_ROW_SHR8, 0xF, 0xF, true);
  v += __builtin_amdgcn_update_dpp(0, v, DPP_ROW_BCAST15, 0xA, 0xF, true);
  v += __builtin_amdgcn_update_dpp(0, v, DPP_ROW_BCAST31, 0xC, 0xF, true);
  return v;
}
__device__ __forceinline__ int half_incl_scan_i32(int v) {
  v += __builtin_amdgcn_update_dpp(0, v, DPP_ROW_SHR1, 0xF, 0xF, true);
  v += __builtin_amdgcn_update_dpp(0, v, DPP_ROW_SHR2, 0xF, 0xF, true);
  v += __builtin_amdgcn_update_dpp(0, v, DPP_ROW_SHR4, 0xF, 0xF, true);
  v += __builtin_amdgcn_update_dpp(0, v, DPP_ROW_SHR8, 0xF, 0xF, true);
  v += __builtin_amdgcn_update_dpp(0, v, DPP_ROW_BCAST15, 0xA, 0xF, true);
  return v;
}

__device__ __forceinline__ int readlane_i32(int v, int lane ) {
  return __builtin_amdgcn_readlane(v, lane);
}

}
```

Before: 14450.

## Add whole-wave-per-query KNN variant for the chain-mode first pass

Templates the KNN cell streaming, merge, select and bound helpers on group width, so a query can use a full 64-lane wave instead of half a wave. When chain mode is on and the KNN grid is small relative to the CU count, the first pass launches with 512 threads and one query per wave. This doubles the lanes streaming each query's candidate cells, aiming to cut per-query latency on an under-filled GPU. In exchange it adds wider reductions and a separate tuning set, and the wide path skips saving positions for the second pass, which may cost reuse later.

```diff
diff --git a/liodom_amd/csrc/kernels_knn.h b/liodom_amd/csrc/kernels_knn.h
--- a/liodom_amd/csrc/kernels_knn.h
+++ b/liodom_amd/csrc/kernels_knn.h
@@ -69,11 +69,16 @@
 #define LIODOM_TUNE_D_LOADS 4
 #define LIODOM_TUNE_D_NEAR 0.04f
 #endif
-template <bool kDeep> struct KnnTune {
-  static constexpr int kBigCell = kDeep ? LIODOM_TUNE_D_BIG : LIODOM_TUNE_B_BIG;
-  static constexpr int kLoadsBig = kDeep ? LIODOM_TUNE_D_LOADS : LIODOM_TUNE_B_LOADS_BIG;
-  static constexpr int kLoadsFlat = kDeep ? LIODOM_TUNE_D_LOADS : LIODOM_TUNE_B_LOADS_FLAT;
-  static constexpr float kNearSq = kDeep ? LIODOM_TUNE_D_NEAR : LIODOM_TUNE_B_NEAR;
+#ifndef LIODOM_TUNE_W_BIG
+#define LIODOM_TUNE_W_BIG 128
+#define LIODOM_TUNE_W_LOADS 4
+#define LIODOM_TUNE_W_NEAR 0.04f
+#endif
+template <bool kDeep, bool kWide = false> struct KnnTune {
+  static constexpr int kBigCell = kWide ? LIODOM_TUNE_W_BIG : kDeep ? LIODOM_TUNE_D_BIG : LIODOM_TUNE_B_BIG;
+  static constexpr int kLoadsBig = kWide ? LIODOM_TUNE_W_LOADS : kDeep ? LIODOM_TUNE_D_LOADS : LIODOM_TUNE_B_LOADS_BIG;
+  static constexpr int kLoadsFlat = kWide ? LIODOM_TUNE_W_LOADS : kDeep ? LIODOM_TUNE_D_LOADS : LIODOM_TUNE_B_LOADS_FLAT;
+  static constexpr float kNearSq = kWide ? LIODOM_TUNE_W_NEAR : kDeep ? LIODOM_TUNE_D_NEAR : LIODOM_TUNE_B_NEAR;
   static constexpr bool kProbeBoth = kDeep;
   static constexpr bool kHoistLoads = kDeep;
   static constexpr bool kCursor = kDeep ? false : LIODOM_TUNE_B_CURSOR;
@@ -95,45 +100,46 @@
   return sqdist_f(qx, qy, qz, m.x, m.y, m.z);
 #endif
 }
-template <class Acc, int UB, int U, int kBigCell, bool kCursor = false>
+template <class Acc, int UB, int U, int kBigCell, bool kCursor = false, int kG = kKnnGroup>
 __device__ __forceinline__ void knn_stream_cells(Acc& t, const float4* sp, int* s_incl, int* s_adj,
                                                  unsigned int start, unsigned int cnt, int hl,
                                                  float qx, float qy, float qz, unsigned int* dbg = nullptr) {
   const unsigned long long dbg_t0 = dbg ? wall_clock64() : 0ull;
   {
-    const int half_base = (threadIdx.x & 32);
-    unsigned int big = (unsigned int)((__ballot(cnt >= (unsigned int)kBigCell) >> half_base) & 0xFFFFFFFFull);
+    grp_mask_t<kG> big = grp_ballot<kG>(cnt >= (unsigned int)kBigCell);
     while (big) {
-      const int l = __ffs(big) - 1;
+      const int l = grp_ffs<kG>(big) - 1;
       big &= big - 1u;
-      const int cs = __shfl((int)start, l, kKnnGroup), cc = __shfl((int)cnt, l, kKnnGroup);
+      const int cs = __shfl((int)start, l, kG), cc = __shfl((int)cnt, l, kG);
       const float4* cp = sp + cs;
-      for (int i = hl; i < cc; i += UB * kKnnGroup) {
+      for (int i = hl; i < cc; i += UB * kG) {
         float4 m[UB];
 #pragma unroll
-        for (int u = 0; u < UB; u++) { const int iu = i + u * kKnnGroup; m[u] = cp[iu < cc ? iu : cc - 1]; }
+        for (int u = 0; u < UB; u++) { const int iu = i + u * kG; m[u] = cp[iu < cc ? iu : cc - 1]; }
 #pragma unroll
         for (int u = 0; u < UB; u++) {
-          const int iu = i + u * kKnnGroup;
+          const int iu = i + u * kG;
           t.consider(iu < cc, sqdist_cand(qx, qy, qz, m[u]), __float_as_int(m[u].w), cs + iu);
         }
       }
     }
     if (cnt >= (unsigned int)kBigCell) cnt = 0;
   }
-  const unsigned int dbg_nseg = dbg ? (unsigned int)__popc((unsigned int)(__ballot(cnt > 0) >> (threadIdx.x & 32))) : 0u;
+  const unsigned int dbg_nseg = dbg ? (unsigned int)grp_popc<kG>(grp_ballot<kG>(cnt > 0)) : 0u;
   const int incl = half_incl_scan_i32((int)cnt);
-  s_incl[hl] = incl;
-  s_adj[hl] = (int)start - (incl - (int)cnt);
+  if (kG == kKnnGroup || hl < kKnnGroup) {
+    s_incl[hl] = incl;
+    s_adj[hl] = (int)start - (incl - (int)cnt);
+  }
   __builtin_amdgcn_wave_barrier();
   const int T = s_incl[kKnnGroup - 1];
   const unsigned long long dbg_t1 = dbg ? wall_clock64() : 0ull;
   int cur = 0;
-  for (int i = hl; i < T; i += U * kKnnGroup) {
+  for (int i = hl; i < T; i += U * kG) {
     int a[U];
     int c[U];
 #pragma unroll
-    for (int u = 0; u < U; u++) { const int iu = i + u * kKnnGroup; a[u] = iu < T ? iu : T - 1; c[u] = 0; }
+    for (int u = 0; u < U; u++) { const int iu = i + u * kG; a[u] = iu < T ? iu : T - 1; c[u] = 0; }
     if (kCursor) {
 #pragma unroll
       for (int u = 0; u < U; u++) {
@@ -160,34 +166,34 @@
     for (int u = 0; u < U; u++) m[u] = sp[a[u]];
 #pragma unroll
     for (int u = 0; u < U; u++)
-      t.consider(i + u * kKnnGroup < T, sqdist_cand(qx, qy, qz, m[u]), __float_as_int(m[u].w), a[u]);
+      t.consider(i + u * kG < T, sqdist_cand(qx, qy, qz, m[u]), __float_as_int(m[u].w), a[u]);
   }
   __builtin_amdgcn_wave_barrier();
   if (dbg && hl == 0) {
     dbg[0] = (unsigned int)(dbg_t1 - dbg_t0);
     dbg[1] = (unsigned int)(wall_clock64() - dbg_t1);
-    dbg[2] = ((unsigned int)((T + U * kKnnGroup - 1) / (U * kKnnGroup)) << 16) | ((unsigned int)T << 20);
+    dbg[2] = ((unsigned int)((T + U * kG - 1) / (U * kG)) << 16) | ((unsigned int)T << 20);
     dbg[3] = dbg_nseg;
   }
 }
 
-__device__ __forceinline__ bool best2_select(const Best2Acc& t, int hl, int half_shift, float& d5, int (&pos)[5]) {
+template <int kG = kKnnGroup>
+__device__ __forceinline__ bool best2_select(const Best2Acc& t, int hl, float& d5, int (&pos)[5]) {
   unsigned int v = (unsigned int)__float_as_int(t.m1), w = (unsigned int)__float_as_int(t.m2);
   int ph = t.p1, pn = t.p2;
   unsigned int g[6];
 #pragma unroll
   for (int r = 0; r < 5; r++) {
-    g[r] = half_min_u32(v);
-    const unsigned int win = (unsigned int)((__ballot(v == g[r]) >> half_shift) & 0xFFFFFFFFull);
-    const int l = __ffs(win) - 1;
-    pos[r] = __shfl(ph, l, kKnnGroup);
+    g[r] = grp_min_u32<kG>(v);
+    const int l = grp_ffs<kG>(grp_ballot<kG>(v == g[r])) - 1;
+    pos[r] = __shfl(ph, l, kG);
     const bool mine = hl == l;
     v = mine ? w : v;
     w = mine ? 0x7f800000u : w;
     ph = mine ? pn : ph;
   }
-  g[5] = half_min_u32(v);
-  const unsigned int s3 = half_min_u32((unsigned int)__float_as_int(t.m3));
+  g[5] = grp_min_u32<kG>(v);
+  const unsigned int s3 = grp_min_u32<kG>((unsigned int)__float_as_int(t.m3));
   const unsigned int one = 0x3f800000u;
   d5 = __int_as_float((int)g[4]);
   if (g[4] < one) return g[0] < g[1] && g[1] < g[2] && g[2] < g[3] && g[3] < g[4] && g[4] < g[5] && g[4] < s3;
@@ -195,22 +201,23 @@
 }
 
 
-__device__ __forceinline__ void knn_merge(Top5& t, Top5& g, int hl, int half_shift) {
+template <int kG = kKnnGroup>
+__device__ __forceinline__ void knn_merge(Top5& t, Top5& g, int hl) {
   unsigned long long gk[5]; int gp[5];
 #pragma unroll
   for (int r = 0; r < 5; r++) {
     const unsigned long long key = t.k0;
-    const unsigned int dmin = half_min_u32((unsigned int)(key >> 32));
-    unsigned int win = (unsigned int)((__ballot((unsigned int)(key >> 32) == dmin) >> half_shift) & 0xFFFFFFFFull);
+    const unsigned int dmin = grp_min_u32<kG>((unsigned int)(key >> 32));
+    grp_mask_t<kG> win = grp_ballot<kG>((unsigned int)(key >> 32) == dmin);
     unsigned long long mk;
-    if (__popc(win) == 1) {
-      mk = ((unsigned long long)dmin << 32) | (unsigned int)__shfl((int)(unsigned int)(key & 0xFFFFFFFFull), __ffs(win) - 1, kKnnGroup);
+    if (grp_popc<kG>(win) == 1) {
+      mk = ((unsigned long long)dmin << 32) | (unsigned int)__shfl((int)(unsigned int)(key & 0xFFFFFFFFull), grp_ffs<kG>(win) - 1, kG);
     } else {
-      mk = half_min_u64(key);
-      win = (unsigned int)((__ballot(key == mk) >> half_shift) & 0xFFFFFFFFull);
-    }
-    const int wl = __ffs(win) - 1;
-    gp[r] = __shfl(t.p0, wl, kKnnGroup);
+      mk = grp_min_u64<kG>(key);
+      win = grp_ballot<kG>(key == mk);
+    }
+    const int wl = grp_ffs<kG>(win) - 1;
+    gp[r] = __shfl(t.p0, wl, kG);
     gk[r] = mk;
     if (hl == wl) {
       t.k0 = t.k1; t.k1 = t.k2; t.k2 = t.k3; t.k3 = t.k4; t.k4 = kTop5Empty;
@@ -234,12 +241,13 @@
   double blk[kQ][24];
 };
 
-__device__ __forceinline__ float best2_bound(const Best2Acc& t, int half_shift) {
+template <int kG = kKnnGroup>
+__device__ __forceinline__ float best2_bound(const Best2Acc& t) {
   float B = 1.0f;
   const float thr[4] = {0.36f, 0.09f, 0.0225f, 0.0036f};
 #pragma unroll
   for (int k = 0; k < 4; k++) {
-    const int c = __popc((unsigned int)(__ballot(t.m1 <= thr[k]) >> half_shift)) + __popc((unsigned int)(__ballot(t.m2 <= thr[k]) >> half_shift));
+    const int c = grp_popc<kG>(grp_ballot<kG>(t.m1 <= thr[k])) + grp_popc<kG>(grp_ballot<kG>(t.m2 <= thr[k]));
     B = c >= 5 ? thr[k] : B;
   }
   return B;
@@ -342,16 +350,16 @@
   for (int k = 0; k < 5; k++) pre.c[k] = sp[pre.p[k] >= 0 ? pre.p[k] : 0];
 }
 
-template <int kKnnThreads, bool kPre = false, bool kTail = true, bool kWt = kPre>
+template <int kKnnThreads, bool kPre = false, bool kTail = true, bool kWt = kPre, int kG = kKnnGroup>
 __device__ __forceinline__ void knn_block(const DevView& v, int s, StreamState& st, int fc, int outer_it, int eb, int bv, int E,
-                                          KnnShared<kKnnThreads / kKnnGroup>& sh, const float4& p_in, const double (&T_in)[12],
+                                          KnnShared<kKnnThreads / kG>& sh, const float4& p_in, const double (&T_in)[12],
                                           const KnnPre& pre, const double* qt) {
-  constexpr int kKnnQueries = kKnnThreads / kKnnGroup;
-  typedef KnnTune<(kKnnThreads >= 256)> Tune;
-  const int grp = threadIdx.x / kKnnGroup;
+  constexpr int kKnnQueries = kKnnThreads / kG;
+  static_assert(kG == kKnnGroup || (!kPre && kWt), "whole-wave queries: the chain-mode first pass only");
+  typedef KnnTune<(kKnnThreads >= 256), (kG == 64)> Tune;
+  const int grp = threadIdx.x / kG;
   const int e = bv * kKnnQueries + grp;
-  const int hl = threadIdx.x & (kKnnGroup - 1);
-  const int half_shift = (threadIdx.x & 32);
+  const int hl = threadIdx.x & (kG - 1);
   const bool dbgb = (bv == 5) && (s == 0) && (threadIdx.x == 0) && (outer_it == 0);
   const unsigned long long t_blk = (kInstrument && (v.debug & 32)) ? wall_clock64() : 0ull;
   DBG_STAMP(v, dbgb, 1, 0);
@@ -394,7 +402,7 @@
         for (int k = 0; k < 5; k++) {
           if (pre.p[k] >= 0) top5_insert(t, sqdist_f(qx, qy, qz, pre.c[k].x, pre.c[k].y, pre.c[k].z), __float_as_int(pre.c[k].w), pre.p[k]);
         }
-        knn_merge(t, g, hl, half_shift);
+        knn_merge(t, g, hl);
         const float d5n = g.p4 >= 0 ? top5_dist(g.k4) : __int_as_float(0x7f800000);
         const double ddx = (double)qx - (double)pre.sq.x, ddy = (double)qy - (double)pre.sq.y, ddz = (double)qz - (double)pre.sq.z;
         const double delta = sqrt(ddx * ddx + ddy * ddy + ddz * ddz) * (1.0 + 1e-12);
@@ -440,7 +448,7 @@
         }
       }
     } else
-    if (outer_it == 1 && v.knn_save_pos && !v.knn_exact_only) {
+    if (kG == kKnnGroup && outer_it == 1 && v.knn_save_pos && !v.knn_exact_only) {
       const float gsq = v.knn_save_g[(size_t)s * v.edge_cap + e];
       if (gsq > 0.f) {
         const float4 sq = v.knn_save_q[(size_t)s * v.edge_cap + e];
@@ -452,7 +460,7 @@
         br.consider(sv.y >= 0, sqdist_f(qx, qy, qz, m1.x, m1.y, m1.z), 0, sv.y);
         float d5n;
         int p5[5];
-        const bool sel_ok = best2_select(br, hl, half_shift, d5n, p5);
+        const bool sel_ok = best2_select<kG>(br, hl, d5n, p5);
         const double ddx = (double)qx - (double)sq.x, ddy = (double)qy - (double)sq.y, ddz = (double)qz - (double)sq.z;
         const double delta = sqrt(ddx * ddx + ddy * ddy + ddz * ddz) * (1.0 + 1e-12);
         const double r = sqrt((double)gsq) * (1.0 - 2e-7) - delta;
@@ -490,24 +498,24 @@
     bool dbg_two_phase = false;
     {
       const bool now = pend && (have_b ? !(lb > B) : (hl == 13 || hl == 27 || lb <= Tune::kNearSq));
-      if (kInstrument && (v.debug & 32)) dbg_n = __shfl(half_incl_scan_i32(now ? (int)cnt : 0), kKnnGroup - 1, kKnnGroup);
-      knn_stream_cells<Best2Acc, Tune::kLoadsBig, Tune::kLoadsFlat, Tune::kBigCell, Tune::kCursor>(b2, sp, sh.incl[grp], sh.adj[grp], start, now ? cnt : 0u, hl, qx, qy, qz,
+      if (kInstrument && (v.debug & 32)) dbg_n = __shfl(half_incl_scan_i32(now ? (int)cnt : 0), kKnnGroup - 1, kG);
+      knn_stream_cells<Best2Acc, Tune::kLoadsBig, Tune::kLoadsFlat, Tune::kBigCell, Tune::kCursor, kG>(b2, sp, sh.incl[grp], sh.adj[grp], start, now ? cnt : 0u, hl, qx, qy, qz,
                                                                                      ((kInstrument && (v.debug & 32)) && s == 0 && e < E) ? v.dbg_q + ((size_t)outer_it * v.edge_cap + e) * 12 + 8 : nullptr);
       pend = pend && !now;
     }
     DBG_STAMP(v, dbgb, 1, 3); DBG_QSTAMP(3);
-    if (!have_b && ((__ballot(pend) >> half_shift) & 0xFFFFFFFFull)) {
-      B = best2_bound(b2, half_shift);
+    if (!have_b && grp_ballot<kG>(pend)) {
+      B = best2_bound<kG>(b2);
       pend = pend && !(lb > B);
-      if ((__ballot(pend) >> half_shift) & 0xFFFFFFFFull) {
-        if (kInstrument && (v.debug & 32)) { dbg_n += __shfl(half_incl_scan_i32(pend ? (int)cnt : 0), kKnnGroup - 1, kKnnGroup); dbg_two_phase = true; }
-        knn_stream_cells<Best2Acc, Tune::kLoadsBig, Tune::kLoadsFlat, Tune::kBigCell, Tune::kCursor>(b2, sp, sh.incl[grp], sh.adj[grp], start, pend ? cnt : 0u, hl, qx, qy, qz);
+      if (grp_ballot<kG>(pend)) {
+        if (kInstrument && (v.debug & 32)) { dbg_n += __shfl(half_incl_scan_i32(pend ? (int)cnt : 0), kKnnGroup - 1, kG); dbg_two_phase = true; }
+        knn_stream_cells<Best2Acc, Tune::kLoadsBig, Tune::kLoadsFlat, Tune::kBigCell, Tune::kCursor, kG>(b2, sp, sh.incl[grp], sh.adj[grp], start, pend ? cnt : 0u, hl, qx, qy, qz);
       }
     } else {
       pend = false;
     }
     DBG_STAMP(v, dbgb, 1, 4); DBG_QSTAMP(4);
-    const bool certain = best2_select(b2, hl, half_shift, d5, pos5) && !v.knn_exact_only;
+    const bool certain = best2_select<kG>(b2, hl, d5, pos5) && !v.knn_exact_only;
     if ((kInstrument && (v.debug & 32)) && s == 0 && e < E && hl == 0) v.dbg_q[((size_t)outer_it * v.edge_cap + e) * 12] = (unsigned int)dbg_n | (dbg_two_phase ? 0x40000000u : 0u) | (certain ? 0u : 0x80000000u);
     if ((kInstrument && (v.debug & 64)) && hl == 0) {
       atomicAdd(&v.dbg_clk[256 + (certain ? 0 : 1)], 1ull);
@@ -524,12 +532,12 @@
         ta.t.k0 = ta.t.k1 = ta.t.k2 = ta.t.k3 = ta.t.k4 = sentinel;
         ta.t.p0 = ta.t.p1 = ta.t.p2 = ta.t.p3 = ta.t.p4 = -1;
       }
-      knn_stream_cells<Top5Acc, 2, 2, 64>(ta, sp, sh.incl[grp], sh.adj[grp], start, all ? cnt : 0u, hl, qx, qy, qz);
-      knn_merge(ta.t, g, hl, half_shift);
+      knn_stream_cells<Top5Acc, 2, 2, 64, false, kG>(ta, sp, sh.incl[grp], sh.adj[grp], start, all ? cnt : 0u, hl, qx, qy, qz);
+      knn_merge<kG>(ta.t, g, hl);
       d5 = g.p4 >= 0 ? top5_dist(g.k4) : __int_as_float(0x7f800000);
       pos5[0] = g.p0; pos5[1] = g.p1; pos5[2] = g.p2; pos5[3] = g.p3; pos5[4] = g.p4;
     }
-    if (outer_it == 0 && v.knn_save_pos && !(kWt && !kPre)) {
+    if (kG == kKnnGroup && outer_it == 0 && v.knn_save_pos && !(kWt && !kPre)) {
       const float sk = (cnt > 0 && !(!(lb > B) || (!have_b && (hl == 13 || hl == 27 || lb <= Tune::kNearSq)))) ? lb : __int_as_float(0x7f800000);
       unsigned int gd = half_min_u32((unsigned int)__float_as_int(sk));
       const unsigned int m3m = half_min_u32((unsigned int)__float_as_int(b2.m3));
@@ -749,11 +757,12 @@
   if (signal_odo && threadIdx.x == 0) __hip_atomic_store((gu32*)(v.pipe_flags + kEdgePipeBufs), signal_odo, __ATOMIC_RELAXED, __HIP_MEMORY_SCOPE_AGENT);
 }
 
-template <int kKnnThreads, bool kOv, bool kChain>
+template <int kKnnThreads, bool kOv, bool kChain, int kG = kKnnGroup>
 __device__ __forceinline__ bool knn_pass(const DevView& v, int s, int bxi, int byi, int outer_it, int eb, unsigned int wait_edges,
-                                         unsigned int signal_odo, unsigned int seq, int scan_no, KnnShared<kKnnThreads / kKnnGroup>& sh, KnnShared<kKnnThreads / kKnnGroup>& sh2, double* sh_ov, int pred_copy = 0) {
-  constexpr int kKnnQueries = kKnnThreads / kKnnGroup;
+                                         unsigned int signal_odo, unsigned int seq, int scan_no, KnnShared<kKnnThreads / kG>& sh, KnnShared<kKnnThreads / kG>& sh2, double* sh_ov, int pred_copy = 0) {
+  constexpr int kKnnQueries = kKnnThreads / kG;
   static_assert(!(kOv && kChain), "the overlapped pass is the second pass, the chain-mode instance the first");
+  static_assert(kG == kKnnGroup || kChain, "whole-wave queries: the chain-mode first pass only");
   StreamState& st = v.state[s];
   if (kOv) {
     if (!pipe_wait(v.ov_flags + s, seq, &st.status)) return false;
@@ -779,8 +788,8 @@
     }
     if (!kChain && wait_edges && !pipe_wait(v.pipe_flags + eb, wait_edges, &st.status)) return false;
   }
-  typedef KnnTune<(kKnnThreads >= 256)> Tune;
-  const int e_first = bxi * kKnnQueries + (int)(threadIdx.x / kKnnGroup);
+  typedef KnnTune<(kKnnThreads >= 256), (kG == 64)> Tune;
+  const int e_first = bxi * kKnnQueries + (int)(threadIdx.x / kG);
   float4 p_first = make_float4(0.f, 0.f, 0.f, 0.f);
   double T[12] = {0, 0, 0, 0, 0, 0, 0, 0, 0, 0, 0, 0};
   if (Tune::kHoistLoads) {
@@ -817,11 +826,11 @@
     return true;
   }
   const int bv2 = bxi + v.knn_grid;
-  const int e_second = bv2 * kKnnQueries + (int)(threadIdx.x / kKnnGroup);
+  const int e_second = bv2 * kKnnQueries + (int)(threadIdx.x / kG);
   const bool second = bv2 < v.knn_blocks && bv2 * kKnnQueries < E;
   KnnPre pre1, pre2;
   float4 p_second = make_float4(0.f, 0.f, 0.f, 0.f);
-  if (kOv) {
+  if constexpr (kOv) {
     if (second) p_second = v.edges[((size_t)eb * v.n_streams + s) * v.edge_cap + (e_second < v.edge_cap ? e_second : v.edge_cap - 1)];
     knn_presearch<kKnnThreads>(v, s, st, fc, e_first, E, sh, pre1, sqrtf(p_first.x * p_first.x + p_first.y * p_first.y + p_first.z * p_first.z));
     if (second) knn_presearch<kKnnThreads>(v, s, st, fc, e_second, E, sh2, pre2, sqrtf(p_second.x * p_second.x + p_second.y * p_second.y + p_second.z * p_second.z));
@@ -848,7 +857,7 @@
     if ((kInstrument && (v.debug & 64)) && threadIdx.x == 0) atomicAdd(&v.dbg_clk[271 + (cf == 1 ? 0 : 1)], 1ull);
     return cf == 1;
   }
-  knn_block<kKnnThreads, false, true, kWt>(v, s, st, fc, outer_it, eb, bxi, E, sh, p_first, T, pre1, kChain ? sh_ov + 12 : nullptr);
+  knn_block<kKnnThreads, false, true, kWt, kG>(v, s, st, fc, outer_it, eb, bxi, E, sh, p_first, T, pre1, kChain ? sh_ov + 12 : nullptr);
   if (bv2 >= v.knn_blocks) return true;
   if (!second) {
     if (threadIdx.x == 0) { unsigned char* cm = &v.corr_mask[((size_t)s * 2 + outer_it) * v.mask_stride + bv2]; if (kWt) wt_store_u8(cm, 0); else *cm = 0; }
@@ -867,13 +876,13 @@
       for (int i = 0; i < 12; i++) T2[i] = st.odom[i];
     }
   }
-  knn_block<kKnnThreads, false, true, kWt>(v, s, st, fc, outer_it, eb, bv2, E, sh, p_second, T2, pre2, kChain ? sh_ov + 12 : nullptr);
+  knn_block<kKnnThreads, false, true, kWt, kG>(v, s, st, fc, outer_it, eb, bv2, E, sh, p_second, T2, pre2, kChain ? sh_ov + 12 : nullptr);
   return true;
 }
 
-template <int kKnnThreads, bool kOv = false, bool kChain = false>
+template <int kKnnThreads, bool kOv = false, bool kChain = false, int kG = kKnnGroup>
 __global__ __launch_bounds__(kKnnThreads, (kKnnThreads >= 256 ? 1 : LIODOM_TUNE_B_WAVES)) void k_knn(DevView v, int s0, int outer_it, int eb, unsigned int wait_edges, unsigned int signal_odo, unsigned int seq, int scan_no) {
-  constexpr int kKnnQueries = kKnnThreads / kKnnGroup;
+  constexpr int kKnnQueries = kKnnThreads / kG;
 #if defined(LIODOM_CHAIN_PRIO)
   if (kKnnThreads >= 256) __builtin_amdgcn_s_setprio(LIODOM_CHAIN_PRIO);
 #endif
@@ -908,7 +917,7 @@
     }
     OV_STAMP(v, threadIdx.x == 0 && bxi == 0, 16);
   }
-  const bool pass_ok = knn_pass<kKnnThreads, kOv, kChain>(v, s, bxi, byi, outer_it, eb, wait_edges, signal_odo, seq, scan_no, sh, shs[kOv ? 1 : 0], sh_ov);
+  const bool pass_ok = knn_pass<kKnnThreads, kOv, kChain, kG>(v, s, bxi, byi, outer_it, eb, wait_edges, signal_odo, seq, scan_no, sh, shs[kOv ? 1 : 0], sh_ov);
   if (kOv) { if (scan_no >= 0) { if (pass_ok) chain_count_done(v.knn_done0 + 32 + s); } else if (pass_ok || !v.speculate) ov_signal_knn_done(v, s, bxi, seq); }
   if (kChain) {
     int vd = 1;
diff --git a/liodom_amd/csrc/liodom_hip.hip b/liodom_amd/csrc/liodom_hip.hip
--- a/liodom_amd/csrc/liodom_hip.hip
+++ b/liodom_amd/csrc/liodom_hip.hip
@@ -70,6 +70,7 @@
   double replay_enq_ns = 0.0, replay_wait_ns = 0.0;
   long long replay_timed = 0;
   bool chain_ok = false;
+  bool chain_wide = false;
   bool chain_prev = false;
   unsigned int chain_count = 0;
   int verdict_scan = -1;
@@ -313,7 +314,8 @@
     const int gx = (h->v.lm_groups - 1) * 8 + 1;
     const size_t lds = lm_lds_bytes(h->v.edge_cap);
     const int nCP = cdiv(h->v.edge_cap * std::max(1, h->P - 1), 256) + cdiv(h->v.edge_cap, 256);
-    hipLaunchKernelGGL((k_knn<256, false, true>), dim3(v.knn_grid, 1), dim3(256), 0, h->stream_k, v, s0, 0, eb, wait_edges, signal_odo, seq_k, scan_no);
+    if (h->chain_wide) hipLaunchKernelGGL((k_knn<512, false, true, 64>), dim3(v.knn_grid, 1), dim3(512), 0, h->stream_k, v, s0, 0, eb, wait_edges, signal_odo, seq_k, scan_no);
+    else hipLaunchKernelGGL((k_knn<256, false, true>), dim3(v.knn_grid, 1), dim3(256), 0, h->stream_k, v, s0, 0, eb, wait_edges, signal_odo, seq_k, scan_no);
     if (v.speculate) {
       const int nA = cdiv(h->v.edge_cap, 256);
       hipLaunchKernelGGL(k_chain_redo0<256>, dim3(nA + v.knn_grid + 1, 1), dim3(256), 0, h->stream_k, v, s0, eb, wait_edges, signal_odo, seq_k, scan_no, nA, 1, h->chain_fix_pending ? 1 : 0);
@@ -904,6 +906,7 @@
     h->ov_ok = knn_overlap != 0 && v.early_rebuild && S == 1 && v.knn_partials && (knn_overlap == 2 || (long long)v.knn_grid * 4 * 3 <= (long long)cus * 24);
     h->chain_ok = v.early_rebuild && S == 1 && v.knn_partials && !v.use_imu && (long long)v.knn_grid * 4 * 2 <= (long long)cus * 24;
     if (knn_overlap == 0 || env_int("LIODOM_CHAIN", 1) == 0) h->chain_ok = false;
+    h->chain_wide = h->chain_ok && (long long)v.knn_grid * 8 * 2 <= (long long)cus * 24;
     v.speculate = (h->ov_ok || h->chain_ok) ? 1 : 0;
     if (v.speculate) v.speculate = std::max(0, std::min(7, env_int("LIODOM_SPECULATE", 1)));
     v.spec_backoff = 16;
@@ -1766,13 +1769,13 @@
   snprintf(buf, (size_t)cap,
            "n_streams=%d early_rebuild=%d hash_build=%s pipe_flags=%d flag_gate=%d lm_groups=%d knn_instance=%d knn_queries=%d "
            "knn_grid=%d/%d knn8=%d hash_incr=%d hash_rebuilds=%d hash_appends=%d hash_appends_spilled=%d hash_points_spilled=%d knn_partials=%d knn_saved_bound=%d knn_exact_only=%d line_gate_kernel=%d filter_local_map=%d mapping=%d "
-           "rotation_mode=%d table_size=%d rebuild_delta=%.3f knn_overlap=%d streams_concurrent=%d safe_mode=%d ring_split=%d ring_split_max_wgs=%d ring_split_lb=%d chain=%d speculate=%d spec_early=%d/%d spec_unconfirmed=%d/%d chain_done=%u/%u/%u replay_enqueue_us=%.2f replay_wait_us=%.2f debug=%d",
+           "rotation_mode=%d table_size=%d rebuild_delta=%.3f knn_overlap=%d streams_concurrent=%d safe_mode=%d ring_split=%d ring_split_max_wgs=%d ring_split_lb=%d chain=%d chain_wide=%d speculate=%d spec_early=%d/%d spec_unconfirmed=%d/%d chain_done=%u/%u/%u replay_enqueue_us=%.2f replay_wait_us=%.2f debug=%d",
            h->S, v.early_rebuild, v.early_rebuild ? "streamed" : (h->lds_hash_build ? "lds" : "global"), h->use_flags ? 1 : 0,
            (h->use_flags && h->flag_gate) ? 1 : 0, v.lm_groups, h->lockstep ? 128 : 256, v.knn_queries, v.knn_grid,
            v.knn_blocks, h->knn8 ? 1 : 0, v.hash_incr, hbs[0], hbs[1], hbs[2], hbs[3], v.knn_partials, v.knn_save_pos ? 2 : (v.knn_save_q ? 1 : 0), v.knn_exact_only, v.knn_nn ? 1 : 0, v.filter_local_map, v.mapping,
            v.rotation_mode, v.table_size, (double)v.rebuild_delta,
            (om.ov || om.chain) ? 1 : 0, h->streams_concurrent ? 1 : 0, h->safe_mode ? 1 : 0, h->ring_split ? 1 : 0, h->ring_split ? h->ring_split_max_wgs : 0, h->ring_split_lb ? 1 : 0,
-           om.chain ? 1 : 0, v.speculate, spec[0], spec[2], spec[1], spec[3], h->chain_count, done_cnt[0], done_cnt[32],
+           om.chain ? 1 : 0, (om.chain && h->chain_wide) ? 1 : 0, v.speculate, spec[0], spec[2], spec[1], spec[3], h->chain_count, done_cnt[0], done_cnt[32],
            h->replay_timed ? h->replay_enq_ns / (1e3 * (double)h->replay_timed) : 0.0, h->replay_timed ? h->replay_wait_ns / (1e3 * (double)h->replay_timed) : 0.0, v.debug);
   return LIODOM_OK;
 }
diff --git a/liodom_amd/csrc/wave_ops.h b/liodom_amd/csrc/wave_ops.h
--- a/liodom_amd/csrc/wave_ops.h
+++ b/liodom_amd/csrc/wave_ops.h
@@ -1,5 +1,6 @@
 #pragma once
 #include <hip/hip_runtime.h>
+#include <type_traits>
 
 namespace liodom_dev {
 
@@ -125,6 +126,35 @@
   return v;
 }
 
+template <int kG> using grp_mask_t = typename std::conditional<kG == 64, unsigned long long, unsigned int>::type;
+template <int kG>
+__device__ __forceinline__ grp_mask_t<kG> grp_ballot(bool p) {
+  static_assert(kG == 32 || kG == 64, "half or whole wave");
+  if constexpr (kG == 64) return __ballot(p);
+  else return (unsigned int)((__ballot(p) >> (threadIdx.x & 32)) & 0xFFFFFFFFull);
+}
+template <int kG>
+__device__ __forceinline__ int grp_ffs(grp_mask_t<kG> m) {
+  if constexpr (kG == 64) return __ffsll(m);
+  else return __ffs(m);
+}
+template <int kG>
+__device__ __forceinline__ int grp_popc(grp_mask_t<kG> m) {
+  if constexpr (kG == 64) return __popcll(m);
+  else return __popc(m);
+}
+template <int kG>
+__device__ __forceinline__ unsigned int grp_min_u32(unsigned int v) {
+  v = half_min_u32(v);
+  if constexpr (kG == 64) { const unsigned int o = (unsigned int)xor32_i32((int)v); v = o < v ? o : v; }
+  return v;
+}
+template <int kG>
+__device__ __forceinline__ unsigned long long grp_min_u64(unsigned long long v) {
+  v = half_min_u64(v);
+  if constexpr (kG == 64) { const unsigned long long o = xor32_u64(v); v = o < v ? o : v; }
+  return v;
+}
 __device__ __forceinline__ int readlane_i32(int v, int lane ) {
   return __builtin_amdgcn_readlane(v, lane);
 }
```

After: 14770, median of 6. 2.2% higher.
